# allenai/embodied-clip

Measured on AMD Instinct MI355X. Metric: env-frames/sec (CLIP encode + policy fwd/bwd + PPO update), higher is better.
Workload: dtype bf16

## Files before the change

embodied_clip_amd/_lib.py:

```python
from __future__ import annotations

import ctypes as C
import os

_HERE = os.path.dirname(os.path.abspath(__file__))
LIB_PATH = os.environ.get("EC_AMD_LIB") or os.path.join(_HERE, "lib", "libec_amd.so")

c_void_p, c_int, c_size_t, c_float = C.c_void_p, C.c_int, C.c_size_t, C.c_float

SIGNATURES = {
    "ec_version": (c_int, []),
    "ec_strerror": (C.c_char_p, [c_int]),
    "ec_bind_streams": (c_int, [c_void_p, c_int, c_int]),
    "ec_stream_pair_overlap": (c_int, [c_void_p, c_void_p, c_int, c_void_p]),
    "ec_conv_bf16": (c_int, [c_void_p] * 5 + [c_int] * 8 + [c_void_p]),
    "ec_conv_bf16_ld": (c_int, [c_void_p] * 5 + [c_int] * 9 + [c_void_p]),
    "ec_conv3x3_img_pack": (c_int, [c_void_p, c_void_p, c_int, c_void_p]),
    "ec_conv3x3_img_bf16": (c_int, [c_void_p] * 4 + [c_int] * 5 + [c_void_p]),
    "ec_conv3x3_img_bf16_ld": (c_int, [c_void_p] * 4 + [c_int] * 6 + [c_void_p]),
    "ec_bneck3_packed_elems": (c_size_t, [c_int]),
    "ec_bneck3_pack_weights": (c_int, [c_void_p] * 4 + [c_int, c_void_p]),
    "ec_bneck_conv123_bf16": (c_int, [c_void_p] * 6 + [c_int] * 4 + [c_void_p]),
    "ec_bneck_packed_elems": (c_size_t, [c_int]),
    "ec_bneck_pack_weights": (c_int, [c_void_p] * 3 + [c_int, c_void_p]),
    "ec_bneck_conv23_bf16": (c_int, [c_void_p] * 6 + [c_int] * 4 + [c_void_p]),
    "ec_clip_resize_table_ints": (c_size_t, [c_int, c_int, c_int]),
    "ec_clip_resize_table": (c_int, [c_int, c_int, c_int, c_void_p, c_size_t]),
    "ec_clip_resize_crop_u8": (c_int, [c_void_p, c_void_p, c_int, c_void_p, c_int, c_int, c_int, c_int, c_void_p]),
    "ec_semantic_labels_u8": (c_int, [c_void_p] * 4 + [c_int] * 4 + [c_void_p]),
    "ec_gemm_bf16": (c_int, [c_void_p] * 5 + [c_int] * 4 + [c_void_p]),
    "ec_split3_bf16": (c_int, [c_void_p] * 2 + [C.c_long, c_int, c_void_p]),
    "ec_gemm_bf16a_x3": (c_int, [c_void_p] * 4 + [C.c_long, c_int, c_int, c_int, c_void_p]),
    "ec_dw_tn_x3_splits": (c_int, [C.c_long, c_int]),
    "ec_dw_tn_x3": (c_int, [c_void_p] * 4 + [C.c_long, c_int, c_void_p]),
    "ec_stem_conv1": (c_int, [c_void_p] * 4 + [c_int] * 4 + [c_void_p]),
    "ec_avgpool2_bf16": (c_int, [c_void_p] * 2 + [c_int] * 4 + [c_void_p]),
    "ec_avgpool2_bf16_ld": (c_int, [c_void_p] * 2 + [c_int] * 5 + [c_void_p]),
    "ec_nhwc_bf16_to_nchw_f32": (c_int, [c_void_p] * 2 + [c_int] * 3 + [c_void_p]),
    "ec_nchw_f32_to_nhwc_bf16": (c_int, [c_void_p, c_void_p, c_int, c_int, c_int, c_void_p, c_void_p]),
    "ec_spatial_mean_bf16": (c_int, [c_void_p] * 2 + [c_int] * 3 + [c_void_p]),
    "ec_rn50_create": (c_int, [C.POINTER(c_void_p), c_int, C.POINTER(c_int), c_int, c_void_p, c_void_p, c_size_t,
                               c_void_p, c_size_t]),
    "ec_rn50tv_create": (c_int, [C.POINTER(c_void_p), C.POINTER(c_int), c_int, c_void_p, c_void_p, c_size_t, c_void_p,
                                 c_size_t]),
    "ec_conv_bf16_s2": (c_int, [c_void_p] * 5 + [c_int] * 7 + [c_void_p]),
    "ec_basic_tail_s2_bf16": (c_int, [c_void_p] * 5 + [c_int] * 6 + [c_void_p]),
    "ec_tvresnet_basic_create": (c_int, [C.POINTER(c_void_p), C.POINTER(c_int), c_int, c_void_p, c_void_p, c_size_t,
                                         c_void_p, c_size_t]),
    "ec_stem7_pool": (c_int, [c_void_p, c_int, C.POINTER(c_float), C.POINTER(c_float), c_void_p, c_void_p, c_void_p,
                              c_int, c_int, c_int, c_void_p]),
    "ec_rn50_destroy": (None, [c_void_p]),
    "ec_rn50_workspace_bytes": (c_size_t, [c_void_p, c_int]),
    "ec_rn50_out_channels": (c_int, [c_void_p]),
    "ec_rn50_out_spatial": (c_int, [c_void_p]),
    "ec_rn50_forward": (c_int, [c_void_p, c_void_p, c_int, c_void_p, c_size_t, c_void_p, c_int, c_void_p]),
    "ec_stem_conv1_depth": (c_int, [c_void_p, c_float, c_float, c_void_p, c_void_p, c_void_p] + [c_int] * 4 + [c_void_p]),
    "ec_rn50_forward_depth": (c_int, [c_void_p, c_void_p, c_float, c_float, c_void_p, c_int, c_void_p, c_size_t, c_void_p, c_int,
                                      c_void_p]),
    "ec_spatial_mean_pair_bf16": (c_int, [c_void_p] * 3 + [c_int] * 3 + [c_void_p]),
    "ec_rn50_rgbd_workspace_bytes": (c_size_t, [c_void_p, c_int]),
    "ec_rn50_embed_rgbd": (c_int, [c_void_p, c_void_p, c_int, C.POINTER(c_float), C.POINTER(c_float), c_void_p, c_float, c_float,
                                   c_void_p, c_int, c_void_p, c_size_t, c_void_p, c_int, c_void_p]),
    "ec_rn50_num_ops": (c_int, [c_void_p]),
    "ec_rn50_plan_hash": (C.c_uint64, [c_void_p]),
    "ec_rn50_set_conv8_min_tiles": (c_int, [c_void_p, c_int]),
    "ec_text_create": (c_int, [C.POINTER(c_void_p), c_int, c_int, c_int, c_int, c_int, c_int, c_void_p, c_size_t, c_void_p,
                               c_size_t]),
    "ec_text_destroy": (None, [c_void_p]),
    "ec_text_workspace_bytes": (c_size_t, [c_void_p, c_int]),
    "ec_text_forward": (c_int, [c_void_p, c_void_p, c_int, c_void_p, c_size_t, c_void_p, c_void_p]),
    "ec_probe_head": (c_int, [c_int, c_void_p, c_void_p, c_void_p, c_int, c_int, c_int, c_void_p, c_void_p, c_void_p,
                              c_void_p, c_void_p]),
    "ec_probe_pool3": (c_int, [c_void_p, c_void_p, c_int, c_int, c_int, c_int, c_void_p]),
    "ec_conv1x1_pair_pool_bf16": (c_int, [c_void_p] * 9 + [c_int] * 6 + [c_void_p]),
    "ec_conv1x1_pair_bf16": (c_int, [c_void_p] * 11 + [C.c_long, c_int, c_int, c_int, c_void_p]),
    "ec_stem_conv1_u8": (c_int, [c_void_p, C.POINTER(c_float), C.POINTER(c_float), c_void_p, c_void_p, c_void_p]
                         + [c_int] * 4 + [c_void_p]),
    "ec_rn50_forward_u8": (c_int, [c_void_p, c_void_p, C.POINTER(c_float), C.POINTER(c_float), c_int, c_void_p,
                                   c_size_t, c_void_p, c_int, c_void_p]),
    "ec_gemm_f32": (c_int, [c_void_p] * 3 + [c_int] * 3 + [C.c_long] * 4 + [c_int, c_int] + [c_void_p] * 3 + [c_int]
                    + [c_void_p] * 2 + [c_int, c_void_p]),
    "ec_policy_create": (c_int, [C.POINTER(c_void_p), c_void_p]),
    "ec_policy_destroy": (None, [c_void_p]),
    "ec_policy_num_param_tensors": (c_int, [c_void_p]),
    "ec_policy_flat_size": (c_size_t, [c_void_p]),
    "ec_policy_param_offset": (c_int, [c_void_p, c_int, C.POINTER(c_size_t), C.POINTER(c_size_t)]),
    "ec_policy_workspace_bytes": (c_size_t, [c_void_p, c_int, c_int, c_int]),
    "ec_policy_forward": (c_int, [c_void_p, c_void_p, c_void_p, c_int, c_void_p, c_void_p, c_void_p, c_int, c_int,
                                  c_void_p, c_size_t, c_int, c_void_p, c_void_p, c_void_p]),
    "ec_policy_forward2": (c_int, [c_void_p, c_void_p, c_void_p, c_void_p, c_int, c_void_p, c_void_p, c_void_p, c_int, c_int,
                                   c_void_p, c_size_t, c_int, c_void_p, c_void_p, c_void_p]),
    "ec_policy_act": (c_int, [c_void_p] * 4 + [c_int] + [c_void_p] * 3 + [c_int, c_void_p, c_size_t, c_int] + [c_void_p] * 5
                      + [C.c_uint64, C.c_uint64, c_int, c_void_p]),
    "ec_policy_forward_vec": (c_int, [c_void_p, c_void_p, c_void_p, c_void_p, c_int, c_void_p, c_void_p, c_void_p, c_int, c_int,
                                      c_void_p, c_size_t, c_int, c_void_p, c_void_p, c_void_p]),
    "ec_policy_act_vec": (c_int, [c_void_p] * 4 + [c_int] + [c_void_p] * 3 + [c_int, c_void_p, c_size_t, c_int] + [c_void_p] * 5
                          + [C.c_uint64, C.c_uint64, c_int, c_void_p]),
    "ec_policy_act_greedy": (c_int, [c_void_p] * 4 + [c_int] + [c_void_p] * 3 + [c_int, c_void_p, c_size_t, c_int] + [c_void_p] * 5
                             + [c_void_p]),
    "ec_policy_act_vec_greedy": (c_int, [c_void_p] * 4 + [c_int] + [c_void_p] * 3 + [c_int, c_void_p, c_size_t, c_int] + [c_void_p] * 5
                                 + [c_void_p]),
    "ec_policy_backward2": (c_int, [c_void_p, c_void_p, c_void_p, c_void_p, c_int, c_void_p, c_int, c_int, c_void_p, c_size_t,
                                    c_void_p, c_void_p, c_void_p, c_void_p]),
    "ec_policy_backward3": (c_int, [c_void_p, c_void_p, c_void_p, c_void_p, c_int, c_void_p, c_int, c_int, c_void_p, c_size_t,
                                    c_void_p, c_void_p, c_void_p, c_void_p, c_void_p]),
    "ec_policy_set_goal_table": (c_int, [c_void_p, c_void_p]),
    "ec_policy_backward": (c_int, [c_void_p, c_void_p, c_void_p, c_int, c_void_p, c_int, c_int, c_void_p, c_size_t,
                                   c_void_p, c_void_p, c_void_p, c_void_p]),
    "ec_gae": (c_int, [c_void_p] * 7 + [c_int, c_int, c_float, c_float, c_float, c_void_p]),
    "ec_ppo_loss": (c_int, [c_void_p] * 8 + [C.c_long, c_int, c_float, c_float, c_float, c_float, c_void_p]),
    "ec_ppo_loss_ex": (c_int, [c_void_p] * 8 + [C.c_long, c_int, c_float, c_float, c_float, c_float, c_float, c_void_p]),
    "ec_sample_actions": (c_int, [c_void_p] * 4 + [c_int, c_int, C.c_uint64, C.c_uint64, c_int, c_void_p]),
    "ec_mode_actions": (c_int, [c_void_p] * 4 + [c_int, c_int, c_void_p]),
    "ec_episode_stats": (c_int, [c_void_p] * 8 + [c_int, c_void_p, c_int, c_int, c_void_p]),
    "ec_nav_episode_stats": (c_int, [c_void_p] * 7 + [c_int] + [c_void_p] * 6 + [c_int, c_void_p, c_int, c_int, c_void_p]),
    "ec_vit_create": (c_int, [C.POINTER(c_void_p), c_int, c_int, c_int, c_int, c_int, c_void_p, c_size_t, c_void_p,
                              c_size_t]),
    "ec_vit_destroy": (None, [c_void_p]),
    "ec_vit_tokens": (c_int, [c_void_p]),
    "ec_vit_set_conv8_min_tiles": (c_int, [c_void_p, c_int]),
    "ec_vit_plan_hash": (C.c_uint64, [c_void_p]),
    "ec_vit_workspace_bytes": (c_size_t, [c_void_p, c_int]),
    "ec_vit_forward": (c_int, [c_void_p, c_void_p, c_int, c_void_p, c_size_t, c_void_p, c_void_p]),
    "ec_mha_bf16": (c_int, [c_void_p] * 2 + [c_int] * 5 + [c_void_p]),
    "ec_layernorm_bf16": (c_int, [c_void_p] * 4 + [C.c_long, c_int, c_void_p]),
    "ec_vit_assemble_bf16": (c_int, [c_void_p] * 7 + [c_int] * 3 + [c_void_p]),
    "ec_row_stats_bf16": (c_int, [c_void_p] * 2 + [C.c_long, c_int, c_void_p]),
    "ec_ln_fold_bf16": (c_int, [c_void_p] * 7 + [c_int] * 2 + [c_void_p]),
    "ec_gemm_bf16_ln": (c_int, [c_void_p] * 5 + [c_int] * 4 + [c_void_p] * 2 + [c_int, c_void_p, C.POINTER(c_int), c_void_p]),
    "ec_bf16_to_f32": (c_int, [c_void_p, c_void_p, C.c_long, C.c_long, C.c_long, c_void_p]),
    "ec_attnpool_workspace_bytes": (c_size_t, [c_int, c_int, c_int]),
    "ec_attnpool_forward": (c_int, [c_void_p, c_int, c_int, c_int, c_int, c_int] + [c_void_p] * 8 + [c_size_t, c_void_p,
                                    c_void_p]),
    "ec_clip_adam_scratch_doubles": (c_int, []),
    "ec_clip_adam_step": (c_int, [c_void_p] * 5 + [C.c_long, c_float, c_float, c_float, c_float, c_float, c_int,
                                  c_void_p]),
    "ec_imitation_scratch_doubles": (c_int, []),
    "ec_imitation_loss": (c_int, [c_void_p] * 7 + [C.c_long, c_int, c_float, c_float, c_int, c_void_p]),
    "ec_expert_count": (c_int, [c_void_p, c_int, c_int, c_int, c_int, c_void_p, c_void_p]),
    "ec_teacher_force": (c_int, [c_void_p] * 3 + [c_float] + [c_void_p] * 2 + [c_int, c_int, C.c_uint64, C.c_uint64, c_int,
                                                                            c_void_p]),
    "ec_heads_wide": (c_int, [c_void_p] * 6 + [C.c_long, c_int, c_int] + [c_void_p] * 3 + [c_int, C.c_uint64, C.c_uint64, c_int]
                      + [c_void_p] * 2 + [c_float, c_void_p]),
    "ec_policy_act_ex": (c_int, [c_void_p] * 4 + [c_int] + [c_void_p] * 4 + [c_int, c_void_p, c_size_t, c_int] + [c_void_p] * 5
                         + [c_int, C.c_uint64, C.c_uint64, c_int] + [c_void_p] * 2 + [c_float, c_void_p]),
    "ec_ppo_loss_wide_scratch_doubles": (c_int, []),
    "ec_ppo_loss_wide": (c_int, [c_void_p] * 9 + [C.c_long, c_int, c_float, c_float, c_float, c_float, c_float, c_void_p]),
    "ec_prev_action_table": (c_int, [c_void_p, c_void_p, C.c_long, c_int, c_void_p, c_int, c_int, c_int, c_int, c_void_p]),
    "ec_prev_action_add": (c_int, [c_void_p] * 4 + [c_int, c_int, C.c_long, c_int, c_void_p]),
    "ec_prev_action_grad_scratch_floats": (c_size_t, [C.c_long, c_int, c_int, c_int]),
    "ec_policy_forward_pa": (c_int, [c_void_p] * 4 + [c_int] + [c_void_p] * 5 + [c_int, c_int, c_void_p, c_size_t, c_int] + [c_void_p] * 3),
    "ec_policy_act_pa": (c_int, [c_void_p] * 4 + [c_int] + [c_void_p] * 5 + [c_int, c_void_p, c_size_t, c_int] + [c_void_p] * 5
                         + [c_int, C.c_uint64, C.c_uint64, c_int] + [c_void_p] * 2 + [c_float, c_void_p]),
    "ec_prev_action_grad": (c_int, [c_void_p] * 3 + [c_int, c_int, c_void_p, c_void_p, C.c_long, c_int] + [c_void_p] * 3
                            + [C.c_long, c_int, c_int, c_void_p]),
    "ec_policy_create_rnn": (c_int, [C.POINTER(c_void_p), c_void_p, c_int]),
    "ec_policy_rnn_type": (c_int, [c_void_p]),
    "ec_policy_create_rnn_layers": (c_int, [C.POINTER(c_void_p), c_void_p, c_int, c_int]),
    "ec_policy_rnn_layers": (c_int, [c_void_p]),
    "ec_rnn_stack_step_fwd": (c_int, [c_int, c_void_p, C.c_long] + [c_void_p] * 5 + [C.c_long, c_void_p, c_void_p, C.c_long, c_void_p, C.c_long,
                                      c_void_p, C.c_long, c_int, c_int, c_void_p]),
    "ec_policy_state_width": (c_int, [c_void_p]),
    "ec_lstm_step_fwd": (c_int, [c_void_p] * 4 + [C.c_long, c_void_p, c_void_p, C.c_long, c_void_p, C.c_long, c_void_p, c_int, c_int,
                                 c_void_p]),
    "ec_lstm_step_bwd": (c_int, [c_void_p] * 12 + [c_int, c_int, c_void_p]),
    "ec_policy_create_pooled": (c_int, [C.POINTER(c_void_p), c_void_p]),
    "ec_policy_is_pooled": (c_int, [c_void_p]),
    "ec_policy_forward_pooled": (c_int, [c_void_p] * 8 + [c_int, c_int, c_void_p, c_size_t, c_int] + [c_void_p] * 3),
    "ec_policy_act_pooled": (c_int, [c_void_p] * 8 + [c_int, c_void_p, c_size_t, c_int] + [c_void_p] * 5
                             + [c_int, C.c_uint64, C.c_uint64, c_int] + [c_void_p] * 2 + [c_float, c_void_p]),
    "ec_pooled_fc_act": (c_int, [c_void_p] * 5 + [c_int] * 3 + [c_void_p]),
    "ec_pooled_step0_fwd": (c_int, [c_int, c_void_p, C.c_long] + [c_void_p] * 7 + [c_int, c_void_p, c_void_p, c_int, c_int, c_void_p, c_void_p,
                                    c_int, c_void_p, C.c_long, c_void_p, c_void_p, C.c_long, c_void_p, C.c_long, c_void_p, C.c_long, c_int,
                                    c_int, c_void_p]),
}

RNN_TYPES = {"GRU": 0, "LSTM": 1}


class PolicyCfg(C.Structure):
    _fields_ = [(n, c_int) for n in ("in_channels", "spatial", "hidden", "goal_dims", "num_goals", "num_actions",
                                     "compress_hid", "compress_out", "comb_hid", "comb_out", "fusion", "dual", "goal_in",
                                     "prev_action_dims", "prev_action_null")]


class PooledCfg(C.Structure):
    _fields_ = [("embed_in", c_int), ("hidden", c_int), ("embed_dims", c_int), ("num_goals", c_int), ("num_sensors", c_int),
                ("sensor_in", c_int * 3), ("num_actions", c_int), ("prev_action_dims", c_int), ("prev_action_null", c_int),
                ("rnn_type", c_int), ("num_layers", c_int)]


_lib = None


class EcError(RuntimeError):
    pass


def load() -> C.CDLL:
    global _lib
    if _lib is not None:
        return _lib
    if not os.path.exists(LIB_PATH):
        raise ImportError(
            f"embodied_clip_amd: HIP library not found at {LIB_PATH}. Build it with `make` or "
            "`python -c 'import __graft_entry__ as g; g.build()'` (needs hipcc, gfx950). "
            "There is deliberately no CPU fallback.")
    lib = C.CDLL(LIB_PATH)
    for name, (res, args) in SIGNATURES.items():
        fn = getattr(lib, name)
        fn.restype = res
        fn.argtypes = args
    _lib = lib
    return lib


def check(rc: int, what: str = "") -> None:
    if rc != 0:
        msg = load().ec_strerror(rc).decode()
        raise EcError(f"{what or 'ec_amd call'} failed: {msg} (code {rc})")


def ptr(t) -> int:
    return 0 if t is None else t.data_ptr()


def stream_ptr(device=None) -> int:
    import torch
# ... 56 lines not shown
```

embodied_clip_amd/csrc/conv_pair.hip:

```cpp
#include <stdlib.h>

#include <type_traits>
#include <utility>

#include "common.h"

namespace {

typedef unsigned int u32x4 __attribute__((ext_vector_type(4)));
constexpr int PX = 32;
constexpr int NY = 256;
constexpr int KA = 64;
constexpr int SP = 272;
constexpr int STG = PX * SP;

struct PairArgs {
    const uint16_t *a0, *a1, *w0, *w1, *w2, *res;
    const float *b0, *b1, *b2;
    uint16_t *y, *z;
    int ntiles;
    uint16_t* yp;
    int H, W;
};

__device__ __forceinline__ float pq_xor1(float v) {
    return __builtin_bit_cast(float, __builtin_amdgcn_update_dpp(0, __builtin_bit_cast(int, v), 0xB1, 0xF, 0xF, true));
}
__device__ __forceinline__ float pq_xor2(float v) {
    return __builtin_bit_cast(float, __builtin_amdgcn_update_dpp(0, __builtin_bit_cast(int, v), 0x4E, 0xF, 0xF, true));
}

__device__ __forceinline__ int pw_off(int row, int chunk) {
    return row * 128 + ((chunk ^ ((row >> 1) & 7)) << 4);
}

template <int I, int LEAD, class AddrFn>
__device__ __forceinline__ void lsm_issue(u32x4 (&ring)[LEAD], AddrFn& addr) {
    const auto a = addr(std::integral_constant<int, I>{});
    asm volatile("ds_read_b128 %0, %1 offset:%2" : "=v"(ring[I % LEAD]) : "v"(a.first), "n"(decltype(a.second)::value));
}
template <int I, int NSTEP, int LEAD, class AddrFn, class MmaFn>
__device__ __forceinline__ void lsm_step(u32x4 (&ring)[LEAD], AddrFn& addr, MmaFn& mma) {
    if constexpr (I < NSTEP) {
        constexpr int after = (LEAD - 1 < NSTEP - 1 - I) ? LEAD - 1 : NSTEP - 1 - I;
        asm volatile("s_waitcnt lgkmcnt(%1)" : "+v"(ring[I % LEAD]) : "n"(after));
        mma(std::integral_constant<int, I>{}, ring[I % LEAD]);
        if constexpr (I + LEAD < NSTEP) lsm_issue<I + LEAD, LEAD>(ring, addr);
        lsm_step<I + 1, NSTEP, LEAD>(ring, addr, mma);
    }
}
template <int I, int N, int LEAD, class AddrFn>
__device__ __forceinline__ void lsm_prologue(u32x4 (&ring)[LEAD], AddrFn& addr) {
    if constexpr (I < N) {
        lsm_issue<I, LEAD>(ring, addr);
        lsm_prologue<I + 1, N, LEAD>(ring, addr);
    }
}
template <int NSTEP, int LEAD, class AddrFn, class MmaFn>
__device__ __forceinline__ void lds_stream_mfma(AddrFn addr, MmaFn mma) {
    u32x4 ring[LEAD];
    lsm_prologue<0, (LEAD < NSTEP ? LEAD : NSTEP), LEAD>(ring, addr);
    lsm_step<0, NSTEP, LEAD>(ring, addr, mma);
}

template <bool TWO, bool RES, int N2, bool PL>
__global__ __launch_bounds__(256, 1) void conv1x1_pair_kernel(PairArgs p) {
    static_assert(!PL || N2 == 128, "pooled variant: the layer-1 -> layer-2 boundary");
    constexpr int W0_BYTES = (TWO ? 2 : 1) * NY * 128;
    constexpr int W2_BYTES = 4 * N2 * 128;
    constexpr int FN2 = N2 / 32;
    extern __shared__ __attribute__((aligned(16))) unsigned char sm[];
    unsigned char* sW0 = sm;
    unsigned char* sW2 = sm + W0_BYTES;
    float* sBy = reinterpret_cast<float*>(sm + W0_BYTES + W2_BYTES);
    float* sBz = sBy + NY;
    const int tid = threadIdx.x, lane = tid & 63, wave = tid >> 6;
    unsigned char* stg = sm + W0_BYTES + W2_BYTES + (NY + N2) * 4 + wave * STG;
    const int px = lane & 31, h = lane >> 5;
    const unsigned w_lds = (unsigned)(unsigned long)(__attribute__((address_space(3))) unsigned char*)sW0;
    unsigned wk_off[4];
#pragma unroll
    for (int ks = 0; ks < 4; ++ks) wk_off[ks] = (unsigned)pw_off(px, 2 * ks + h);
    auto roff = [&](int r) -> int {
        if (!PL) return r;
        return (2 * (r >> 4) + ((r >> 1) & 1)) * p.W + 2 * ((r >> 2) & 3) + (r & 1);
    };
    const int roff_px = roff(px);
    int rrow[8];
#pragma unroll
    for (int j = 0; j < 8; ++j) rrow[j] = roff(4 * j + (lane >> 4));
    auto tile_base = [&](int tile) -> long {
        if (!PL) return (long)tile * PX;
        const int t = __builtin_amdgcn_readfirstlane(tile);
        const int tpr = p.W / 8, tpi = (p.H / 4) * tpr;
        const int b = t / tpi, rem = t - b * tpi, ty = rem / tpr, tx = rem - ty * tpr;
        return ((long)b * p.H + 4 * ty) * p.W + 8 * tx;
    };

    ec_stage_all<(TWO ? 2 : 1) * NY * 8, 256, uint4>(
        tid,
        [&](int idx) {
            const int kt = idx / (NY * 8), r = (idx / 8) % NY, c = idx & 7;
            return *reinterpret_cast<const uint4*>((kt == 0 ? p.w0 : p.w1) + r * KA + c * 8);
        },
        [&](int idx, const uint4& v) {
            const int kt = idx / (NY * 8), r = (idx / 8) % NY, c = idx & 7;
            *reinterpret_cast<uint4*>(sW0 + kt * (NY * 128) + pw_off(r, c)) = v;
        });
    ec_stage_all<N2 * 32, 256, uint4>(
        tid,
        [&](int idx) {
            const int n = idx >> 5, q = idx & 31;
            const int s = q >> 1, hh = q & 1;
            const int c0 = 32 * (s >> 1) + 16 * (s & 1) + 4 * hh;
            const uint2 lo = *reinterpret_cast<const uint2*>(p.w2 + n * NY + c0);
            const uint2 hi = *reinterpret_cast<const uint2*>(p.w2 + n * NY + c0 + 8);
            return make_uint4(lo.x, lo.y, hi.x, hi.y);
        },
        [&](int idx, const uint4& v) {
            const int n = idx >> 5, q = idx & 31;
            const int s = q >> 1, hh = q & 1;
            *reinterpret_cast<uint4*>(sW2 + (s >> 2) * (N2 * 128) + pw_off(n, 2 * (s & 3) + hh)) = v;
        });
    for (int i = tid; i < NY; i += 256) sBy[i] = p.b0[i] + (TWO ? p.b1[i] : 0.f);
    for (int i = tid; i < N2; i += 256) sBz[i] = p.b2[i];
    __syncthreads();

    const int gw = blockIdx.x * 4 + wave, GW = gridDim.x * 4;
    int t = gw;
    if (t >= p.ntiles) return;

    u32x4 a0n[4], a1n[TWO ? 4 : 1], rn[RES ? 16 : 1];
    auto prefetch = [&](int tile) {
        const long m0 = tile_base(tile);
#pragma unroll
        for (int ks = 0; ks < 4; ++ks) {
            a0n[ks] = *reinterpret_cast<const u32x4*>(p.a0 + (m0 + roff_px) * KA + (2 * ks + h) * 8);
            if (TWO) a1n[ks] = *reinterpret_cast<const u32x4*>(p.a1 + (m0 + roff_px) * KA + (2 * ks + h) * 8);
        }
        if constexpr (RES) {
            [&]<int... I>(std::integer_sequence<int, I...>) {
                ((rn[I] = *reinterpret_cast<const u32x4*>(p.res + (m0 + rrow[I & 7]) * NY + (I >> 3) * 128 +
                                                          (((I & 7) * 64 + lane) & 15) * 8)), ...);
            }(std::make_integer_sequence<int, 16>{});
        }
    };
    prefetch(t);

    for (;;) {
        const long m0 = tile_base(t);
        u32x4 a0c[4], a1c[TWO ? 4 : 1], rc[RES ? 16 : 1];
#pragma unroll
        for (int ks = 0; ks < 4; ++ks) { a0c[ks] = a0n[ks]; if (TWO) a1c[ks] = a1n[ks]; }
        if constexpr (RES) {
            [&]<int... I>(std::integer_sequence<int, I...>) { ((rc[I] = rn[I]), ...); }(std::make_integer_sequence<int, 16>{});
        }
        const int tn = t + GW;
        const bool more = tn < p.ntiles;
        if (more) prefetch(tn);

        f32x16_t acc[8];
#pragma unroll
        for (int j = 0; j < 8; ++j)
#pragma unroll
            for (int r = 0; r < 16; ++r) acc[j][r] = 0.f;
        {
            constexpr int PER_KS = (TWO ? 16 : 8);
            lds_stream_mfma<4 * PER_KS, 8>(
                [&](auto ic) {
                    constexpr int i = decltype(ic)::value, ks = i / PER_KS, r = i % PER_KS, j = r & 7, second = r >> 3;
                    return std::pair<unsigned, std::integral_constant<int, second * (NY * 128) + j * 4096>>{w_lds + wk_off[ks], {}};
                },
                [&](auto ic, const u32x4& wf) {
                    constexpr int i = decltype(ic)::value, ks = i / PER_KS, r = i % PER_KS, j = r & 7, second = r >> 3;
                    acc[j] = __builtin_amdgcn_mfma_f32_32x32x16_bf16(__builtin_bit_cast(bf16x8_t, wf),
                                                                     __builtin_bit_cast(bf16x8_t, second ? a1c[TWO ? ks : 0] : a0c[ks]),
                                                                     acc[j], 0, 0, 0);
                });
        }

        uint4 P[8][2];
        long pool_base = 0;
        if constexpr (PL) {
            const int tt = __builtin_amdgcn_readfirstlane(t);
            const int tpr = p.W / 8, tpi = (p.H / 4) * tpr;
            const int b = tt / tpi, rem = tt - b * tpi, ty = rem / tpr, tx = rem - ty * tpr;
            pool_base = ((long)b * (p.H / 2) + 2 * ty) * (p.W / 2) + 4 * tx;
        }
        auto half_epilogue = [&](auto hfc) {
            constexpr int hf = decltype(hfc)::value;
            if constexpr (RES) {
                [&]<int... I>(std::integer_sequence<int, I...>) {
                    ((*reinterpret_cast<u32x4*>(stg + ((I * 64 + lane) >> 4) * SP + ((I * 64 + lane) & 15) * 16) = rc[hf * 8 + I]), ...);
                }(std::make_integer_sequence<int, 8>{});
            }
#pragma unroll
            for (int jj = 0; jj < 4; ++jj) {
                const int j = hf * 4 + jj;
                unsigned pk[8];
#pragma unroll
                for (int g = 0; g < 4; ++g) {
                    const int lc = 32 * jj + 8 * g + 4 * h;
                    const float4 bv = *reinterpret_cast<const float4*>(sBy + hf * 128 + lc);
                    float v0 = acc[j][4 * g + 0] + bv.x, v1 = acc[j][4 * g + 1] + bv.y;
                    float v2 = acc[j][4 * g + 2] + bv.z, v3 = acc[j][4 * g + 3] + bv.w;
                    uint2* slot = reinterpret_cast<uint2*>(stg + px * SP + lc * 2);
                    if (RES) {
                        const uint2 rr = *slot;
                        v0 += ec_lo(rr.x); v1 += ec_hi(rr.x); v2 += ec_lo(rr.y); v3 += ec_hi(rr.y);
                    }
                    v0 = fmaxf(v0, 0.f); v1 = fmaxf(v1, 0.f); v2 = fmaxf(v2, 0.f); v3 = fmaxf(v3, 0.f);
                    uint2 o;
                    o.x = ec_pack2(v0, v1);
                    o.y = ec_pack2(v2, v3);
                    *slot = o;
                    pk[2 * g] = o.x; pk[2 * g + 1] = o.y;
                }
                P[j][0] = make_uint4(pk[0], pk[1], pk[2], pk[3]);
                P[j][1] = make_uint4(pk[4], pk[5], pk[6], pk[7]);
            }
            if constexpr (PL) {
#pragma unroll
                for (int it2 = 0; it2 < 2; ++it2) {
                    const int item = it2 * 64 + lane, w = item >> 4, c = item & 15;
                    const uint4 r0 = *reinterpret_cast<const uint4*>(stg + (4 * w + 0) * SP + c * 16);
                    const uint4 r1 = *reinterpret_cast<const uint4*>(stg + (4 * w + 1) * SP + c * 16);
                    const uint4 r2 = *reinterpret_cast<const uint4*>(stg + (4 * w + 2) * SP + c * 16);
                    const uint4 r3 = *reinterpret_cast<const uint4*>(stg + (4 * w + 3) * SP + c * 16);
                    auto avg2 = [](unsigned a, unsigned b, unsigned cc, unsigned d) {
                        const float lo = 0.25f * ((ec_lo(a) + ec_lo(b)) + (ec_lo(cc) + ec_lo(d)));
                        const float hi = 0.25f * ((ec_hi(a) + ec_hi(b)) + (ec_hi(cc) + ec_hi(d)));
                        return ec_pack2(lo, hi);
                    };
                    u32x4 po;
                    po[0] = avg2(r0.x, r1.x, r2.x, r3.x); po[1] = avg2(r0.y, r1.y, r2.y, r3.y);
                    po[2] = avg2(r0.z, r1.z, r2.z, r3.z); po[3] = avg2(r0.w, r1.w, r2.w, r3.w);
                    *reinterpret_cast<u32x4*>(p.yp + (pool_base + (w >> 2) * (p.W / 2) + (w & 3)) * NY + hf * 128 + c * 8) = po;
                }
            }
            if (!PL || p.y) {
#pragma unroll
            for (int i = 0; i < 8; ++i) {
                const int idx = i * 64 + lane;
                const uint4 v = *reinterpret_cast<const uint4*>(stg + (idx >> 4) * SP + (idx & 15) * 16);
                __builtin_nontemporal_store(__builtin_bit_cast(u32x4, v), reinterpret_cast<u32x4*>(p.y + (m0 + rrow[i]) * NY + hf * 128 + (idx & 15) * 8));
            }
            }
        };
        half_epilogue(std::integral_constant<int, 0>{});
        half_epilogue(std::integral_constant<int, 1>{});

        f32x16_t acc2[FN2];
#pragma unroll
        for (int n = 0; n < FN2; ++n)
#pragma unroll
            for (int r = 0; r < 16; ++r) acc2[n][r] = 0.f;
        lds_stream_mfma<16 * FN2, 8>(
            [&](auto ic) {
                constexpr int i = decltype(ic)::value, st = i / FN2, n = i % FN2;
                return std::pair<unsigned, std::integral_constant<int, (st >> 2) * (N2 * 128) + n * 4096>>{w_lds + (unsigned)W0_BYTES + wk_off[st & 3], {}};
            },
            [&](auto ic, const u32x4& wf) {
                constexpr int i = decltype(ic)::value, st = i / FN2, n = i % FN2;
                acc2[n] = __builtin_amdgcn_mfma_f32_32x32x16_bf16(__builtin_bit_cast(bf16x8_t, wf),
                                                                  __builtin_bit_cast(bf16x8_t, P[st >> 1][st & 1]), acc2[n], 0, 0, 0);
            });
        constexpr int ZP = N2 * 2 + 16;
        constexpr int ZC = N2 / 8;
#pragma unroll
        for (int n = 0; n < FN2; ++n)
#pragma unroll
            for (int g = 0; g < 4; ++g) {
                const int lc = 32 * n + 8 * g + 4 * h;
                const float4 bv = *reinterpret_cast<const float4*>(sBz + lc);
                uint2 o;
                o.x = ec_pack2(fmaxf(acc2[n][4 * g + 0] + bv.x, 0.f), fmaxf(acc2[n][4 * g + 1] + bv.y, 0.f));
                o.y = ec_pack2(fmaxf(acc2[n][4 * g + 2] + bv.z, 0.f), fmaxf(acc2[n][4 * g + 3] + bv.w, 0.f));
                *reinterpret_cast<uint2*>(stg + px * ZP + lc * 2) = o;
            }
#pragma unroll
        for (int i = 0; i < PX * ZC / 64; ++i) {
            const int idx = i * 64 + lane;
            const uint4 v = *reinterpret_cast<const uint4*>(stg + (idx / ZC) * ZP + (idx % ZC) * 16);
            __builtin_nontemporal_store(__builtin_bit_cast(u32x4, v), reinterpret_cast<u32x4*>(p.z + (m0 + (PL ? rrow[i] : idx / ZC)) * N2 + (idx % ZC) * 8));
        }
        if (!more) break;
        t = tn;
    }
}

template <bool TWO, bool RES, int N2, bool PL = false>
int launch_pair(const PairArgs& p, hipStream_t s) {
    constexpr size_t lds = (size_t)(TWO ? 2 : 1) * NY * 128 + 4 * N2 * 128 + (NY + N2) * 4 + 4 * STG;
    static_assert(lds <= 160 * 1024, "LDS budget");
    auto kern = conv1x1_pair_kernel<TWO, RES, N2, PL>;
    static std::atomic<uint64_t> attr_done{0};
    if (auto attr_g_ = ec_attr_needed(attr_done)) {
        (void)hipFuncSetAttribute(reinterpret_cast<const void*>(kern), hipFuncAttributeMaxDynamicSharedMemorySize, (int)lds);
    }
    const int wgs = (p.ntiles + 3) / 4 < 256 ? (p.ntiles + 3) / 4 : 256;
    hipLaunchKernelGGL(kern, dim3((unsigned)wgs), dim3(256), lds, s, p);
    EC_CHECK_LAUNCH();
    return EC_OK;
}


constexpr int K2 = 128, NY2 = 512, NZ2 = 128;
constexpr int YP2 = NY2 * 2 + 16;
constexpr int SP2 = 256 + 16;

struct Pair2Args {
    const uint16_t *a0, *w0, *w2, *res;
    const float *b0, *b2;
    uint16_t *y, *z;
    int ntiles;
};

__global__ __launch_bounds__(256, 1) void conv1x1_pair512_kernel(Pair2Args p) {
    extern __shared__ __attribute__((aligned(16))) unsigned char sm[];
    unsigned char* ytile = sm;
    float* sBy = reinterpret_cast<float*>(sm + 2 * PX * YP2);
    float* sBz = sBy + NY2;
    const int tid = threadIdx.x, lane = tid & 63, wave = tid >> 6;
    unsigned char* stg = sm + 2 * PX * YP2 + (NY2 + NZ2) * 4 + wave * (PX * SP2);
    unsigned char* atile = sm + 2 * PX * YP2 + (NY2 + NZ2) * 4 + 4 * (PX * SP2);
    const int px = lane & 31, h = lane >> 5;

    for (int i = tid; i < NY2; i += 256) sBy[i] = p.b0[i];
    for (int i = tid; i < NZ2; i += 256) sBz[i] = p.b2[i];

    u32x4 w0f[4][8];
    u32x4 w2f[32];
    [&]<int... I>(std::integer_sequence<int, I...>) {
        ((w0f[I >> 3][I & 7] = *reinterpret_cast<const u32x4*>(p.w0 + (long)(128 * wave + 32 * (I >> 3) + px) * K2 + 16 * (I & 7) + 8 * h)), ...);
    }(std::make_integer_sequence<int, 32>{});
    [&]<int... I>(std::integer_sequence<int, I...>) {
        ((w2f[I] = *reinterpret_cast<const u32x4*>(p.w2 + (long)(32 * wave + px) * NY2 + 16 * I + 8 * h)), ...);
    }(std::make_integer_sequence<int, 32>{});
    __syncthreads();

    int t = blockIdx.x;
    if (t >= p.ntiles) return;
    const int G = gridDim.x;

    u32x4 an[2], rn[8];
    auto prefetch = [&](int tile) {
        const long m0 = (long)tile * PX;
        [&]<int... I>(std::integer_sequence<int, I...>) {
            ((an[I] = *reinterpret_cast<const u32x4*>(p.a0 + (m0 + 8 * wave + 4 * I + (lane >> 4)) * K2 + (lane & 15) * 8)), ...);
        }(std::make_integer_sequence<int, 2>{});
        [&]<int... I>(std::integer_sequence<int, I...>) {
            ((rn[I] = *reinterpret_cast<const u32x4*>(p.res + (m0 + ((I * 64 + lane) >> 4)) * NY2 + 128 * wave + ((I * 64 + lane) & 15) * 8)), ...);
        }(std::make_integer_sequence<int, 8>{});
    };
    auto publish_a = [&](int buf) {
        [&]<int... I>(std::integer_sequence<int, I...>) {
            ((*reinterpret_cast<u32x4*>(atile + buf * (PX * SP2) + (8 * wave + 4 * I + (lane >> 4)) * SP2 + (lane & 15) * 16) = an[I]), ...);
        }(std::make_integer_sequence<int, 2>{});
    };
    prefetch(t);
    publish_a(0);
    __syncthreads();

    for (int it = 0;; ++it) {
        const long m0 = (long)t * PX;
        unsigned char* yt = ytile + (it & 1) * (PX * YP2);
        u32x4 rc[8];
        [&]<int... I>(std::integer_sequence<int, I...>) { ((rc[I] = rn[I]), ...); }(std::make_integer_sequence<int, 8>{});
        const unsigned char* at = atile + (it & 1) * (PX * SP2);
        const int tn = t + G;
        const bool more = tn < p.ntiles;
        if (more) prefetch(tn);

        f32x16_t acc[4];
#pragma unroll
        for (int j = 0; j < 4; ++j)
#pragma unroll
            for (int r = 0; r < 16; ++r) acc[j][r] = 0.f;
        {
            const unsigned a_lds = (unsigned)(unsigned long)(__attribute__((address_space(3))) const unsigned char*)at +
                                   (unsigned)(px * SP2 + 16 * h);
            lds_stream_mfma<8, 6>(
                [&](auto ic) { return std::pair<unsigned, std::integral_constant<int, 32 * decltype(ic)::value>>{a_lds, {}}; },
                [&](auto ic, const u32x4& avr) {
                    constexpr int ks = decltype(ic)::value;
                    const bf16x8_t av = __builtin_bit_cast(bf16x8_t, avr);
#pragma unroll
                    for (int j = 0; j < 4; ++j)
                        acc[j] = __builtin_amdgcn_mfma_f32_32x32x16_bf16(__builtin_bit_cast(bf16x8_t, w0f[j][ks]), av, acc[j], 0, 0, 0);
                });
        }

        [&]<int... I>(std::integer_sequence<int, I...>) {
            ((*reinterpret_cast<u32x4*>(stg + ((I * 64 + lane) >> 4) * SP2 + ((I * 64 + lane) & 15) * 16) = rc[I]), ...);
        }(std::make_integer_sequence<int, 8>{});
#pragma unroll
        for (int j = 0; j < 4; ++j)
#pragma unroll
            for (int g = 0; g < 4; ++g) {
                const int lc = 32 * j + 8 * g + 4 * h;
                const float4 bv = *reinterpret_cast<const float4*>(sBy + 128 * wave + lc);
                uint2* slot = reinterpret_cast<uint2*>(stg + px * SP2 + lc * 2);
                const uint2 rr = *slot;
                const float v0 = fmaxf(acc[j][4 * g + 0] + bv.x + ec_lo(rr.x), 0.f), v1 = fmaxf(acc[j][4 * g + 1] + bv.y + ec_hi(rr.x), 0.f);
                const float v2 = fmaxf(acc[j][4 * g + 2] + bv.z + ec_lo(rr.y), 0.f), v3 = fmaxf(acc[j][4 * g + 3] + bv.w + ec_hi(rr.y), 0.f);
                uint2 o;
                o.x = ec_pack2(v0, v1);
                o.y = ec_pack2(v2, v3);
                *slot = o;
                *reinterpret_cast<uint2*>(yt + px * YP2 + (128 * wave + lc) * 2) = o;
            }
#pragma unroll
        for (int i = 0; i < 8; ++i) {
            const int idx = i * 64 + lane;
            const u32x4 v = *reinterpret_cast<const u32x4*>(stg + (idx >> 4) * SP2 + (idx & 15) * 16);
            __builtin_nontemporal_store(v, reinterpret_cast<u32x4*>(p.y + (m0 + (idx >> 4)) * NY2 + 128 * wave + (idx & 15) * 8));
        }
        if (more) publish_a((it + 1) & 1);
        __syncthreads();

        f32x16_t acc2;
#pragma unroll
        for (int r = 0; r < 16; ++r) acc2[r] = 0.f;
        {
            const unsigned y_lds = (unsigned)(unsigned long)(__attribute__((address_space(3))) const unsigned char*)yt +
                                   (unsigned)(px * YP2 + 16 * h);
            lds_stream_mfma<32, 8>(
                [&](auto ic) { return std::pair<unsigned, std::integral_constant<int, 32 * decltype(ic)::value>>{y_lds, {}}; },
                [&](auto ic, const u32x4& yv) {
                    constexpr int I = decltype(ic)::value;
                    acc2 = __builtin_amdgcn_mfma_f32_32x32x16_bf16(__builtin_bit_cast(bf16x8_t, w2f[I]), __builtin_bit_cast(bf16x8_t, yv), acc2, 0, 0, 0);
                });
// ... 78 lines not shown
    u32x4 an[AL], rn[RES ? OL : 1];
    const int Wq = PL ? p.W / 2 : 1, QPF = PL ? (p.H / 2) * Wq : 1;
    const int coff = PL ? ((lane >> 5) & 1) * p.W + ((lane >> 4) & 1) : 0;
    auto qpix = [&](int q_) -> long {
        const int q = __builtin_amdgcn_readfirstlane(q_);
        const int f = q / QPF, rem = q - f * QPF, qr = rem / Wq, qc = rem - qr * Wq;
        return ((long)f * p.H + 2 * qr) * p.W + 2 * qc;
    };
    long opix[PL ? OL : 1];
    auto prefetch = [&](int tile) {
        const long m0 = (long)tile * PX;
        if constexpr (PL) {
            static_assert(!PL || (CPR == 16 && OC == 16 && AL == 2 && OL == 8), "row = 4 I + (lane >> 4)");
            [&]<int... I>(std::integer_sequence<int, I...>) {
                ((an[I] = *reinterpret_cast<const u32x4*>(p.a + (qpix(8 * tile + 2 * wave + I) + coff) * K + (lane & 15) * 8)), ...);
            }(std::make_integer_sequence<int, AL>{});
            [&]<int... I>(std::integer_sequence<int, I...>) {
                ((opix[I] = qpix(8 * tile + I) + coff,
                  rn[I] = *reinterpret_cast<const u32x4*>(resg + opix[I] * ld + NPW * wave + (lane & 15) * 8)), ...);
            }(std::make_integer_sequence<int, OL>{});
            return;
        }
        [&]<int... I>(std::integer_sequence<int, I...>) {
            ((an[I] = *reinterpret_cast<const u32x4*>(p.a + (m0 + 8 * wave + (I * 64 + lane) / CPR) * K + ((I * 64 + lane) % CPR) * 8)), ...);
        }(std::make_integer_sequence<int, AL>{});
        if constexpr (RES) {
            [&]<int... I>(std::integer_sequence<int, I...>) {
                ((rn[I] = *reinterpret_cast<const u32x4*>(resg + (m0 + (I * 64 + lane) / OC) * ld + NPW * wave + ((I * 64 + lane) % OC) * 8)), ...);
            }(std::make_integer_sequence<int, OL>{});
        }
    };
    auto publish_a = [&](int buf) {
        [&]<int... I>(std::integer_sequence<int, I...>) {
            ((*reinterpret_cast<u32x4*>(atile + buf * (PX * AP) + (8 * wave + (I * 64 + lane) / CPR) * AP + ((I * 64 + lane) % CPR) * 16) = an[I]), ...);
        }(std::make_integer_sequence<int, AL>{});
    };
    prefetch(t);
    publish_a(0);
    __syncthreads();

    for (int it = 0;; ++it) {
        const long m0 = (long)t * PX;
        const unsigned char* at = atile + (it & 1) * (PX * AP);
        u32x4 rc[RES ? OL : 1];
        long opc[PL ? OL : 1];
        if constexpr (RES) {
            [&]<int... I>(std::integer_sequence<int, I...>) { ((rc[I] = rn[I]), ...); }(std::make_integer_sequence<int, OL>{});
        }
        if constexpr (PL) {
            [&]<int... I>(std::integer_sequence<int, I...>) { ((opc[I] = opix[I]), ...); }(std::make_integer_sequence<int, OL>{});
        }
        const int tn = t + G;
        const bool more = tn < p.ntiles;
        if (more) prefetch(tn);

        f32x16_t acc[FJ];
#pragma unroll
        for (int j = 0; j < FJ; ++j)
#pragma unroll
            for (int r = 0; r < 16; ++r) acc[j][r] = 0.f;
        {
            const unsigned a_lds = (unsigned)(unsigned long)(__attribute__((address_space(3))) const unsigned char*)at +
                                   (unsigned)(px * AP + 16 * h);
            lds_stream_mfma<KS, (KS < 6 ? KS : 6)>(
                [&](auto ic) { return std::pair<unsigned, std::integral_constant<int, 32 * decltype(ic)::value>>{a_lds, {}}; },
                [&](auto ic, const u32x4& avr) {
                    constexpr int I = decltype(ic)::value;
                    const bf16x8_t av = __builtin_bit_cast(bf16x8_t, avr);
#pragma unroll
                    for (int j = 0; j < FJ; ++j)
                        acc[j] = __builtin_amdgcn_mfma_f32_32x32x16_bf16(__builtin_bit_cast(bf16x8_t, wf[j][I]), av, acc[j], 0, 0, 0);
                });
        }

        if constexpr (RES) {
            [&]<int... I>(std::integer_sequence<int, I...>) {
                ((*reinterpret_cast<u32x4*>(stg + ((I * 64 + lane) / OC) * OPW + ((I * 64 + lane) % OC) * 16) = rc[I]), ...);
            }(std::make_integer_sequence<int, OL>{});
        }
#pragma unroll
        for (int j = 0; j < FJ; ++j)
#pragma unroll
            for (int g = 0; g < 4; ++g) {
                const int lc = 32 * j + 8 * g + 4 * h;
                const float4 bv = *reinterpret_cast<const float4*>(sB + NPW * wave + lc);
                uint2* slot = reinterpret_cast<uint2*>(stg + px * OPW + lc * 2);
                float v0 = acc[j][4 * g + 0] + bv.x, v1 = acc[j][4 * g + 1] + bv.y;
                float v2 = acc[j][4 * g + 2] + bv.z, v3 = acc[j][4 * g + 3] + bv.w;
                if constexpr (RES) {
                    const uint2 rr = *slot;
                    v0 += ec_lo(rr.x); v1 += ec_hi(rr.x); v2 += ec_lo(rr.y); v3 += ec_hi(rr.y);
                }
                if constexpr (RELU) { v0 = fmaxf(v0, 0.f); v1 = fmaxf(v1, 0.f); v2 = fmaxf(v2, 0.f); v3 = fmaxf(v3, 0.f); }
                uint2 o;
                o.x = ec_pack2(v0, v1);
                o.y = ec_pack2(v2, v3);
                *slot = o;
            }
#pragma unroll
        for (int i = 0; i < OL; ++i) {
            const int idx = i * 64 + lane;
            const u32x4 v = *reinterpret_cast<const u32x4*>(stg + (idx / OC) * OPW + (idx % OC) * 16);
            if constexpr (PL) *reinterpret_cast<u32x4*>(yg + opc[i] * ld + NPW * wave + (idx % OC) * 8) = v;
            else
            *reinterpret_cast<u32x4*>(yg + (m0 + idx / OC) * ld + NPW * wave + (idx % OC) * 8) = v;
        }
        if constexpr (PL) {
#pragma unroll
            for (int it2 = 0; it2 < 2; ++it2) {
                const int item = it2 * 64 + lane, w = item >> 4, c = item & 15;
                const uint4 r0 = *reinterpret_cast<const uint4*>(stg + (4 * w + 0) * OPW + c * 16);
                const uint4 r1 = *reinterpret_cast<const uint4*>(stg + (4 * w + 1) * OPW + c * 16);
                const uint4 r2 = *reinterpret_cast<const uint4*>(stg + (4 * w + 2) * OPW + c * 16);
                const uint4 r3 = *reinterpret_cast<const uint4*>(stg + (4 * w + 3) * OPW + c * 16);
                auto avg2 = [](unsigned a, unsigned b, unsigned cc, unsigned d) {
                    const float lo = 0.25f * (ec_lo(a) + ec_lo(b) + ec_lo(cc) + ec_lo(d));
                    const float hi = 0.25f * (ec_hi(a) + ec_hi(b) + ec_hi(cc) + ec_hi(d));
                    return ec_pack2(lo, hi);
                };
                u32x4 po;
                po[0] = avg2(r0.x, r1.x, r2.x, r3.x); po[1] = avg2(r0.y, r1.y, r2.y, r3.y);
                po[2] = avg2(r0.z, r1.z, r2.z, r3.z); po[3] = avg2(r0.w, r1.w, r2.w, r3.w);
                *reinterpret_cast<u32x4*>(p.yp + ((long)t * 8 + w) * p.ldp + c0 + NPW * wave + c * 8) = po;
            }
        }
        if (!more) break;
        publish_a((it + 1) & 1);
        __syncthreads();
        t = tn;
    }
}

template <int K, int N, bool RES, bool RELU, bool PL = false>
int launch_regw(const RegwArgs& p, hipStream_t s, int groups = 1) {
    constexpr size_t lds = 2 * (size_t)PX * (K * 2 + 16) + N * 4 + 4 * (size_t)PX * (N / 4 * 2 + 16);
    static_assert(lds <= 160 * 1024, "LDS budget");
    auto kern = conv1x1_regw_kernel<K, N, RES, RELU, PL>;
    static std::atomic<uint64_t> attr_done{0};
    if (auto attr_g_ = ec_attr_needed(attr_done)) {
        (void)hipFuncSetAttribute(reinterpret_cast<const void*>(kern), hipFuncAttributeMaxDynamicSharedMemorySize, (int)lds);
    }
    int wgs = 256 / groups;
    if (wgs > p.ntiles) wgs = p.ntiles;
    hipLaunchKernelGGL(kern, dim3((unsigned)wgs, (unsigned)groups), dim3(256), lds, s, p);
    EC_CHECK_LAUNCH();
    return EC_OK;
}

}

extern "C" int ec_conv1x1_pair_bf16(const void* a0, const void* w0, const float* b0, const void* a1, const void* w1,
                                    const float* b1, const void* res, void* y, const void* w2, const float* b2, void* z,
                                    long M, int K0, int N, int N2, ec_stream_t stream) {
    if (!a0 || !w0 || !b0 || !y || !w2 || !b2 || !z) return EC_ERR_ARG;
    if ((a1 != nullptr) != (w1 != nullptr) || (a1 != nullptr) != (b1 != nullptr)) return EC_ERR_ARG;
    if (M <= 0 || (M % PX) != 0 || M / PX > 0x7fffffffL) return EC_ERR_SHAPE;
    if (K0 == K2 && N == NY2 && N2 == NZ2) {
        if (a1 || !res) return EC_ERR_SHAPE;
        Pair2Args q{(const uint16_t*)a0, (const uint16_t*)w0, (const uint16_t*)w2, (const uint16_t*)res, b0, b2, (uint16_t*)y,
                    (uint16_t*)z, (int)(M / PX)};
        return launch_pair512(q, (hipStream_t)stream);
    }
    if (K0 != KA || N != NY || (N2 != 64 && N2 != 128)) return EC_ERR_SHAPE;
    PairArgs p{(const uint16_t*)a0, (const uint16_t*)a1, (const uint16_t*)w0, (const uint16_t*)w1, (const uint16_t*)w2,
               (const uint16_t*)res, b0, b1, b2, (uint16_t*)y, (uint16_t*)z, (int)(M / PX), nullptr, 0, 0};
    hipStream_t s = (hipStream_t)stream;
    const bool two = a1 != nullptr, hres = res != nullptr;
    if (N2 == 64) {
        if (two && hres) return launch_pair<true, true, 64>(p, s);
        if (two) return launch_pair<true, false, 64>(p, s);
        if (hres) return launch_pair<false, true, 64>(p, s);
        return launch_pair<false, false, 64>(p, s);
    }
    if (two) return EC_ERR_SHAPE;
    if (hres) return launch_pair<false, true, 128>(p, s);
    return launch_pair<false, false, 128>(p, s);
}

extern "C" int ec_conv1x1_pair_pool_bf16(const void* a0, const void* w0, const float* b0, const void* res, void* y,
                                         void* y_pooled, const void* w2, const float* b2, void* z, int B, int H, int W,
                                         int K0, int N, int N2, ec_stream_t stream) {
    if (!a0 || !w0 || !b0 || !res || !y_pooled || !w2 || !b2 || !z) return EC_ERR_ARG;
    if (K0 != KA || N != NY || N2 != 128 || B <= 0 || H <= 0 || W <= 0 || (H % 4) != 0 || (W % 8) != 0) return EC_ERR_SHAPE;
    const long tiles = (long)B * (H / 4) * (W / 8);
    if (tiles > 0x7fffffffL) return EC_ERR_SHAPE;
    PairArgs p{(const uint16_t*)a0, nullptr, (const uint16_t*)w0, nullptr, (const uint16_t*)w2, (const uint16_t*)res, b0,
               nullptr, b2, (uint16_t*)y, (uint16_t*)z, (int)tiles, (uint16_t*)y_pooled, H, W};
    return launch_pair<false, true, 128, true>(p, (hipStream_t)stream);
}

int ec_conv1x1_regw(const void* a, const void* w, const float* bias, const void* res, void* y, long M, int K, int N, int act,
                    hipStream_t s) {
    const bool on = ec_config().conv_regw != 0;
    if (!on || (M % PX) != 0 || M / PX > 0x7fffffffL) return EC_ERR_SHAPE;
    const long tiles = M / PX;
    RegwArgs p{(const uint16_t*)a, (const uint16_t*)w, (const uint16_t*)res, bias, (uint16_t*)y, (int)tiles, N, nullptr, 0, 0, 0};
    if (tiles >= 1024) {
        if (K == 256 && N == 512 && !res && act == EC_ACT_NONE) return launch_regw<256, 512, false, false>(p, s);
        if (K == 512 && N == 256 && !res && act == EC_ACT_RELU) return launch_regw<512, 256, false, true>(p, s);
        if (K == 128 && N == 512 && res && act == EC_ACT_RELU) return launch_regw<128, 512, true, true>(p, s);
    }
    return EC_ERR_SHAPE;
}

int ec_conv1x1_regw_pool(const void* a, const void* w, const float* bias, const void* res, void* y, void* y_pooled, int B, int H,
                         int W, int K, int N, int act, int ld_pooled, hipStream_t s) {
    if (!a || !w || !bias || !res || !y || !y_pooled) return EC_ERR_ARG;
    if (!ec_config().conv_regw || !ec_config().rn50_poolout) return EC_ERR_SHAPE;
    if (K != 128 || N != 512 || act != EC_ACT_RELU || B <= 0 || (H & 1) || (W & 1) || ld_pooled < N || (ld_pooled & 7) ||
        ((size_t)y_pooled & 15))
        return EC_ERR_SHAPE;
    const long windows = (long)B * (H / 2) * (W / 2);
    if ((windows % 8) != 0 || windows / 8 < 1024 || windows / 8 > 0x7fffffffL) return EC_ERR_SHAPE;
    RegwArgs p{(const uint16_t*)a, (const uint16_t*)w, (const uint16_t*)res, bias, (uint16_t*)y, (int)(windows / 8), N,
               (uint16_t*)y_pooled, ld_pooled, H, W};
    return launch_regw<128, 512, true, true, true>(p, s);
}
```

embodied_clip_amd/csrc/rn50.hip:

```cpp
#include <stdlib.h>

#include <new>
#include <vector>

#include "common.h"


namespace {

enum OpKind { OP_STEM1, OP_CONV, OP_POOL, OP_PAIR, OP_BNECK, OP_STEM7, OP_BTAIL, OP_CAT, OP_CONV_POOLOUT };

constexpr int BUF_NONE = -1, BUF_IN = -2, BUF_OUT = -3;

struct Slot { size_t w = 0, b = 0; };

struct Conv {
    int src, dst, res;
    int H, W, Cin, Cout, ks, pool, act;
    int stride;
    Slot at;
    int ldo = 0, ocol = 0;
    int img_max = 0;
    size_t wimg_off = 0;
};

struct Cat { Slot a, b; int Ka, Kb; size_t w_off = 0, b_off = 0; };

struct Op {
    OpKind kind;
    Conv c;
    struct { int src, dst, H, W, C, ldo, ocol, pool_of; } pl;
    struct { int dst, ld, col; } pd;
    Conv c1, c2, c3, ds, next_c1;
    bool fold_ds;
    int pooled_dst;
    bool fold_c1;
    size_t wpack_off;
    Cat cat;
};

}

struct ec_rn50 {
    int width, res, out_c, out_sp;
    int tv = 0;
    std::vector<Op> ops;
    size_t max_elems_per_frame;
    const float* stem_w;
    const uint16_t* w;
    const float* bias;
    size_t n_w, n_b;
    int conv8_min_tiles = 0;
    uint16_t* wbneck = nullptr;
    float* bias_cat = nullptr;
    ~ec_rn50() {
        if (wbneck) (void)hipFree(wbneck);
        if (bias_cat) (void)hipFree(bias_cat);
    }
};

namespace {
constexpr int NBUF = 5;
inline size_t align_up(size_t v, size_t a) { return (v + a - 1) / a * a; }

enum TowerKind { CLIP = 0, TV_BOTTLENECK = 1, TV_BASIC = 2 };

struct Blk {
    int li, planes, inplanes, stride;
    int R, Ro;
    int x, out;
    int y;
    bool ds, last_of_layer;
    Slot c1, c2, c3, dsc;
};
struct Arch { TowerKind kind; int width, R1; Slot stem[3], total; std::vector<Blk> B; };

Arch walk_arch(TowerKind kind, int width, int sc, const int* layers4, int R) {
    Arch a{kind, width, R};
    Slot& at = a.total;
    auto take = [&](size_t Cout, size_t K) { const Slot s = at; at.w += Cout * K; at.b += Cout; return s; };
    a.stem[0] = take(kind == CLIP ? sc : width, 0);
    if (kind == CLIP) { a.stem[1] = take(sc, (size_t)9 * sc); a.stem[2] = take(width, (size_t)9 * sc); }
    const int expansion = kind == TV_BASIC ? 1 : 4;
    int inplanes = width, x = 0;
    for (int li = 0; li < 4; ++li)
        for (int b = 0; b < layers4[li]; ++b) {
            Blk k{li, width << li, inplanes, (b == 0 && li > 0) ? 2 : 1};
            const size_t p = k.planes, in = inplanes;
            k.ds = k.stride > 1 || inplanes != k.planes * expansion;
            k.last_of_layer = b + 1 == layers4[li];
            k.R = R; k.Ro = R / k.stride;
            k.x = x; k.y = k.out = (x == 0) ? 4 : 0;
            k.c1 = take(p, kind == TV_BASIC ? 9 * in : in);
            k.c2 = take(p, 9 * p);
            if (kind != TV_BASIC) k.c3 = take(4 * p, p);
            if (k.ds) k.dsc = take(expansion * p, in);
            a.B.push_back(k);
            x = k.y; inplanes = k.planes * expansion; R = k.Ro;
        }
    if (!a.B.empty()) a.B.back().out = BUF_OUT;
    return a;
}

int img3_max_frames(const Conv& c, bool bneck_conv2 = false) {
    if (!ec_config().rn50_img3 || c.ks != 3) return 0;
    if (bneck_conv2) return 32;
    if (c.Cin != 512 || c.Cout != 512 || c.res >= 0) return 0;
    return !c.pool && c.H == 7 && c.W == 7 ? 64 : c.pool && c.H == 14 && c.W == 14 ? 16 : 0;
}

Conv mk_conv(int src, int dst, int res, int H, int W, int Cin, int Cout, int ks, int pool, int act, Slot at, int stride = 1) {
    Conv c{src, dst, res, H, W, Cin, Cout, ks, pool, act, stride, at};
    c.img_max = img3_max_frames(c);
    return c;
}

struct Plan {
    std::vector<Op>& ops;
    size_t mx = 0;
    void track(int H, int W, int C) { mx = std::max(mx, (size_t)H * W * C); }
    void push(const Op& o, int H, int W, int C) { ops.push_back(o); track(H, W, C); }
    void conv(const Conv& c) {
        Op o{OP_CONV, c};
        const int half = (c.pool || c.stride == 2) ? 2 : 1;
        push(o, c.H / half, c.W / half, c.Cout);
    }
    void pool(int src, int dst, int R, int C, int ldo, int ocol, bool pool_of) {
        Op o{OP_POOL};
        o.pl = {src, dst, R, R, C, ldo, ocol, pool_of};
        push(o, R / 2, R / 2, ldo ? ldo : C);
    }
};

struct Given { int c1_buf = BUF_NONE, pooled_in = BUF_NONE; };

enum Form {
    F_PLAIN,
    F_POOLOUT,
    F_PAIR1,
    F_PAIR1_POOL,
    F_PAIR2,
    F_CAT,
    F_BNECK
};

Form block_form(const Arch& a, size_t i) {
    const Blk& k = a.B[i];
    const Blk* nx = i + 1 < a.B.size() ? &a.B[i + 1] : nullptr;
    const auto& cfg = ec_config();
    const bool fuse = cfg.rn50_fuse != 0 && a.width == 64 && (a.R1 % 8) == 0;
    if (fuse && k.li == 0 && nx && nx->li <= 1 && (!k.ds || (k.inplanes == k.planes && !k.last_of_layer)))
        return (a.kind == CLIP && k.last_of_layer && !k.ds) ? F_PAIR1_POOL : F_PAIR1;
    if (k.ds && a.kind == CLIP && k.stride > 1 && k.li >= 2 && cfg.rn50_dscat && (k.planes % 8) == 0) return F_CAT;
    if (fuse && k.li == 1 && k.planes == 128 && !k.last_of_layer) return F_PAIR2;
    if (cfg.rn50_bneck > 0 && !k.ds && k.stride == 1 && k.planes == 256 && k.Ro == 14) return F_BNECK;
    if (cfg.rn50_poolout && k.planes == 128 && nx && block_form(a, i + 1) == F_CAT) return F_POOLOUT;
    return F_PLAIN;
}

Given plan_bottleneck(Plan& p, const Arch& a, size_t i, Given g) {
    const Blk& k = a.B[i];
    const Blk* nx = i + 1 < a.B.size() ? &a.B[i + 1] : nullptr;
    const Form f = block_form(a, i);
    const bool tv = a.kind != CLIP, c1_given = g.c1_buf != BUF_NONE;
    const int planes = k.planes, inplanes = k.inplanes, R = k.R, Ro = k.Ro, x = k.x, c1_buf = c1_given ? g.c1_buf : 1;
    const bool fold_c1 = f == F_BNECK && ec_config().rn50_bneck3 && !c1_given;
    const Conv c1 = mk_conv(x, 1, BUF_NONE, R, R, inplanes, planes, 1, 0, EC_ACT_RELU, k.c1);
    Conv c2 = tv && k.stride > 1 ? mk_conv(c1_buf, 2, BUF_NONE, R, R, planes, planes, 3, 0, EC_ACT_RELU, k.c2, 2)
                                 : mk_conv(c1_buf, 2, BUF_NONE, R, R, planes, planes, 3, k.stride > 1 ? 1 : 0, EC_ACT_RELU, k.c2);
    if (!c1_given && !fold_c1) p.conv(c1);
    Op o{};
    if (f == F_BNECK) {
        o.kind = OP_BNECK; o.fold_c1 = fold_c1;
        o.c1 = c1; o.c2 = c2; o.c2.img_max = img3_max_frames(c2, true);
        o.c3 = mk_conv(2, k.out, x, Ro, Ro, planes, planes * 4, 1, 0, EC_ACT_RELU, k.c3);
        p.push(o, Ro, Ro, planes * 4);
        return Given{};
    }
    if (f == F_PAIR1 || f == F_PAIR1_POOL) {
        p.conv(c2);
        o.kind = OP_PAIR;
        o.c3 = mk_conv(2, k.out, k.ds ? BUF_NONE : x, R, R, planes, planes * 4, 1, 0, EC_ACT_RELU, k.c3);
        o.fold_ds = k.ds;
        if (k.ds) o.ds = mk_conv(x, BUF_NONE, BUF_NONE, R, R, inplanes, planes * 4, 1, 0, EC_ACT_NONE, k.dsc);
        o.next_c1 = mk_conv(k.out, 1, BUF_NONE, R, R, planes * 4, nx->planes, 1, 0, EC_ACT_RELU, nx->c1);
        o.pooled_dst = f == F_PAIR1_POOL ? 3 : BUF_NONE;
        if (f == F_PAIR1_POOL) p.track(R / 2, R / 2, planes * 4);
        p.push(o, R, R, planes * 4);
        return Given{1, o.pooled_dst};
    }
    if (f == F_CAT) {
        const int Kc = planes + inplanes;
        const int cat = 3;
        c2.dst = cat; c2.ldo = Kc;
        p.conv(c2);
        p.pool(x, cat, R, inplanes, Kc, planes, i > 0 && block_form(a, i - 1) == F_POOLOUT);
        o.kind = OP_CAT;
        o.c = mk_conv(cat, k.out, BUF_NONE, Ro, Ro, Kc, planes * 4, 1, 0, EC_ACT_RELU, Slot{});
        o.cat = Cat{k.c3, k.dsc, planes, inplanes};
        p.push(o, Ro, Ro, planes * 4);
        return Given{};
    }
    p.conv(c2);
    int idt = x;
    if (k.ds) {
        int dsrc = x, ddst = 3;
        if (tv) {
        } else if (k.stride > 1 && g.pooled_in != BUF_NONE) {
            dsrc = g.pooled_in;
            ddst = 1;
        } else if (k.stride > 1) {
            p.pool(x, k.y, R, inplanes, 0, 0, false);
            dsrc = k.y;
        }
        p.conv(tv && k.stride > 1 ? mk_conv(dsrc, ddst, BUF_NONE, R, R, inplanes, planes * 4, 1, 0, EC_ACT_NONE, k.dsc, 2)
                                  : mk_conv(dsrc, ddst, BUF_NONE, Ro, Ro, inplanes, planes * 4, 1, 0, EC_ACT_NONE, k.dsc));
        idt = ddst;
    }
    const Conv c3 = mk_conv(2, k.out, idt, Ro, Ro, planes, planes * 4, 1, 0, EC_ACT_RELU, k.c3);
    if (f == F_PLAIN) { p.conv(c3); return Given{}; }
    if (f == F_PAIR2) {
        o.kind = OP_PAIR;
        o.c3 = c3;
        o.next_c1 = mk_conv(k.out, idt == 1 ? 3 : 1, BUF_NONE, Ro, Ro, planes * 4, planes, 1, 0, EC_ACT_RELU, nx->c1);
        o.pooled_dst = BUF_NONE;
    } else {
        o.kind = OP_CONV_POOLOUT;
        o.c = c3;
        o.pd = {3, nx->planes + nx->inplanes, nx->planes};
    }
    p.push(o, Ro, Ro, planes * 4);
    return f == F_PAIR2 ? Given{o.next_c1.dst, BUF_NONE} : Given{};
}

void plan_basic(Plan& p, const Blk& k) {
    const int planes = k.planes, Ro = k.Ro;
    p.conv(mk_conv(k.x, 1, BUF_NONE, k.R, k.R, k.inplanes, planes, 3, 0, EC_ACT_RELU, k.c1, k.stride));
    if (!k.ds) {
        p.conv(mk_conv(1, k.out, k.x, Ro, Ro, planes, planes, 3, 0, EC_ACT_RELU, k.c2));
        return;
    }
    Op o{};
    o.kind = OP_BTAIL;
    o.ds = mk_conv(k.x, 3, BUF_NONE, k.R, k.R, k.inplanes, planes, 1, 0, EC_ACT_NONE, k.dsc, 2);
    o.c2 = mk_conv(1, k.out, 3, Ro, Ro, planes, planes, 3, 0, EC_ACT_RELU, k.c2);
    o.cat = Cat{k.c2, k.dsc, 9 * planes, k.inplanes};
    p.push(o, Ro, Ro, planes);
}

int pack_plan_weights(ec_rn50* h) {
    size_t tot = 0, btot = 0;
    auto cat_n = [](const Op& o) { return (size_t)(o.kind == OP_CAT ? o.c.Cout : o.c2.Cout); };
    for (Op& o : h->ops)
        if (o.kind == OP_CAT || o.kind == OP_BTAIL) {
            o.cat.w_off = tot; tot += cat_n(o) * (size_t)(o.cat.Ka + o.cat.Kb);
            o.cat.b_off = btot; btot += cat_n(o);
        }
    for (Op& o : h->ops) {
        if (o.kind == OP_BNECK) { o.wpack_off = o.c2.wimg_off = tot; tot += ec_bneck3_packed_elems(o.c2.Cin); }
        if (o.kind == OP_CONV && o.c.img_max) { o.c.wimg_off = tot; tot += (size_t)o.c.Cout * 9 * o.c.Cin; }
    }
    if (btot && hipMalloc(&h->bias_cat, btot * sizeof(float)) != hipSuccess) { h->bias_cat = nullptr; return EC_ERR_LAUNCH; }
    if (!tot) return EC_OK;
    if (hipMalloc(&h->wbneck, tot * sizeof(uint16_t)) != hipSuccess) { h->wbneck = nullptr; return EC_ERR_LAUNCH; }
    auto pack_cat = [&](const Cat& c, size_t N) -> int {
        const size_t K = (size_t)c.Ka + c.Kb;
        uint16_t* wc = h->wbneck + c.w_off;
        if (hipMemcpy2D(wc, K * 2, h->w + c.a.w, (size_t)c.Ka * 2, (size_t)c.Ka * 2, N, hipMemcpyDeviceToDevice) != hipSuccess ||
            hipMemcpy2D(wc + c.Ka, K * 2, h->w + c.b.w, (size_t)c.Kb * 2, (size_t)c.Kb * 2, N, hipMemcpyDeviceToDevice) != hipSuccess) return EC_ERR_LAUNCH;
        std::vector<float> ba(N), bb(N);
        if (hipMemcpy(ba.data(), h->bias + c.a.b, N * 4, hipMemcpyDeviceToHost) != hipSuccess ||
            hipMemcpy(bb.data(), h->bias + c.b.b, N * 4, hipMemcpyDeviceToHost) != hipSuccess) return EC_ERR_LAUNCH;
        for (size_t i = 0; i < N; ++i) ba[i] += bb[i];
        return hipMemcpy(h->bias_cat + c.b_off, ba.data(), N * 4, hipMemcpyHostToDevice) != hipSuccess ? EC_ERR_LAUNCH : EC_OK;
    };
    for (const Op& o : h->ops) {
        int rc = EC_OK;
        if (o.kind == OP_CAT || o.kind == OP_BTAIL) rc = pack_cat(o.cat, cat_n(o));
        else if (o.kind == OP_BNECK)
            rc = o.fold_c1 ? ec_bneck3_pack_weights(h->w + o.c1.at.w, h->w + o.c2.at.w, h->w + o.c3.at.w, h->wbneck + o.wpack_off, o.c2.Cin, nullptr)
                           : ec_bneck_pack_weights(h->w + o.c2.at.w, h->w + o.c3.at.w, h->wbneck + o.wpack_off, o.c2.Cin, nullptr);
        else if (o.kind == OP_CONV && o.c.img_max) rc = ec_conv3x3_img_pack(h->w + o.c.at.w, h->wbneck + o.c.wimg_off, o.c.Cin, nullptr);
        if (rc != EC_OK) return EC_ERR_LAUNCH;
    }
    (void)hipStreamSynchronize(nullptr);
    return EC_OK;
}

int rn50_build(ec_rn50_t** out, TowerKind kind, int width, const int* layers4, int input_resolution, const void* stem_w,
               const void* w_bf16, size_t n_w, const float* bias, size_t n_bias) {
    if (!out || !layers4 || !stem_w || !w_bf16 || !bias) return EC_ERR_ARG;
    if (width % 32 != 0 || width < 32 || input_resolution % 32 != 0) return EC_ERR_SHAPE;
    if (kind == TV_BASIC && (input_resolution < 32 || layers4[0] < 1 || layers4[1] < 1 || layers4[2] < 1 || layers4[3] < 1)) return EC_ERR_SHAPE;
    const int sc = (width / 2 + 31) / 32 * 32, res = input_resolution;
    const Arch a = walk_arch(kind, width, sc, layers4, res / 4);
    if (n_w != a.total.w || n_bias != a.total.b) return EC_ERR_SHAPE;
    ec_rn50* h = new (std::nothrow) ec_rn50();
    if (!h) return EC_ERR_ALLOC;
    h->width = width; h->res = res; h->tv = kind;
    h->stem_w = (const float*)stem_w; h->w = (const uint16_t*)w_bf16; h->bias = bias;
    h->n_w = a.total.w; h->n_b = a.total.b;
    Plan p{h->ops};
    const int x0 = a.B.empty() ? BUF_OUT : 0;
    if (kind == CLIP) {
        const int R = res / 2;
        p.push(Op{OP_STEM1, mk_conv(BUF_IN, 1, BUF_NONE, res, res, 3, sc, 3, 0, EC_ACT_RELU, a.stem[0])}, R, R, sc);
        p.conv(mk_conv(1, 2, BUF_NONE, R, R, sc, sc, 3, 0, EC_ACT_RELU, a.stem[1]));
        p.conv(mk_conv(2, x0, BUF_NONE, R, R, sc, width, 3, 1, EC_ACT_RELU, a.stem[2]));
    } else {
        p.push(Op{OP_STEM7, mk_conv(BUF_IN, x0, BUF_NONE, res, res, 3, width, 7, 0, EC_ACT_RELU, a.stem[0])}, a.R1, a.R1, width);
    }
    Given g;
    for (size_t i = 0; i < a.B.size(); ++i)
        if (kind == TV_BASIC) plan_basic(p, a.B[i]);
        else g = plan_bottleneck(p, a, i, g);
    h->out_c = a.B.empty() ? width : a.B.back().planes * (kind == TV_BASIC ? 1 : 4);
    h->out_sp = a.B.empty() ? a.R1 : a.B.back().Ro;
    h->max_elems_per_frame = p.mx;
    const int rc = pack_plan_weights(h);
    if (rc != EC_OK) { delete h; return rc; }
    *out = h;
    return EC_OK;
}
}

extern "C" int ec_rn50_create(ec_rn50_t** out, int width, const int* layers4, int input_resolution, const float* stem_w_f32,
                              const void* w_bf16, size_t n_w, const float* bias, size_t n_bias) {
    return rn50_build(out, CLIP, width, layers4, input_resolution, stem_w_f32, w_bf16, n_w, bias, n_bias);
}

extern "C" int ec_rn50tv_create(ec_rn50_t** out, const int* layers4, int input_resolution, const void* stem_w_bf16,
                                const void* w_bf16, size_t n_w, const float* bias, size_t n_bias) {
    return rn50_build(out, TV_BOTTLENECK, 64, layers4, input_resolution, stem_w_bf16, w_bf16, n_w, bias, n_bias);
}

extern "C" int ec_tvresnet_basic_create(ec_rn50_t** out, const int* layers4, int input_resolution, const void* stem_w_bf16,
                                        const void* w_bf16, size_t n_w, const float* bias, size_t n_bias) {
    return rn50_build(out, TV_BASIC, 64, layers4, input_resolution, stem_w_bf16, w_bf16, n_w, bias, n_bias);
}

extern "C" void ec_rn50_destroy(ec_rn50_t* h) { delete h; }
extern "C" int ec_rn50_out_channels(const ec_rn50_t* h) { return h ? h->out_c : 0; }
extern "C" int ec_rn50_out_spatial(const ec_rn50_t* h) { return h ? h->out_sp : 0; }
extern "C" int ec_rn50_num_ops(const ec_rn50_t* h) { return h ? (int)h->ops.size() : 0; }

extern "C" uint64_t ec_rn50_plan_hash(const ec_rn50_t* h) {
    if (!h) return 0;
    uint64_t x = 1469598103934665603ull;
    auto mix = [&](long v) {
        for (int i = 0; i < 8; ++i) { x ^= (uint64_t)((v >> (8 * i)) & 0xff); x *= 1099511628211ull; }
    };
    mix(ec_version()); mix((long)ec_config_hash());
    mix(h->width); mix(h->res); mix(h->conv8_min_tiles); mix(h->tv);
    for (const Op& o : h->ops) {
        const Conv& c = o.kind == OP_PAIR || o.kind == OP_BNECK ? o.c3 : o.kind == OP_BTAIL ? o.c2 : o.c;
        long f[24] = {o.kind, c.src, c.dst, c.res, c.H, c.W, c.Cin, c.Cout, c.ks, c.pool, c.act, c.stride, -1, -1, 0, -1, 0, c.ldo, c.ocol, 0, -1, 0, 0, 0};
        if (o.kind == OP_POOL) {
            const long p[12] = {OP_POOL, o.pl.src, o.pl.dst, -1, o.pl.H, o.pl.W, o.pl.C, o.pl.C, 0, 0, 0, 1};
            std::copy(p, p + 12, f);
            f[17] = o.pl.ldo; f[18] = o.pl.ocol; f[23] = o.pl.pool_of;
        }
        if (o.kind == OP_PAIR) { f[12] = o.fold_ds ? o.ds.src : -1; f[13] = o.next_c1.dst; f[14] = o.next_c1.Cout; f[15] = o.pooled_dst; }
        if (o.kind == OP_BNECK) { f[1] = o.c2.src; f[8] = 3; f[16] = o.fold_c1; }
        if (o.kind == OP_BTAIL) { f[3] = -1; f[6] = o.cat.Ka + o.cat.Kb; f[12] = o.ds.src; f[14] = o.cat.Ka; f[19] = 1; }
        if (o.kind == OP_CAT) { f[0] = OP_CONV; f[14] = o.cat.Ka; f[19] = 1; }
        if (o.kind == OP_CONV_POOLOUT) { f[0] = OP_CONV; f[20] = o.pd.dst; f[21] = o.pd.ld; f[22] = o.pd.col; }
        for (long v : f) mix(v);
    }
    return x;
}

extern "C" int ec_rn50_set_conv8_min_tiles(ec_rn50_t* h, int n) {
    if (!h) return EC_ERR_ARG;
    h->conv8_min_tiles = n > 0 ? n : 0;
    return EC_OK;
}

extern "C" size_t ec_rn50_workspace_bytes(const ec_rn50_t* h, int batch) {
    if (!h || batch <= 0) return 0;
    return NBUF * align_up(h->max_elems_per_frame * 2 * (size_t)batch, 256);
}

namespace {
struct FrameIn {
    enum Kind { F32, U8, DEPTH, RGBD } kind;
    const void* p;
    const float *mean3, *std3;
    float scale, shift;
    const float* stem_w9;
    const float* depth = nullptr;
    bool rgb_u8 = false;
    bool u8() const { return kind == U8 || (kind == RGBD && rgb_u8); }
};
struct Run {
    const ec_rn50* h;
    const FrameIn& in;
    const void* frames;
    const float* depth;
    int nb;
    unsigned char* base;
    size_t bufsz;
    void* out;
    hipStream_t stream;
    bool pooled_emitted;
    void* buf(int id) const { return id == BUF_OUT ? out : base + (size_t)id * bufsz; }
    const void* opt(int id) const { return id == BUF_NONE ? nullptr : buf(id); }
};

int run_conv(const Run& r, const Conv& c) {
    const ec_rn50* h = r.h;
    if (c.stride == 2)
        return ec_conv_bf16_s2(r.buf(c.src), h->w + c.at.w, h->bias + c.at.b, r.opt(c.res), r.buf(c.dst), r.nb, c.H, c.W, c.Cin, c.Cout, c.ks,
                               c.act, r.stream);
    uint16_t* dst = (uint16_t*)r.buf(c.dst) + c.ocol;
    if (r.nb <= c.img_max)
        return ec_conv3x3_img_bf16_ld(r.buf(c.src), h->wbneck + c.wimg_off, h->bias + c.at.b, dst, r.nb, c.H, c.W, c.Cin, c.pool,
                                      c.ldo ? c.ldo : c.Cin, r.stream);
    return ec_conv_bf16_ld(r.buf(c.src), h->w + c.at.w, h->bias + c.at.b, r.opt(c.res), dst, r.nb, c.H, c.W, c.Cin, c.Cout, c.ks, c.pool, c.act,
                           c.ldo ? c.ldo : c.Cout, r.stream);
}

int run_stem(const Run& r, const Op& o) {
    const FrameIn& in = r.in;
    const Conv& c = o.c;
    const float* bias = r.h->bias + c.at.b;
    if (o.kind == OP_STEM7)
        return ec_stem7_pool(r.frames, in.u8() ? 1 : 0, in.mean3, in.std3, r.h->stem_w, bias, r.buf(c.dst), r.nb, c.H, c.W, r.stream);
    const int n_rgb = !r.frames ? 0 : r.depth ? r.nb / 2 : r.nb;
    int rc = EC_OK;
    if (n_rgb && in.u8())
        rc = ec_stem_conv1_u8((const uint8_t*)r.frames, in.mean3, in.std3, r.h->stem_w, bias, r.buf(c.dst), n_rgb, c.H, c.W, c.Cout, r.stream);
    else if (n_rgb)
        rc = ec_stem_conv1((const float*)r.frames, r.h->stem_w, bias, r.buf(c.dst), n_rgb, c.H, c.W, c.Cout, r.stream);
    if (rc != EC_OK || !r.depth) return rc;
    const size_t frame_out = (size_t)((c.H - 1) / 2 + 1) * ((c.W - 1) / 2 + 1) * c.Cout;
    return ec_stem_conv1_depth(r.depth, in.scale, in.shift, in.stem_w9, bias, (uint16_t*)r.buf(c.dst) + (size_t)n_rgb * frame_out, r.nb - n_rgb,
                               c.H, c.W, c.Cout, r.stream);
}

int run_pool(Run& r, const Op& o) {
    const auto& p = o.pl;
    if (p.pool_of && r.pooled_emitted) { r.pooled_emitted = false; return EC_OK; }
    if (p.ldo) return ec_avgpool2_bf16_ld(r.buf(p.src), (uint16_t*)r.buf(p.dst) + p.ocol, r.nb, p.H, p.W, p.C, p.ldo, r.stream);
    return ec_avgpool2_bf16(r.buf(p.src), r.buf(p.dst), r.nb, p.H, p.W, p.C, r.stream);
}

int run_conv_poolout(Run& r, const Op& o) {
    const Conv& c = o.c;
    const int rc = ec_conv1x1_regw_pool(r.buf(c.src), r.h->w + c.at.w, r.h->bias + c.at.b, r.buf(c.res), r.buf(c.dst),
                                        (uint16_t*)r.buf(o.pd.dst) + o.pd.col, r.nb, c.H, c.W, c.Cin, c.Cout, c.act, o.pd.ld, r.stream);
    if (rc == EC_OK) r.pooled_emitted = true;
    return rc == EC_ERR_SHAPE ? run_conv(r, c) : rc;
}

int run_cat(const Run& r, const Op& o) {
    const Conv& c = o.c;
    return ec_conv_bf16_ld(r.buf(c.src), r.h->wbneck + o.cat.w_off, r.h->bias_cat + o.cat.b_off, nullptr, r.buf(c.dst), r.nb, c.H, c.W, c.Cin,
                           c.Cout, 1, 0, c.act, c.Cout, r.stream);
}

int run_pair(const Run& r, const Op& o) {
    const ec_rn50* h = r.h;
    const Conv &c3 = o.c3, &c1 = o.next_c1;
    if (o.pooled_dst != BUF_NONE)
        return ec_conv1x1_pair_pool_bf16(r.buf(c3.src), h->w + c3.at.w, h->bias + c3.at.b, r.buf(c3.res), nullptr, r.buf(o.pooled_dst),
                                         h->w + c1.at.w, h->bias + c1.at.b, r.buf(c1.dst), r.nb, c3.H, c3.W, c3.Cin, c3.Cout, c1.Cout, r.stream);
    int rc = ec_conv1x1_pair_bf16(r.buf(c3.src), h->w + c3.at.w, h->bias + c3.at.b, o.fold_ds ? r.buf(o.ds.src) : nullptr,
                                  o.fold_ds ? h->w + o.ds.at.w : nullptr, o.fold_ds ? h->bias + o.ds.at.b : nullptr, r.opt(c3.res),
                                  r.buf(c3.dst), h->w + c1.at.w, h->bias + c1.at.b, r.buf(c1.dst), (long)r.nb * c3.H * c3.W, c3.Cin, c3.Cout,
                                  c1.Cout, r.stream);
    if (rc == EC_ERR_SHAPE && !o.fold_ds) {
        rc = run_conv(r, c3);
        if (rc == EC_OK) rc = run_conv(r, c1);
    }
    return rc;
}

bool bneck_fused(int nb) { return nb >= ec_config().rn50_bneck; }

int run_bneck(const Run& r, const Op& o) {
    const ec_rn50* h = r.h;
    const Conv &c1 = o.c1, &c2 = o.c2, &c3 = o.c3;
    if (bneck_fused(r.nb) && o.fold_c1)
        return ec_bneck_conv123_bf16(r.buf(c3.res), h->wbneck + o.wpack_off, h->bias + c1.at.b, h->bias + c2.at.b, h->bias + c3.at.b,
                                     r.buf(c3.dst), r.nb, c3.H, c3.W, c2.Cin, r.stream);
    if (bneck_fused(r.nb))
        return ec_bneck_conv23_bf16(r.buf(c2.src), h->wbneck + o.wpack_off, h->bias + c2.at.b, h->bias + c3.at.b, r.buf(c3.res),
                                    r.buf(c3.dst), r.nb, c3.H, c3.W, c2.Cin, r.stream);
    int rc = o.fold_c1 ? run_conv(r, c1) : EC_OK;
    if (rc == EC_OK) rc = run_conv(r, c2);
    return rc == EC_OK ? run_conv(r, c3) : rc;
}

bool btail_fused(const Op& o, int nb) { return o.c2.Cout <= 128 || (o.c2.Cout <= 256 && nb <= 32); }

int run_btail(const Run& r, const Op& o) {
    const Conv &c2 = o.c2, &ds = o.ds;
    if (btail_fused(o, r.nb))
        return ec_basic_tail_s2_bf16(r.buf(c2.src), r.buf(ds.src), r.h->wbneck + o.cat.w_off, r.h->bias_cat + o.cat.b_off, r.buf(c2.dst), r.nb,
                                     c2.H, c2.W, c2.Cin, ds.Cin, c2.Cout, r.stream);
    const int rc = run_conv(r, ds);
    return rc == EC_OK ? run_conv(r, c2) : rc;
}

bool rgbd_joint(int ) { return ec_config().rgbd_joint != 0; }

int rn50_run(const ec_rn50_t* h, const FrameIn& in, int batch, void* workspace, size_t ws_bytes, void* feat, int chunk,
             ec_stream_t stream_main) {
    const bool rgbd = in.kind == FrameIn::RGBD;
    if (!h || !in.p || !workspace || !feat || (rgbd && !in.depth)) return EC_ERR_ARG;
    if (batch <= 0) return EC_ERR_SHAPE;
    if ((in.kind == FrameIn::DEPTH || rgbd) && (h->ops.empty() || h->ops.front().kind != OP_STEM1))
        return EC_ERR_UNSUPPORTED;
    if (chunk <= 0 || chunk > batch) chunk = batch;
    const int per = rgbd ? 2 : 1;
    {
        const long maxc = ((1L << 31) - 1) / (long)(h->max_elems_per_frame * 2) / per;
        if (chunk > maxc) chunk = (int)(maxc > 0 ? maxc : 1);
    }
    if (ws_bytes < (rgbd ? ec_rn50_rgbd_workspace_bytes(h, chunk) : ec_rn50_workspace_bytes(h, chunk))) return EC_ERR_WORKSPACE;
    const ec_min_tiles_scope mint_scope(h->conv8_min_tiles);
    const size_t bufsz = align_up(h->max_elems_per_frame * 2 * (size_t)chunk * per, 256);
    const size_t frame_bytes = (size_t)h->res * h->res * (in.kind == FrameIn::DEPTH ? 1 : 3) * (in.u8() ? 1 : 4);
    const size_t out_stride = (size_t)h->out_sp * h->out_sp * h->out_c;
    const hipStream_t stream = (hipStream_t)stream_main;
    auto pass = [&](Run r) -> int {
        for (const Op& o : h->ops) {
            int rc;
            switch (o.kind) {
                case OP_STEM1:
                case OP_STEM7: rc = run_stem(r, o); break;
                case OP_POOL: rc = run_pool(r, o); break;
                case OP_PAIR: rc = run_pair(r, o); break;
                case OP_BNECK: rc = run_bneck(r, o); break;
                case OP_BTAIL: rc = run_btail(r, o); break;
                case OP_CAT: rc = run_cat(r, o); break;
                case OP_CONV_POOLOUT: rc = run_conv_poolout(r, o); break;
                default: rc = run_conv(r, o.c);
            }
            if (rc != EC_OK) return rc;
        }
        return EC_OK;
    };
    unsigned char* const base = (unsigned char*)workspace;
    for (int b0 = 0; b0 < batch; b0 += chunk) {
        const int nb = std::min(chunk, batch - b0);
        const void* frames = (const unsigned char*)in.p + (size_t)b0 * frame_bytes;
        int rc;
        if (!rgbd) {
            const bool d = in.kind == FrameIn::DEPTH;
            rc = pass(Run{h, in, d ? nullptr : frames, d ? (const float*)frames : nullptr, nb, base, bufsz,
                          (uint16_t*)feat + (size_t)b0 * out_stride, stream, false});
        } else {
            const float* dep = in.depth + (size_t)b0 * h->res * h->res;
            uint16_t* map = (uint16_t*)(base + NBUF * bufsz);
            if (rgbd_joint(nb)) {
                rc = pass(Run{h, in, frames, dep, 2 * nb, base, bufsz, map, stream, false});
            } else {
                rc = pass(Run{h, in, frames, nullptr, nb, base, bufsz, map, stream, false});
                if (rc == EC_OK) rc = pass(Run{h, in, nullptr, dep, nb, base, bufsz, map + (size_t)nb * out_stride, stream, false});
            }
            if (rc == EC_OK)
                rc = ec_spatial_mean_pair_bf16(map, map + (size_t)nb * out_stride, (float*)feat + (size_t)b0 * h->out_c, nb,
                                               h->out_sp * h->out_sp, h->out_c, stream_main);
        }
        if (rc != EC_OK) return rc;
    }
    return EC_OK;
}
}

extern "C" size_t ec_rn50_rgbd_workspace_bytes(const ec_rn50_t* h, int pairs) {
    if (!h || pairs <= 0) return 0;
    const size_t map = (size_t)2 * pairs * h->out_sp * h->out_sp * h->out_c * sizeof(uint16_t);
    return ec_rn50_workspace_bytes(h, 2 * pairs) + align_up(map, 256);
}

extern "C" int ec_rn50_embed_rgbd(const ec_rn50_t* h, const void* rgb, int rgb_u8, const float* h_mean3, const float* h_std3,
                                  const float* depth, float scale, float shift, const float* stem_w9, int pairs, void* workspace,
                                  size_t ws_bytes, float* embed, int chunk, ec_stream_t stream) {
    if (!depth || !stem_w9 || (rgb_u8 && (!h_mean3 || !h_std3))) return EC_ERR_ARG;
    FrameIn in{FrameIn::RGBD, rgb, h_mean3, h_std3, scale, shift, stem_w9};
    in.depth = depth;
    in.rgb_u8 = rgb_u8 != 0;
    return rn50_run(h, in, pairs, workspace, ws_bytes, embed, chunk, stream);
}

extern "C" int ec_rn50_forward(const ec_rn50_t* h, const float* rgb, int batch, void* workspace, size_t ws_bytes,
                               void* feat, int chunk, ec_stream_t stream) {
    return rn50_run(h, FrameIn{FrameIn::F32, rgb, nullptr, nullptr, 1.f, 0.f, nullptr}, batch, workspace, ws_bytes, feat, chunk, stream);
}

extern "C" int ec_rn50_forward_u8(const ec_rn50_t* h, const uint8_t* rgb_u8, const float* h_mean3, const float* h_std3, int batch,
                                  void* workspace, size_t ws_bytes, void* feat, int chunk, ec_stream_t stream) {
    if (!h_mean3 || !h_std3) return EC_ERR_ARG;
    return rn50_run(h, FrameIn{FrameIn::U8, rgb_u8, h_mean3, h_std3, 1.f, 0.f, nullptr}, batch, workspace, ws_bytes, feat, chunk, stream);
}

extern "C" int ec_rn50_forward_depth(const ec_rn50_t* h, const float* depth, float scale, float shift, const float* stem_w9,
                                     int batch, void* workspace, size_t ws_bytes, void* feat, int chunk, ec_stream_t stream) {
    if (!stem_w9) return EC_ERR_ARG;
    return rn50_run(h, FrameIn{FrameIn::DEPTH, depth, nullptr, nullptr, scale, shift, stem_w9}, batch, workspace, ws_bytes, feat, chunk, stream);
}
```

embodied_clip_amd/encoder.py:

```python
from __future__ import annotations

import ctypes as C
from typing import Dict, List, Optional, Tuple

import torch

from . import _lib

BN_EPS = 1e-5


def _fold(w: torch.Tensor, sd: Dict[str, torch.Tensor], bn: str) -> Tuple[torch.Tensor, torch.Tensor]:
    g, b = sd[bn + ".weight"].float(), sd[bn + ".bias"].float()
    mu, var = sd[bn + ".running_mean"].float(), sd[bn + ".running_var"].float()
    s = g / torch.sqrt(var + BN_EPS)
    return w.float() * s.view(-1, 1, 1, 1), b - mu * s


def _layers(sd) -> List[int]:
    out = []
    for li in range(1, 5):
        n = 0
        while f"layer{li}.{n}.conv1.weight" in sd:
            n += 1
        out.append(n)
    return out


def pack_rn50(sd: Dict[str, torch.Tensor]):
    sd = {k[len("visual."):] if k.startswith("visual.") else k: v.detach().cpu() for k, v in sd.items()}
    width = sd["conv3.weight"].shape[0]
    layers = _layers(sd)
    ws: List[torch.Tensor] = []
    bs: List[torch.Tensor] = []

    def add(conv, bn, keep_f32=False):
        w, b = _fold(sd[conv + ".weight"], sd, bn)
        bs.append(b)
        w = w.permute(0, 2, 3, 1).contiguous()
        if keep_f32:
            return w
        ws.append(w.reshape(-1).to(torch.bfloat16))
        return None

    sc_real = sd["conv1.weight"].shape[0]
    sc = (sc_real + 31) // 32 * 32

    def pad_out(w, b):
        if w.shape[0] == sc:
            return w, b
        return (torch.cat([w, w.new_zeros((sc - w.shape[0],) + tuple(w.shape[1:]))]), torch.cat([b, b.new_zeros(sc - b.shape[0])]))

    def pad_in(w):
        if w.shape[3] == sc:
            return w
        return torch.cat([w, w.new_zeros(tuple(w.shape[:3]) + (sc - w.shape[3],))], dim=3)

    w1, b1 = _fold(sd["conv1.weight"], sd, "bn1")
    w1, b1 = pad_out(w1.permute(0, 2, 3, 1).contiguous(), b1)
    bs.append(b1)
    stem_w = w1.reshape(sc, 27).t().contiguous()
    w2, b2 = _fold(sd["conv2.weight"], sd, "bn2")
    w2, b2 = pad_out(pad_in(w2.permute(0, 2, 3, 1).contiguous()), b2)
    bs.append(b2)
    ws.append(w2.reshape(-1).to(torch.bfloat16))
    w3, b3 = _fold(sd["conv3.weight"], sd, "bn3")
    bs.append(b3)
    ws.append(pad_in(w3.permute(0, 2, 3, 1).contiguous()).reshape(-1).to(torch.bfloat16))
    for li, n in enumerate(layers, start=1):
        for b in range(n):
            p = f"layer{li}.{b}"
            add(p + ".conv1", p + ".bn1")
            add(p + ".conv2", p + ".bn2")
            add(p + ".conv3", p + ".bn3")
            if (p + ".downsample.0.weight") in sd:
                add(p + ".downsample.0", p + ".downsample.1")
    return (width, layers), stem_w, torch.cat(ws), torch.cat(bs)


def fold_stem_depth(stem_w: torch.Tensor) -> torch.Tensor:
    w = stem_w.detach().to("cpu", torch.float32)
    assert w.dim() == 2 and w.shape[0] == 27, tuple(w.shape)
    return w.view(9, 3, w.shape[1]).sum(dim=1).contiguous()


class ClipResizeCrop:

    def __init__(self, device="cuda", n_px: int = 224):
        self.lib = _lib.load()
        self.device = torch.device(device)
        self.n_px = n_px
        self._tables: Dict[Tuple[int, int], Tuple[torch.Tensor, int]] = {}

    def table(self, H: int, W: int) -> Tuple[torch.Tensor, int]:
        n = self.lib.ec_clip_resize_table_ints(H, W, self.n_px)
        if n == 0:
            raise _lib.EcError(f"unsupported frame geometry {H}x{W} -> {self.n_px}")
        t = torch.empty(n, dtype=torch.int32)
        _lib.check(self.lib.ec_clip_resize_table(H, W, self.n_px, t.data_ptr(), n), "ec_clip_resize_table")
        return t, int(t[6])

    @_lib.on_device
    def __call__(self, frames_u8: torch.Tensor, out: Optional[torch.Tensor] = None) -> torch.Tensor:
        assert frames_u8.is_cuda and frames_u8.dtype == torch.uint8 and frames_u8.is_contiguous() and frames_u8.shape[3] == 3
        B, H, W, _ = frames_u8.shape
        if (H, W) not in self._tables:
            t, rows = self.table(H, W)
            self._tables[(H, W)] = (t.to(self.device), rows)
        tab, rows = self._tables[(H, W)]
        if out is None:
            out = torch.empty((B, self.n_px, self.n_px, 3), dtype=torch.uint8, device=self.device)
        _lib.check(self.lib.ec_clip_resize_crop_u8(frames_u8.data_ptr(), tab.data_ptr(), rows, out.data_ptr(), B, H, W,
                                                   self.n_px, _lib.stream_ptr()), "ec_clip_resize_crop_u8")
        return out


class RN50Trunk:

    def __init__(self, state_dict: Dict[str, torch.Tensor], device="cuda", input_resolution: int = 224,
                 chunk: int = 0, weights_from: Optional["RN50Trunk"] = None):
        self.lib = _lib.load()
        self.device = torch.device(device)
        if weights_from is not None:
            assert weights_from.device == self.device and weights_from.input_resolution == input_resolution
            width, layers = weights_from._arch
            self.stem_w, self.w, self.bias = weights_from.stem_w, weights_from.w, weights_from.bias
            self.stem_w9 = weights_from.stem_w9
        else:
            (width, layers), stem_w, w, bias = self._pack(state_dict)
            self.stem_w = stem_w.to(self.device)
            self.stem_w9 = fold_stem_depth(stem_w).to(self.device) if stem_w.dtype == torch.float32 and stem_w.shape[0] == 27 else None
            self.w = w.to(self.device)
            self.bias = bias.to(self.device)
        self._arch = (width, layers)
        self.input_resolution = input_resolution
        self.chunk = chunk
        self.h = self._create(width, layers, input_resolution)
        self.out_channels = self.lib.ec_rn50_out_channels(self.h)
        self.out_spatial = self.lib.ec_rn50_out_spatial(self.h)
        self._ws: Optional[torch.Tensor] = None
        self._ws_rgbd: Optional[torch.Tensor] = None
        self._resize: Optional[ClipResizeCrop] = None

    _pack = staticmethod(pack_rn50)

    def _create(self, width, layers, input_resolution):
        h = C.c_void_p()
        arr = (C.c_int * 4)(*layers)
        _lib.check(self.lib.ec_rn50_create(C.byref(h), width, arr, input_resolution, self.stem_w.data_ptr(),
                                           self.w.data_ptr(), self.w.numel(), self.bias.data_ptr(),
                                           self.bias.numel()), "ec_rn50_create")
        return h

    def __del__(self):
        try:
            if getattr(self, "h", None):
                self.lib.ec_rn50_destroy(self.h)
                self.h = None
        except Exception:
            pass

    def plan_hash(self) -> str:
        return f"{self.lib.ec_rn50_plan_hash(self.h):016x}"

    def set_conv8_min_tiles(self, n: int) -> None:
        _lib.check(self.lib.ec_rn50_set_conv8_min_tiles(self.h, int(n)), "ec_rn50_set_conv8_min_tiles")

    def _workspace(self, n: int) -> torch.Tensor:
        need = self.lib.ec_rn50_workspace_bytes(self.h, n)
        if self._ws is None or self._ws.numel() < need:
            self._ws = torch.empty(need, dtype=torch.uint8, device=self.device)
        return self._ws

    @_lib.on_device
    def forward(self, rgb: torch.Tensor, out: Optional[torch.Tensor] = None) -> torch.Tensor:
        assert rgb.is_cuda and rgb.dtype == torch.float32 and rgb.is_contiguous()
        B, R, R2, c3 = rgb.shape
        assert R == self.input_resolution and R2 == R and c3 == 3, rgb.shape
        S, Cc = self.out_spatial, self.out_channels
        if out is None:
            out = torch.empty((B, S, S, Cc), dtype=torch.bfloat16, device=self.device)
        assert out.is_contiguous() and out.dtype == torch.bfloat16 and out.numel() == B * S * S * Cc
        chunk = self.chunk if self.chunk > 0 else B
        ws = self._workspace(min(chunk, B))
        _lib.check(self.lib.ec_rn50_forward(self.h, rgb.data_ptr(), B, ws.data_ptr(), ws.numel(), out.data_ptr(),
                                            chunk, _lib.stream_ptr()), "ec_rn50_forward")
        return out

    @_lib.on_device
    def forward_u8(self, rgb_u8: torch.Tensor, out: Optional[torch.Tensor] = None,
                   mean=(0.48145466, 0.4578275, 0.40821073), std=(0.26862954, 0.26130258, 0.27577711)) -> torch.Tensor:
        assert rgb_u8.is_cuda and rgb_u8.dtype == torch.uint8 and rgb_u8.is_contiguous() and rgb_u8.shape[3] == 3
        if rgb_u8.shape[1] != self.input_resolution or rgb_u8.shape[2] != self.input_resolution:
            if self._resize is None:
                self._resize = ClipResizeCrop(self.device, self.input_resolution)
            rgb_u8 = self._resize(rgb_u8)
        B, R = rgb_u8.shape[0], rgb_u8.shape[1]
        S, Cc = self.out_spatial, self.out_channels
        if out is None:
            out = torch.empty((B, S, S, Cc), dtype=torch.bfloat16, device=self.device)
        chunk = self.chunk if self.chunk > 0 else B
        ws = self._workspace(min(chunk, B))
        m3, s3 = (C.c_float * 3)(*mean), (C.c_float * 3)(*std)
        _lib.check(self.lib.ec_rn50_forward_u8(self.h, rgb_u8.data_ptr(), m3, s3, B, ws.data_ptr(), ws.numel(),
                                               out.data_ptr(), chunk, _lib.stream_ptr()), "ec_rn50_forward_u8")
        return out

    @_lib.on_device
    def forward_depth(self, depth: torch.Tensor, out: Optional[torch.Tensor] = None, scale: float = 1.0,
                      shift: float = 0.0) -> torch.Tensor:
        assert depth.is_cuda and depth.dtype == torch.float32 and depth.is_contiguous()
        assert depth.dim() in (3, 4) and (depth.dim() == 3 or depth.shape[3] == 1), depth.shape
        B, R, R2 = depth.shape[:3]
        assert R == self.input_resolution and R2 == R, depth.shape
        if self.stem_w9 is None:
            raise _lib.EcError("forward_depth: this tower has no one-channel stem (CLIP ModifiedResNet towers only)")
        S, Cc = self.out_spatial, self.out_channels
        if out is None:
            out = torch.empty((B, S, S, Cc), dtype=torch.bfloat16, device=self.device)
        assert out.is_contiguous() and out.dtype == torch.bfloat16 and out.numel() == B * S * S * Cc
        chunk = self.chunk if self.chunk > 0 else B
        ws = self._workspace(min(chunk, B))
        _lib.check(self.lib.ec_rn50_forward_depth(self.h, depth.data_ptr(), float(scale), float(shift), self.stem_w9.data_ptr(),
                                                  B, ws.data_ptr(), ws.numel(), out.data_ptr(), chunk, _lib.stream_ptr()),
                   "ec_rn50_forward_depth")
        return out

    @_lib.on_device
    def embed_rgbd(self, rgb: torch.Tensor, depth: torch.Tensor, out: Optional[torch.Tensor] = None, scale: float = 1.0,
                   shift: float = 0.0, mean=(0.48145466, 0.4578275, 0.40821073),
                   std=(0.26862954, 0.26130258, 0.27577711)) -> torch.Tensor:
        assert rgb.is_cuda and rgb.dtype in (torch.float32, torch.uint8) and rgb.is_contiguous()
        assert depth.is_cuda and depth.dtype == torch.float32 and depth.is_contiguous()
        assert depth.dim() in (3, 4) and (depth.dim() == 3 or depth.shape[3] == 1), depth.shape
        B, R, R2 = depth.shape[:3]
        assert R == self.input_resolution and R2 == R, depth.shape
        assert tuple(rgb.shape) == (B, R, R, 3), (rgb.shape, depth.shape)
        if self.stem_w9 is None:
            raise _lib.EcError("embed_rgbd: this tower has no one-channel stem (CLIP ModifiedResNet towers only)")
        Cc = self.out_channels
        if out is None:
            out = torch.empty((B, Cc), dtype=torch.float32, device=self.device)
        assert out.is_contiguous() and out.dtype == torch.float32 and out.numel() == B * Cc
        chunk = self.chunk if self.chunk > 0 else B
        need = self.lib.ec_rn50_rgbd_workspace_bytes(self.h, min(chunk, B))
        if self._ws_rgbd is None or self._ws_rgbd.numel() < need:
            self._ws_rgbd = torch.empty(need, dtype=torch.uint8, device=self.device)
        ws = self._ws_rgbd
        u8 = rgb.dtype == torch.uint8
        m3, s3 = ((C.c_float * 3)(*mean), (C.c_float * 3)(*std)) if u8 else (None, None)
        _lib.check(self.lib.ec_rn50_embed_rgbd(self.h, rgb.data_ptr(), int(u8), m3, s3, depth.data_ptr(), float(scale), float(shift),
                                               self.stem_w9.data_ptr(), B, ws.data_ptr(), ws.numel(), out.data_ptr(), chunk,
                                               _lib.stream_ptr()), "ec_rn50_embed_rgbd")
        return out

    @_lib.on_device
    def to_nchw_f32(self, feat: torch.Tensor, out: Optional[torch.Tensor] = None) -> torch.Tensor:
        B = feat.shape[0]
        S, Cc = self.out_spatial, self.out_channels
        o = out if out is not None else torch.empty((B, Cc, S, S), dtype=torch.float32, device=self.device)
        assert o.is_contiguous() and o.dtype == torch.float32 and o.numel() == B * Cc * S * S
        _lib.check(self.lib.ec_nhwc_bf16_to_nchw_f32(feat.data_ptr(), o.data_ptr(), B, S * S, Cc, _lib.stream_ptr()),
                   "ec_nhwc_bf16_to_nchw_f32")
        if out is not None and not torch.is_inference(o):
            o.view(-1)[:0].zero_()
        return o

    @_lib.on_device
    def spatial_mean(self, feat: torch.Tensor) -> torch.Tensor:
        B = feat.shape[0]
        S, Cc = self.out_spatial, self.out_channels
        o = torch.empty((B, Cc), dtype=torch.float32, device=self.device)
        _lib.check(self.lib.ec_spatial_mean_bf16(feat.data_ptr(), o.data_ptr(), B, S * S, Cc, _lib.stream_ptr()),
                   "ec_spatial_mean_bf16")
        return o


IMAGENET_RGB_MEANS = (0.485, 0.456, 0.406)
IMAGENET_RGB_STDS = (0.229, 0.224, 0.225)
TV_STEM_KROW, TV_STEM_K = 24, 176


def pack_tv_resnet(sd: Dict[str, torch.Tensor]):
    sd = {k: v.detach().cpu() for k, v in sd.items()}
    width = sd["conv1.weight"].shape[0]
    assert tuple(sd["conv1.weight"].shape[1:]) == (3, 7, 7), "not a torchvision ResNet state dict"
    layers = _layers(sd)
    w1, b1 = _fold(sd["conv1.weight"], sd, "bn1")
    rows = w1.permute(0, 2, 3, 1).reshape(width, 7, 21)
    stem = torch.zeros(width, TV_STEM_K)
    stem[:, :7 * TV_STEM_KROW].view(width, 7, TV_STEM_KROW)[:, :, :21] = rows
    ws: List[torch.Tensor] = []
    bs: List[torch.Tensor] = [b1]
    for li, n in enumerate(layers, start=1):
        for b in range(n):
            p = f"layer{li}.{b}"
            for conv, bn in ((".conv1", ".bn1"), (".conv2", ".bn2"), (".conv3", ".bn3"), (".downsample.0", ".downsample.1")):
                if (p + conv + ".weight") not in sd:
                    continue
                w, bb = _fold(sd[p + conv + ".weight"], sd, p + bn)
                bs.append(bb)
                ws.append(w.permute(0, 2, 3, 1).reshape(-1).to(torch.bfloat16))
    return (width, layers), stem.to(torch.bfloat16).contiguous(), torch.cat(ws), torch.cat(bs)


class ImageNetRN50Trunk(RN50Trunk):

    _pack = staticmethod(pack_tv_resnet)

    def _create(self, width, layers, input_resolution):
        if width != 64:
            raise _lib.EcError("ec_rn50tv_create: the 7x7 stem kernel is built for 64 channels (torchvision resnet50/101/152)")
        h = C.c_void_p()
        arr = (C.c_int * 4)(*layers)
        _lib.check(self.lib.ec_rn50tv_create(C.byref(h), arr, input_resolution, self.stem_w.data_ptr(), self.w.data_ptr(),
                                             self.w.numel(), self.bias.data_ptr(), self.bias.numel()), "ec_rn50tv_create")
        return h

    def forward_u8(self, rgb_u8, out=None, mean=IMAGENET_RGB_MEANS, std=IMAGENET_RGB_STDS):
# ... 176 lines not shown


@_guard_first
def conv_bf16(x, w, bias, res=None, ksize=1, pool=False, act=1, out=None):
    lib = _lib.load()
    B, H, W, Cin = x.shape
    Cout = w.shape[0]
    Ho, Wo = (H // 2, W // 2) if pool else (H, W)
    if out is None:
        out = torch.empty((B, Ho, Wo, Cout), dtype=torch.bfloat16, device=x.device)
    ld = _row_stride(out, (B, Ho, Wo, Cout))
    _lib.check(lib.ec_conv_bf16_ld(x.data_ptr(), w.data_ptr(), _lib.ptr(bias), _lib.ptr(res), out.data_ptr(), B, H, W,
                                   Cin, Cout, ksize, int(pool), act, ld, _lib.stream_ptr()), "ec_conv_bf16_ld")
    return out


def _row_stride(out, shape) -> int:
    assert tuple(out.shape) == tuple(shape) and out.dtype == torch.bfloat16, (out.shape, shape, out.dtype)
    B, H, W, C = shape
    ld = out.stride(2)
    assert out.stride(3) == 1 and ld >= C and out.stride(1) == W * ld and (B == 1 or out.stride(0) == H * W * ld), out.stride()
    return ld


@_guard_first
def avgpool2_bf16(x, out=None):
    lib = _lib.load()
    B, H, W, C = x.shape
    if out is None:
        out = torch.empty((B, H // 2, W // 2, C), dtype=torch.bfloat16, device=x.device)
    ld = _row_stride(out, (B, H // 2, W // 2, C))
    _lib.check(lib.ec_avgpool2_bf16_ld(x.data_ptr(), out.data_ptr(), B, H, W, C, ld, _lib.stream_ptr()), "ec_avgpool2_bf16_ld")
    return out


@_guard_first
def conv_bf16_s2(x, w, bias, res=None, ksize=1, act=1, out=None):
    lib = _lib.load()
    B, H, W, Cin = x.shape
    Cout = w.shape[0]
    if out is None:
        out = torch.empty((B, H // 2, W // 2, Cout), dtype=torch.bfloat16, device=x.device)
    _lib.check(lib.ec_conv_bf16_s2(x.data_ptr(), w.data_ptr(), _lib.ptr(bias), _lib.ptr(res), out.data_ptr(), B, H, W, Cin, Cout,
                                   ksize, act, _lib.stream_ptr()), "ec_conv_bf16_s2")
    return out


@_guard_first
def stem7_pool(rgb, stem_w, bias, mean=None, std=None):
    lib = _lib.load()
    B, H, W, _ = rgb.shape
    u8 = rgb.dtype == torch.uint8
    out = torch.empty((B, H // 4, W // 4, 64), dtype=torch.bfloat16, device=rgb.device)
    m3 = (C.c_float * 3)(*(mean or (0.0, 0.0, 0.0)))
    s3 = (C.c_float * 3)(*(std or (1.0, 1.0, 1.0)))
    _lib.check(lib.ec_stem7_pool(rgb.data_ptr(), int(u8), m3, s3, stem_w.data_ptr(), bias.data_ptr(), out.data_ptr(), B, H, W,
                                 _lib.stream_ptr()), "ec_stem7_pool")
    return out


@_guard_first
def bneck_conv23_bf16(c1, w2, b2, w3, b3, x, out=None):
    lib = _lib.load()
    B, H, W, C = c1.shape
    if out is None:
        out = torch.empty_like(x)
    packed = bneck_pack_weights(w2, w3)
    _lib.check(lib.ec_bneck_conv23_bf16(c1.data_ptr(), packed.data_ptr(), b2.data_ptr(), b3.data_ptr(), x.data_ptr(),
                                        out.data_ptr(), B, H, W, C, _lib.stream_ptr()), "ec_bneck_conv23_bf16")
    return out


@_guard_first
def conv3x3_img_bf16(x, w, bias, out=None, pool=False):
    lib = _lib.load()
    B, H, W, C = x.shape
    packed = _packed_lookup("img", (w,))
    if packed is None:
        packed = torch.empty_like(w)
        _lib.check(lib.ec_conv3x3_img_pack(w.data_ptr(), packed.data_ptr(), C, _lib.stream_ptr()), "ec_conv3x3_img_pack")
        _packed_store("img", (w,), packed)
    if out is None:
        out = torch.empty((B, H // 2, W // 2, C), dtype=x.dtype, device=x.device) if pool else torch.empty_like(x)
    ld = _row_stride(out, (B, H // 2, W // 2, C) if pool else (B, H, W, C))
    _lib.check(lib.ec_conv3x3_img_bf16_ld(x.data_ptr(), packed.data_ptr(), bias.data_ptr(), out.data_ptr(), B, H, W, C, int(pool),
                                          ld, _lib.stream_ptr()), "ec_conv3x3_img_bf16_ld")
    return out


@_guard_first
def bneck_conv123_bf16(x, w1, b1, w2, b2, w3, b3, out=None):
    lib = _lib.load()
    B, H, W, C4 = x.shape
    C = C4 // 4
    packed = _packed_lookup("bneck3", (w1, w2, w3))
    if packed is None:
        packed = torch.empty(lib.ec_bneck3_packed_elems(C), dtype=torch.bfloat16, device=x.device)
        _lib.check(lib.ec_bneck3_pack_weights(w1.data_ptr(), w2.data_ptr(), w3.data_ptr(), packed.data_ptr(), C, _lib.stream_ptr()),
                   "ec_bneck3_pack_weights")
        _packed_store("bneck3", (w1, w2, w3), packed)
    if out is None:
        out = torch.empty_like(x)
    _lib.check(lib.ec_bneck_conv123_bf16(x.data_ptr(), packed.data_ptr(), b1.data_ptr(), b2.data_ptr(), b3.data_ptr(), out.data_ptr(),
                                         B, H, W, C, _lib.stream_ptr()), "ec_bneck_conv123_bf16")
    return out


_BNECK_PACKED = {}


def _packed_lookup(tag, tensors):
    import weakref
    hit = _BNECK_PACKED.get((tag,) + tuple(id(t) for t in tensors))
    if hit is None:
        return None
    refs, versions, packed = hit
    if all(r() is t for r, t in zip(refs, tensors)) and versions == tuple(t._version for t in tensors):
        return packed
    return None


def _packed_store(tag, tensors, packed):
    import weakref
    if len(_BNECK_PACKED) > 32:
        _BNECK_PACKED.clear()
    _BNECK_PACKED[(tag,) + tuple(id(t) for t in tensors)] = (tuple(weakref.ref(t) for t in tensors),
                                                           tuple(t._version for t in tensors), packed)


def bneck_pack_weights(w2, w3):
    hit = _packed_lookup("bneck", (w2, w3))
    if hit is not None:
        return hit
    lib = _lib.load()
    C = w3.shape[1]
    packed = torch.empty(lib.ec_bneck_packed_elems(C), dtype=torch.bfloat16, device=w2.device)
    _lib.check(lib.ec_bneck_pack_weights(w2.data_ptr(), w3.data_ptr(), packed.data_ptr(), C, _lib.stream_ptr()), "ec_bneck_pack_weights")
    _packed_store("bneck", (w2, w3), packed)
    return packed


@_guard_first
def gemm_bf16(a, w, bias=None, res=None, act=0):
    lib = _lib.load()
    M, K = a.shape
    N = w.shape[0]
    out = torch.empty((M, N), dtype=torch.bfloat16, device=a.device)
    _lib.check(lib.ec_gemm_bf16(a.data_ptr(), w.data_ptr(), _lib.ptr(bias), _lib.ptr(res), out.data_ptr(), M, N, K,
                                act, _lib.stream_ptr()), "ec_gemm_bf16")
    return out


@_guard_first
def conv1x1_pair_bf16(a0, w0, b0, w2, b2, a1=None, w1=None, b1=None, res=None):
    lib = _lib.load()
    M, K0 = a0.shape
    N, N2 = w0.shape[0], w2.shape[0]
    y = torch.empty((M, N), dtype=torch.bfloat16, device=a0.device)
    z = torch.empty((M, N2), dtype=torch.bfloat16, device=a0.device)
    _lib.check(lib.ec_conv1x1_pair_bf16(a0.data_ptr(), w0.data_ptr(), b0.data_ptr(), _lib.ptr(a1), _lib.ptr(w1),
                                        _lib.ptr(b1), _lib.ptr(res), y.data_ptr(), w2.data_ptr(), b2.data_ptr(),
                                        z.data_ptr(), M, K0, N, N2, _lib.stream_ptr()), "ec_conv1x1_pair_bf16")
    return y, z


def pack_text(sd: Dict[str, torch.Tensor]):
    sd = {k: v.detach().cpu().float() for k, v in sd.items()}
    vocab, D = sd["token_embedding.weight"].shape
    ctx = sd["positional_embedding"].shape[0]
    E = sd["text_projection"].shape[1]
    n = 0
    while f"transformer.resblocks.{n}.ln_1.weight" in sd:
        n += 1
    ws, fs = [], [sd["token_embedding.weight"].reshape(-1), sd["positional_embedding"].reshape(-1)]
    for i in range(n):
        p = f"transformer.resblocks.{i}."
        ws += [sd[p + "attn.in_proj_weight"], sd[p + "attn.out_proj.weight"], sd[p + "mlp.c_fc.weight"],
               sd[p + "mlp.c_proj.weight"]]
        fs += [sd[p + "ln_1.weight"], sd[p + "ln_1.bias"], sd[p + "attn.in_proj_bias"], sd[p + "attn.out_proj.bias"],
               sd[p + "ln_2.weight"], sd[p + "ln_2.bias"], sd[p + "mlp.c_fc.bias"], sd[p + "mlp.c_proj.bias"]]
    ws.append(sd["text_projection"].t().contiguous())
    fs += [sd["ln_final.weight"], sd["ln_final.bias"]]
    w = torch.cat([t.reshape(-1) for t in ws]).to(torch.bfloat16)
    f = torch.cat([t.reshape(-1) for t in fs]).float()
    return dict(width=D, layers=n, context_length=ctx, vocab_size=vocab, embed_dim=E), w, f


class ClipTextEncoder:

    def __init__(self, state_dict, device="cuda", heads: Optional[int] = None):
        self.lib = _lib.load()
        self.device = torch.device(device)
        cfg, w, f = pack_text(state_dict)
        self.cfg = cfg
        self.w, self.f = w.to(self.device), f.to(self.device)
        heads = cfg["width"] // 64 if heads is None else heads
        h = C.c_void_p()
        _lib.check(self.lib.ec_text_create(C.byref(h), cfg["width"], cfg["layers"], heads, cfg["context_length"],
                                           cfg["vocab_size"], cfg["embed_dim"], self.w.data_ptr(), self.w.numel(),
                                           self.f.data_ptr(), self.f.numel()), "ec_text_create")
        self.h = h
        self._ws = None

    def __del__(self):
        try:
            if getattr(self, "h", None):
                self.lib.ec_text_destroy(self.h)
                self.h = None
        except Exception:
            pass

    @_lib.on_device
    @torch.no_grad()
    def encode_text(self, tokens: torch.Tensor) -> torch.Tensor:
        assert tokens.dim() == 2 and tokens.shape[1] == self.cfg["context_length"], tokens.shape
        t = tokens.to(self.device, torch.int32).contiguous()
        B = t.shape[0]
        need = self.lib.ec_text_workspace_bytes(self.h, B)
        if self._ws is None or self._ws.numel() < need:
            self._ws = torch.empty(need, dtype=torch.uint8, device=self.device)
        out = torch.empty((B, self.cfg["embed_dim"]), dtype=torch.float32, device=self.device)
        _lib.check(self.lib.ec_text_forward(self.h, t.data_ptr(), B, self._ws.data_ptr(), self._ws.numel(),
                                            out.data_ptr(), _lib.stream_ptr()), "ec_text_forward")
        return out

    def goal_table(self, goal_tokens: torch.Tensor, normalize: bool = True) -> torch.Tensor:
        e = self.encode_text(goal_tokens)
        return e / e.norm(dim=-1, keepdim=True) if normalize else e


@_guard_first
def conv1x1_pair_pool_bf16(a0, w0, b0, res, w2, b2):
    lib = _lib.load()
    B, H, W, K0 = a0.shape
    N, N2 = w0.shape[0], w2.shape[0]
    y = torch.empty((B, H, W, N), dtype=torch.bfloat16, device=a0.device)
    yp = torch.empty((B, H // 2, W // 2, N), dtype=torch.bfloat16, device=a0.device)
    z = torch.empty((B, H, W, N2), dtype=torch.bfloat16, device=a0.device)
    _lib.check(lib.ec_conv1x1_pair_pool_bf16(a0.data_ptr(), w0.data_ptr(), b0.data_ptr(), res.data_ptr(), y.data_ptr(),
                                             yp.data_ptr(), w2.data_ptr(), b2.data_ptr(), z.data_ptr(), B, H, W, K0, N,
                                             N2, _lib.stream_ptr()), "ec_conv1x1_pair_pool_bf16")
    return y, yp, z
```

embodied_clip_amd/engine.py:

```python
from __future__ import annotations

from collections import OrderedDict
from typing import Dict, List, Optional

import os
import random

import torch

from . import _lib
from . import synthetic as syn
from .dist import (allreduce_flat, check_job_seed, collective_active, gather_actor_counts, global_minibatch_sizes,
                   minibatch_bounds)
from .episodes import EpisodeTracker, NavEpisodeTracker, nav_env_tensors
from .encoder import AttentionPool, ClipTextEncoder, ImageNetBasicTrunk, ImageNetRN50Trunk, RN50Trunk, ViTEmbedder
from .policy import PolicyHandle
from .imitation import imitation_loss_raw, imitation_scratch
from .ppo import PPO_NARROW_MAX_A, FlatAdam, linear_decay_lr, ppo_loss_raw, ppo_wide_scratch

IMAGENET_ENCODERS = {
    "imagenet_rn18": ((2, 2, 2, 2), "basic", ImageNetBasicTrunk),
    "imagenet_rn34": ((3, 4, 6, 3), "basic", ImageNetBasicTrunk),
    "imagenet_rn50": ((3, 4, 6, 3), "bottleneck", ImageNetRN50Trunk),
}
# ... 159 lines not shown
                             f"(rnn_type={getattr(policy, 'rnn_type', 'GRU')!r})")


class _SlicedActor:
    depth = False

    @property
    def dual(self) -> bool:
        return self.depth and not self.pooled_net
    prev_action_dims = 0
    prev_action_null = 0
    rnn_type = "GRU"
    rnn_layers = 1
    hidden_size = 512
    pooled_net = False
    pooling = None
    net_sensors = ()
    goal_ids = True

    _embed = None

    def _goal(self, t: int, rs):
        return self.env.goals[t][rs] if (self.goal_ids or not self.pooled_net) else None

    def _side(self, t: int, rs):
        return {"sensors": self.env.sensors[t][rs]} if self.net_sensors else {}

    def _build_model(self, n_actors, encoder, encoder_sd, policy_sd, encoder_chunk, encoder_streams):
        self.encoder = encoder
        self._embed = "attnpool" if self.zeroshot else self.pooling
        two_min = int(os.environ.get("EC_TWO_SLICE_MIN", "48"))
        ns = encoder_streams if (encoder_streams > 1 and n_actors >= two_min and n_actors % encoder_streams == 0) else 1
        self.ns = ns
        d = self.dev
        pools = [None] * ns
        if encoder in ("rn50", "rn50x16"):
            sd = encoder_sd if encoder_sd is not None else (
                syn.rn50_visual_state_dict(0) if encoder == "rn50" else
                syn.rn50_visual_state_dict(0, width=96, layers=(6, 8, 18, 8), output_dim=768, heads=48))
            share = os.environ.get("EC_SHARE_WEIGHTS", "1") != "0"
            encs = [RN50Trunk(sd, device=d, chunk=encoder_chunk)]
            encs += [RN50Trunk(sd, device=d, chunk=encoder_chunk, weights_from=encs[0] if share else None) for _ in range(ns - 1)]
            self.S, self.C = encs[0].out_spatial, encs[0].out_channels
            if self._embed == "attnpool":
                pools = [AttentionPool(sd, device=d)]
                pools += [AttentionPool(sd, device=d, weights_from=pools[0] if share else None) for _ in range(ns - 1)]
                self.trunk_S, self.trunk_C = self.S, self.C
                self.S, self.C = 1, pools[0].out_dim
        elif encoder in IMAGENET_ENCODERS:
            layers, block, cls = IMAGENET_ENCODERS[encoder]
            sd = encoder_sd if encoder_sd is not None else syn.tv_resnet_state_dict(0, layers=layers, block=block)
            share = os.environ.get("EC_SHARE_WEIGHTS", "1") != "0"
            encs = [cls(sd, device=d, chunk=encoder_chunk)]
            encs += [cls(sd, device=d, chunk=encoder_chunk, weights_from=encs[0] if share else None) for _ in range(ns - 1)]
            self.S, self.C = encs[0].out_spatial, encs[0].out_channels
        elif encoder == "vit":
            sd = encoder_sd if encoder_sd is not None else syn.vit_visual_state_dict(0)
            share = os.environ.get("EC_SHARE_WEIGHTS", "1") != "0"
            encs = [ViTEmbedder(sd, device=d)]
            encs += [ViTEmbedder(sd, device=d, weights_from=encs[0] if share else None) for _ in range(ns - 1)]
            self.S, self.C = 7, encs[0].D
        else:
            raise ValueError(encoder)
        if self._embed == "avgpool":
            self.trunk_S, self.trunk_C = self.S, self.C
            self.S = 1
        if self.pooled_net:
            self.policy = PolicyHandle.pooled(self.C, hidden=self.hidden_size, num_goals=12 if self.goal_ids else 0, sensors=self.net_sensors,
                                              num_actions=self._num_actions, prev_action_dims=self.prev_action_dims,
                                              prev_action_null=self.prev_action_null, rnn_type=self.rnn_type, rnn_layers=self.rnn_layers)
            if policy_sd is not None:
                check_model_tensors(self.policy, policy_sd, getattr(self, "_checkpoint", None) or "policy_sd")
            self.H, self.A, self.SW = self.policy.H, self.policy.A, self.policy.state_width
            self.params = self.policy.flatten(policy_sd if policy_sd is not None
                                              else syn.policy_state_dict(0, pooled=self.policy.pooled_cfg), d)
            return encs, pools
        pkw = dict(in_channels=self.C, spatial=self.S, num_actions=self._num_actions)
        if self.goal_in:
            pkw["goal_in"] = self.goal_in
        if self.dual:
            pkw["dual"] = 1
        if self.zeroshot:
            assert encoder == "rn50", "the zero-shot variant uses the CLIP-RN50 image embedding"
            pkw["fusion"] = 1
        if self.prev_action_dims:
            pkw.update(prev_action_dims=self.prev_action_dims, prev_action_null=self.prev_action_null)
        if self.hidden_size != 512:
            pkw["hidden"] = self.hidden_size
        self.policy = PolicyHandle(rnn_type=self.rnn_type, rnn_layers=self.rnn_layers, **pkw)
        if policy_sd is not None:
            check_model_tensors(self.policy, policy_sd, getattr(self, "_checkpoint", None) or "policy_sd")
        if self.zeroshot:
            tsd = self._text_sd if self._text_sd is not None else syn.text_state_dict(0)
            tok = self._goal_tokens if self._goal_tokens is not None else syn.synthetic_tokens(
                7, 12, context_length=tsd["positional_embedding"].shape[0], vocab_size=tsd["token_embedding.weight"].shape[0])
            self.goal_table = ClipTextEncoder(tsd, device=d).goal_table(tok).contiguous()
            self.policy.set_goal_table(self.goal_table)
        self.H, self.A = self.policy.H, self.policy.A
        self.SW = self.policy.state_width
        self.params = self.policy.flatten(policy_sd if policy_sd is not None
                                          else syn.policy_state_dict(0, **pkw, rnn_type=self.rnn_type, rnn_layers=self.rnn_layers), d)
        return encs, pools

    def _build_slices(self, n_actors, encs, pools, feat_steps, n_comm, frames_host):
        ns, d, encoder = self.ns, self.dev, self.encoder
        n = n_actors // ns
        S2 = self.S * self.S
        self.slices: List[_Slice] = []
        n_own = ns if ns > 1 else 0
        n_copy = ns if frames_host else 0
        plain = lambda k: [torch.cuda.Stream(device=d) for _ in range(k)]
        pool = None
        for take_comm, take_copy in ((n_comm, n_copy), (n_comm, 0), (0, 0)):
            want = n_own + take_comm + take_copy
            try:
                pool = (_lib.concurrent_streams(want, d) if want > 1 else plain(want))
            except RuntimeError:
                if take_comm == 0 and take_copy == 0:
                    raise
                continue
            if (take_comm, take_copy) != (n_comm, n_copy):
                import warnings
                warnings.warn(f"{n_own + n_comm + n_copy} streams exceed the runtime's hardware queues: only {want} are verified concurrent")
            pool = pool + plain(n_comm - take_comm + n_copy - take_copy)
            order = ["own"] * n_own + ["comm"] * take_comm + ["copy"] * take_copy + ["comm"] * (n_comm - take_comm) + ["copy"] * (n_copy - take_copy)
            break
        by = lambda kind: [s_ for s_, k_ in zip(pool, order) if k_ == kind]
        slice_streams = by("own") if n_own else [None]
        copy_streams = by("copy")
        self.comm_stream = by("comm")[0] if n_comm else None
        for i in range(ns):
            sl = _Slice()
            sl.o, sl.n, sl.enc, sl.pool = i * n, n, encs[i], pools[i]
            sl.stream = slice_streams[i]
            sl.feat = torch.empty((feat_steps, n, S2, self.C), dtype=torch.float32 if self._embed else torch.bfloat16, device=d)
            sl.feat2 = torch.empty_like(sl.feat) if self.dual else None
            sl.trunk_out = (torch.empty((n, self.trunk_S, self.trunk_S, self.trunk_C), dtype=torch.bfloat16, device=d)
                            if self._embed and not self.depth else None)
            sl.tok = (torch.empty((n, encs[i].L, encs[i].D), dtype=torch.bfloat16, device=d) if encoder == "vit" else None)
            sl.ws_act = torch.empty(self.policy.workspace_bytes(1, n, False), dtype=torch.uint8, device=d)
            sl.act_tables_valid = False
            if frames_host:
                fshape = (n,) + tuple(self.env.frames.shape[2:])
                sl.stage = [torch.empty(fshape, dtype=self.env.frames.dtype, device=d) for _ in range(2)]
                sl.copy_stream = copy_streams[i]
                sl.copied = [torch.cuda.Event() for _ in range(2)]
                sl.consumed = [None, None]
                sl.k = 0
            self.slices.append(sl)
        self.encode_frames = n
        self._conv8_min_tiles = (50 if n >= 128 else (75 if n >= 64 else 0)) if ns == 2 else 0
        for e in encs:
            e.set_conv8_min_tiles(self._conv8_min_tiles)
        fused = os.environ.get("EC_ACT_FUSED_SAMPLE", "1") != "0"
        self._act_fused = fused and self.A + 1 <= 8
        self._act_wide = fused and 8 < self.A + 1 <= 257 and self.H <= 3576
        self.trunk_events: List = []
        self.time_trunk = False

    @property
    def feat(self) -> torch.Tensor:
        return self.slices[0].feat if self.ns == 1 else torch.cat([sl.feat for sl in self.slices], dim=1)

    @property
    def feat2(self) -> Optional[torch.Tensor]:
        if not self.dual:
            return None
        return self.slices[0].feat2 if self.ns == 1 else torch.cat([sl.feat2 for sl in self.slices], dim=1)

    def _f2(self, sl, t: int):
        return sl.feat2[t] if self.dual else None

    def _observe(self, actions_host=None):
        rgb = self.env.observe(actions_host) if actions_host is not None else self.env.observe()
        return rgb, (self.env.observe_depth() if self.depth else None)

    @property
    def enc_streams(self):
        return [sl.stream for sl in self.slices if sl.stream is not None]

    def _on(self, sl):
        return torch.cuda.stream(sl.stream) if sl.stream is not None else _NullCtx()

    def _fork(self):
        if self.ns > 1:
            cur = torch.cuda.current_stream()
            for sl in self.slices:
                sl.stream.wait_stream(cur)

    def _join(self):
        if self.ns > 1:
            cur = torch.cuda.current_stream()
            for sl in self.slices:
                cur.wait_stream(sl.stream)

    def _encode_slice(self, sl, rgb: torch.Tensor, t: int, dep: Optional[torch.Tensor] = None):
        src = rgb[sl.o:sl.o + sl.n]
        if self.env.host:
            i = sl.k & 1
            sl.k += 1
            cur = torch.cuda.current_stream()
            with torch.cuda.stream(sl.copy_stream):
                if sl.consumed[i] is not None:
                    sl.copy_stream.wait_event(sl.consumed[i])
                sl.stage[i].copy_(src, non_blocking=True)
                sl.copied[i].record(sl.copy_stream)
            cur.wait_event(sl.copied[i])
            src = sl.stage[i]
        timed = self.time_trunk
        if timed:
            e0, e1 = torch.cuda.Event(enable_timing=True), torch.cuda.Event(enable_timing=True)
            e0.record(torch.cuda.current_stream())
        if self._embed and self.depth:
            sl.enc.embed_rgbd(src, dep[sl.o:sl.o + sl.n], sl.feat[t].view(sl.n, self.C))
        elif self._embed:
            (sl.enc.forward_u8 if src.dtype == torch.uint8 else sl.enc.forward)(src, sl.trunk_out)
            if self._embed == "attnpool":
                sl.pool.forward(sl.trunk_out, sl.feat[t].view(sl.n, self.C))
            else:
                _lib.check(self.lib.ec_spatial_mean_bf16(sl.trunk_out.data_ptr(), sl.feat[t].data_ptr(), sl.n, self.trunk_S * self.trunk_S,
                                                         self.trunk_C, _lib.stream_ptr()), "ec_spatial_mean_bf16")
        elif self.encoder in ("rn50", "rn50x16") or self.encoder in IMAGENET_ENCODERS:
            (sl.enc.forward_u8 if src.dtype == torch.uint8 else sl.enc.forward)(src, sl.feat[t])
            if self.dual:
                sl.enc.forward_depth(dep[sl.o:sl.o + sl.n], sl.feat2[t])
        else:
            sl.enc.forward(src, sl.tok)
            sl.feat[t].copy_(sl.tok[:, 1:, :])
        if timed:
            e1.record(torch.cuda.current_stream())
            self.trunk_events.append((e0, e1))
        if self.env.host:
            ev = torch.cuda.Event()
            ev.record(torch.cuda.current_stream())
            sl.consumed[i] = ev

    def invalidate_act_tables(self):
        for sl in self.slices:
            sl.act_tables_valid = False

    def set_params(self, flat: torch.Tensor):
        self.params.copy_(flat.to(self.params.device, self.params.dtype).view_as(self.params))
        self.invalidate_act_tables()


class Worker(_SlicedActor):

    def __init__(self, n_actors: int, T: int = 128, device="cuda:0", seed: int = 0, rank: int = 0, world: int = 1,
                 update_repeats: int = 4, lr: float = 3e-4, max_grad_norm: float = 0.5, gamma: float = 0.99,
                 tau: float = 0.95, encoder_sd=None, policy_sd=None, lr_total_steps: int = 300_000_000,
                 encoder_chunk: int = 0, encoder: str = "rn50", encoder_streams: int = 2, frames_u8: bool = False,
                 frames_host: bool = False, zeroshot: bool = False, text_sd=None, goal_tokens=None,
                 num_mini_batch: int = 1, sync_actions: bool = False, force_allreduce: bool = False,
                 overlap_allreduce: bool = True, goal_in: int = 0, num_actions: int = 6, track_episodes: bool = False,
                 nav_metrics: bool = False, depth: bool = False, loss: str = "ppo", il_weight: float = 1.0,
                 teacher_forcing=None, prev_actions: int = 0, prev_action_null_token: bool = True, rnn_type: str = "GRU",
                 rnn_layers: int = 1, hidden: int = 512, net: str = "goal_encoder", pooling: str = "attnpool", sensors=(),
                 goal_ids: bool = True):
        self.pooled_net, self.pooling, self.net_sensors = check_net(net, pooling, sensors, goal_ids, encoder, bool(depth), bool(zeroshot), goal_in)
        self.goal_ids = bool(goal_ids)
        if depth:
            check_rgbd(encoder, zeroshot, goal_in, frames_host)
        two_tower = bool(depth) and not self.pooled_net
        self.prev_action_dims = check_prev_actions(prev_actions, two_tower, bool(zeroshot))
        self.prev_action_null = int(bool(prev_action_null_token)) if self.prev_action_dims else 0
        self.rnn_type = check_rnn_type(rnn_type, two_tower, bool(zeroshot))
        self.rnn_layers = check_rnn_layers(rnn_layers, two_tower, bool(zeroshot))
        self.hidden_size = int(hidden)
        self.depth = bool(depth)
        self.lib = _lib.load()
        self.zeroshot, self._text_sd, self._goal_tokens = zeroshot, text_sd, goal_tokens
        assert not (goal_in and zeroshot), "coordinate goals go through the goal encoder, not the zero-shot fusion"
        self.goal_in, self._num_actions = goal_in, num_actions
        self.track_episodes = track_episodes
        if nav_metrics and not track_episodes:
            raise ValueError("Worker(nav_metrics=True) needs track_episodes=True")
        self.nav_metrics = nav_metrics
        if loss not in ("ppo", "imitation", "ppo+imitation"):
            raise ValueError(f"Worker(loss={loss!r}): one of 'ppo', 'imitation', 'ppo+imitation'")
        if teacher_forcing is not None and not callable(teacher_forcing):
            raise ValueError("Worker(teacher_forcing=...): None or a callable of total_steps")
        self.loss_mode, self.il_weight, self.teacher_forcing = loss, float(il_weight), teacher_forcing
        self._ppo, self._il = loss != "imitation", loss != "ppo"
        self._tf_p = 0.0
        self.sync_actions = sync_actions
        self.force_allreduce = force_allreduce
        self.overlap_allreduce = overlap_allreduce
        assert 1 <= num_mini_batch <= n_actors, "num_mini_batch must not exceed the number of samplers"
        self.num_mini_batch = num_mini_batch
        self._mb_rng = random.Random(seed)
        self.dev = self.device = torch.device(device)
        if self.dev.index is None:
            self.dev = self.device = torch.device("cuda", torch.cuda.current_device())
        check_job_seed(seed, world, device=self.dev)
        self.shard_counts = gather_actor_counts(n_actors, world, device=self.dev)
        assert all(num_mini_batch <= c for c in self.shard_counts), "num_mini_batch must not exceed the smallest shard"
        self._mb_global = global_minibatch_sizes(self.shard_counts, num_mini_batch)
        self._init(n_actors, T, seed, rank, world, update_repeats, lr, max_grad_norm, gamma, tau, encoder_sd, policy_sd,
                   lr_total_steps, encoder_chunk, encoder, encoder_streams, frames_u8, frames_host)

    @_lib.on_device
    def _init(self, n_actors, T, seed, rank, world, update_repeats, lr, max_grad_norm, gamma, tau, encoder_sd, policy_sd,
              lr_total_steps, encoder_chunk, encoder, encoder_streams, frames_u8, frames_host=False):
        self.N, self.T, self.rank, self.world = n_actors, T, rank, world
        self.update_repeats, self.gamma, self.tau = update_repeats, gamma, tau
        self.base_lr, self.lr_total_steps = lr, lr_total_steps
# ... 429 lines not shown
```

include/ec_amd.h:

```cpp
#ifndef EC_AMD_H
#define EC_AMD_H

#include <stddef.h>
#include <stdint.h>

#ifdef __cplusplus
extern "C" {
#endif

typedef void* ec_stream_t;
typedef void* ec_event_t;

enum {
    EC_OK = 0,
    EC_ERR_ARG = -1,
    EC_ERR_SHAPE = -2,
    EC_ERR_LAUNCH = -3,
    EC_ERR_WORKSPACE = -4,
    EC_ERR_ALLOC = -5,
    EC_ERR_UNSUPPORTED = -6
};

enum { EC_ACT_NONE = 0, EC_ACT_RELU = 1, EC_ACT_QUICKGELU = 2 };

int ec_version(void);
const char* ec_strerror(int code);

int ec_bind_streams(ec_stream_t* streams, int n, int spin_us);
int ec_stream_pair_overlap(ec_stream_t a, ec_stream_t b, int spin_us, float* ratio);


int ec_conv_bf16(const void* in, const void* w, const float* bias, const void* res, void* out,
                 int B, int H, int W, int Cin, int Cout, int ksize, int pool, int act,
                 ec_stream_t stream);
int ec_conv_bf16_ld(const void* in, const void* w, const float* bias, const void* res, void* out,
                    int B, int H, int W, int Cin, int Cout, int ksize, int pool, int act, int out_row_stride,
                    ec_stream_t stream);
int ec_gemm_bf16(const void* A, const void* W, const float* bias, const void* res, void* out,
                 int M, int N, int K, int act, ec_stream_t stream);

int ec_mha_bf16(const void* qkv, void* out, int B, int L, int D, int heads, int causal, ec_stream_t stream);
int ec_layernorm_bf16(const void* x, const float* gamma, const float* beta, void* out, long rows, int D, ec_stream_t stream);
int ec_vit_assemble_bf16(const void* pemb, const float* cls, const float* pos, const float* gamma, const float* beta, void* out,
                         float* stats_or_null, int B, int L, int D, ec_stream_t stream);
int ec_row_stats_bf16(const void* x, float* stats, long rows, int D, ec_stream_t stream);
int ec_ln_fold_bf16(const void* W, const float* gamma, const float* beta, const float* b, void* Wg, float* s, float* c, int N,
                    int K, ec_stream_t stream);
int ec_gemm_bf16_ln(const void* A, const void* Wt, const float* bias, const void* res, void* out, int M, int N, int K, int act,
                    const float* ln_s, const float* ln_stats, int ln_np, float* stats_out, int* np_out, ec_stream_t stream);

size_t ec_clip_resize_table_ints(int H, int W, int n_px);
int ec_clip_resize_table(int H, int W, int n_px, int* host_table, size_t n_ints);
int ec_clip_resize_crop_u8(const uint8_t* frames_u8, const int* table_dev, int table_max_rows, uint8_t* out_u8, int B,
                           int H, int W, int n_px, ec_stream_t stream);

int ec_semantic_labels_u8(const uint8_t* sem_u8, const uint8_t* colors_u8, int64_t* presence, int64_t* localization,
                          int B, int H, int W, int C, ec_stream_t stream);


int ec_split3_bf16(const float* W, void* planes, long rows, int K, ec_stream_t stream);
int ec_gemm_bf16a_x3(const void* A_bf16, const void* W_planes, const float* bias, float* out, long M, int N, int K,
                     int act, ec_stream_t stream);

int ec_dw_tn_x3_splits(long M, int NX);
int ec_dw_tn_x3(const void* dY_planes, const void* X_bf16, float* part, float* dW, long M, int NX, ec_stream_t stream);

int ec_stem_conv1(const float* rgb_nhwc, const float* w, const float* bias, void* out,
                  int B, int H, int W, int Cout, ec_stream_t stream);

int ec_stem_conv1_depth(const float* depth, float scale, float shift, const float* w9, const float* bias, void* out,
                        int B, int H, int W, int Cout, ec_stream_t stream);

int ec_conv1x1_pair_bf16(const void* a0, const void* w0, const float* b0, const void* a1, const void* w1,
                         const float* b1, const void* res, void* y, const void* w2, const float* b2, void* z,
                         long M, int K0, int N, int N2, ec_stream_t stream);

int ec_conv1x1_pair_pool_bf16(const void* a0, const void* w0, const float* b0, const void* res, void* y,
                              void* y_pooled, const void* w2, const float* b2, void* z, int B, int H, int W, int K0,
                              int N, int N2, ec_stream_t stream);

int ec_stem_conv1_u8(const uint8_t* rgb_u8_nhwc, const float* h_mean3, const float* h_std3, const float* w,
                     const float* bias, void* out, int B, int H, int W, int Cout, ec_stream_t stream);

size_t ec_bneck_packed_elems(int C);
int ec_bneck_pack_weights(const void* w2, const void* w3, void* packed, int C, ec_stream_t stream);
int ec_bneck_conv23_bf16(const void* c1, const void* packed, const float* b2, const float* b3,
                         const void* x, void* y, int B, int H, int W, int C, ec_stream_t stream);

size_t ec_bneck3_packed_elems(int C);
int ec_bneck3_pack_weights(const void* w1, const void* w2, const void* w3, void* packed, int C, ec_stream_t stream);
int ec_bneck_conv123_bf16(const void* x, const void* packed, const float* b1, const float* b2, const float* b3,
                          void* y, int B, int H, int W, int C, ec_stream_t stream);

int ec_conv3x3_img_pack(const void* w, void* packed, int C, ec_stream_t stream);
int ec_conv3x3_img_bf16(const void* in, const void* packed, const float* bias, void* out, int B, int H, int W, int C,
                        int pool, ec_stream_t stream);
int ec_conv3x3_img_bf16_ld(const void* in, const void* packed, const float* bias, void* out, int B, int H, int W, int C,
                           int pool, int out_row_stride, ec_stream_t stream);

int ec_conv_bf16_s2(const void* in, const void* w, const float* bias, const void* res, void* out, int B, int H, int W,
                    int Cin, int Cout, int ksize, int act, ec_stream_t stream);
int ec_basic_tail_s2_bf16(const void* c1, const void* x, const void* w_cat, const float* bias_cat, void* out, int B, int Ho,
                          int Wo, int planes, int inplanes, int Cout, ec_stream_t stream);
int ec_stem7_pool(const void* rgb, int u8, const float* h_mean3, const float* h_std3, const void* w, const float* bias,
                  void* out, int B, int H, int W, ec_stream_t stream);

int ec_avgpool2_bf16(const void* in, void* out, int B, int H, int W, int C, ec_stream_t stream);
int ec_avgpool2_bf16_ld(const void* in, void* out, int B, int H, int W, int C, int out_row_stride, ec_stream_t stream);

int ec_nhwc_bf16_to_nchw_f32(const void* in, float* out, int B, int HW, int C, ec_stream_t stream);
int ec_nchw_f32_to_nhwc_bf16(const float* in, void* out, int B, int HW, int C, int* inexact, ec_stream_t stream);

int ec_spatial_mean_bf16(const void* in, float* out, int B, int HW, int C, ec_stream_t stream);
int ec_spatial_mean_pair_bf16(const void* a, const void* b, float* out, int B, int HW, int C, ec_stream_t stream);

typedef struct ec_rn50 ec_rn50_t;

int ec_rn50_create(ec_rn50_t** out, int width, const int* layers4, int input_resolution,
                   const float* stem_w_f32, const void* w_bf16, size_t n_w, const float* bias, size_t n_bias);
int ec_rn50tv_create(ec_rn50_t** out, const int* layers4, int input_resolution, const void* stem_w_bf16,
                     const void* w_bf16, size_t n_w, const float* bias, size_t n_bias);
int ec_tvresnet_basic_create(ec_rn50_t** out, const int* layers4, int input_resolution, const void* stem_w_bf16,
                             const void* w_bf16, size_t n_w, const float* bias, size_t n_bias);
void ec_rn50_destroy(ec_rn50_t* h);
size_t ec_rn50_workspace_bytes(const ec_rn50_t* h, int batch);
int ec_rn50_out_channels(const ec_rn50_t* h);
int ec_rn50_out_spatial(const ec_rn50_t* h);
int ec_rn50_forward(const ec_rn50_t* h, const float* rgb_nhwc, int batch, void* workspace, size_t ws_bytes,
                    void* feat_bf16_nhwc, int chunk, ec_stream_t stream);
int ec_rn50_forward_u8(const ec_rn50_t* h, const uint8_t* rgb_u8_nhwc, const float* h_mean3, const float* h_std3,
                       int batch, void* workspace, size_t ws_bytes, void* feat_bf16_nhwc, int chunk,
                       ec_stream_t stream);
int ec_rn50_forward_depth(const ec_rn50_t* h, const float* depth, float scale, float shift, const float* stem_w9, int batch,
                          void* workspace, size_t ws_bytes, void* feat_bf16_nhwc, int chunk, ec_stream_t stream);
size_t ec_rn50_rgbd_workspace_bytes(const ec_rn50_t* h, int pairs);
int ec_rn50_embed_rgbd(const ec_rn50_t* h, const void* rgb, int rgb_u8, const float* h_mean3, const float* h_std3,
                       const float* depth, float scale, float shift, const float* stem_w9, int pairs, void* workspace,
                       size_t ws_bytes, float* embed, int chunk, ec_stream_t stream);
int ec_rn50_num_ops(const ec_rn50_t* h);
uint64_t ec_rn50_plan_hash(const ec_rn50_t* h);
int ec_rn50_set_conv8_min_tiles(ec_rn50_t* h, int n);


enum {
    EC_GEMM_A_BF16 = 1,
    EC_GEMM_B_BF16 = 2,
    EC_GEMM_RELU = 4,
    EC_GEMM_ACCUMULATE = 8,
    EC_GEMM_SPLIT_PARTS = 16,
    EC_GEMM_3PRODUCTS = 32
};
int ec_gemm_f32(const void* A, const void* B, float* C, int M, int N, int K, long sam, long sak, long sbk, long sbn,
                int ldc, int flags, const float* bias, const float* gbias, const int* gidx, int group,
                const float* dmask, const float* rowscale, int splitk, ec_stream_t stream);

typedef struct {
    int in_channels;
    int spatial;
    int hidden;
    int goal_dims;
    int num_goals;
    int num_actions;
    int compress_hid;
    int compress_out;
    int comb_hid;
    int comb_out;
    int fusion;
    int dual;
    int goal_in;
    int prev_action_dims;
    int prev_action_null;
} ec_policy_cfg;
typedef struct ec_policy ec_policy_t;

int ec_policy_create(ec_policy_t** out, const ec_policy_cfg* cfg);
enum { EC_RNN_GRU = 0, EC_RNN_LSTM = 1 };
int ec_policy_create_rnn(ec_policy_t** out, const ec_policy_cfg* cfg, int rnn_type);
int ec_policy_rnn_type(const ec_policy_t* h);
int ec_policy_state_width(const ec_policy_t* h);
#define EC_RNN_MAX_LAYERS 4
int ec_policy_create_rnn_layers(ec_policy_t** out, const ec_policy_cfg* cfg, int rnn_type, int num_layers);
int ec_policy_rnn_layers(const ec_policy_t* h);
int ec_policy_set_goal_table(ec_policy_t* h, const float* table);
void ec_policy_destroy(ec_policy_t* h);
int ec_policy_num_param_tensors(const ec_policy_t* h);
size_t ec_policy_flat_size(const ec_policy_t* h);
int ec_policy_param_offset(const ec_policy_t* h, int idx, size_t* off, size_t* numel);
size_t ec_policy_workspace_bytes(const ec_policy_t* h, int T, int N, int for_backward);
enum { EC_POLICY_INFER = 0, EC_POLICY_LEARN = 1, EC_POLICY_INFER_REUSE = 2 };
int ec_policy_forward(const ec_policy_t* h, const float* params, const void* feat, int feat_bf16,
                      const int64_t* goal, const float* h0, const float* masks, int T, int N,
                      void* workspace, size_t ws_bytes, int for_backward, float* hv, float* h_final, ec_stream_t stream);
int ec_policy_forward2(const ec_policy_t* h, const float* params, const void* feat, const void* feat2, int feat_bf16,
                       const int64_t* goal, const float* h0, const float* masks, int T, int N,
                       void* workspace, size_t ws_bytes, int for_backward, float* hv, float* h_final, ec_stream_t stream);
int ec_policy_act(const ec_policy_t* h, const float* params, const void* feat, const void* feat2, int feat_bf16,
                  const int64_t* goal, const float* h0, const float* masks, int N, void* workspace, size_t ws_bytes,
                  int reuse_tables, float* hv, float* h_final, int64_t* actions, float* logp, float* values,
                  uint64_t seed, uint64_t step, int first_actor, ec_stream_t stream);
int ec_policy_forward_vec(const ec_policy_t* h, const float* params, const void* feat, const void* feat2, int feat_bf16,
                          const float* goal_vec, const float* h0, const float* masks, int T, int N,
                          void* workspace, size_t ws_bytes, int for_backward, float* hv, float* h_final, ec_stream_t stream);
int ec_policy_act_vec(const ec_policy_t* h, const float* params, const void* feat, const void* feat2, int feat_bf16,
                      const float* goal_vec, const float* h0, const float* masks, int N, void* workspace, size_t ws_bytes,
                      int reuse_tables, float* hv, float* h_final, int64_t* actions, float* logp, float* values,
                      uint64_t seed, uint64_t step, int first_actor, ec_stream_t stream);
int ec_policy_act_greedy(const ec_policy_t* h, const float* params, const void* feat, const void* feat2, int feat_bf16,
                         const int64_t* goal, const float* h0, const float* masks, int N, void* workspace, size_t ws_bytes,
                         int reuse_tables, float* hv, float* h_final, int64_t* actions, float* logp, float* values,
                         ec_stream_t stream);
int ec_policy_act_vec_greedy(const ec_policy_t* h, const float* params, const void* feat, const void* feat2, int feat_bf16,
                             const float* goal_vec, const float* h0, const float* masks, int N, void* workspace, size_t ws_bytes,
                             int reuse_tables, float* hv, float* h_final, int64_t* actions, float* logp, float* values,
                             ec_stream_t stream);
int ec_policy_backward(const ec_policy_t* h, const float* params, const void* feat, int feat_bf16,
                       const float* masks, int T, int N, void* workspace, size_t ws_bytes, const float* dhv,
                       const float* dh_final, float* grads, ec_stream_t stream);
int ec_policy_backward2(const ec_policy_t* h, const float* params, const void* feat, const void* feat2, int feat_bf16,
                        const float* masks, int T, int N, void* workspace, size_t ws_bytes, const float* dhv,
                        const float* dh_final, float* grads, ec_stream_t stream);
int ec_policy_backward3(const ec_policy_t* h, const float* params, const void* feat, const void* feat2, int feat_bf16,
                        const float* masks, int T, int N, void* workspace, size_t ws_bytes, const float* dhv,
                        const float* dh_final, float* grads, ec_event_t recurrent_grads_ready, ec_stream_t stream);

int ec_lstm_step_fwd(const float* a_in, const float* whh, const float* bhh, const float* state_prev, long ld_prev,
                     const float* mask, float* h_out, long ld_h, float* c_out, long ld_c, float* gates, int N, int H,
                     ec_stream_t stream);
int ec_lstm_step_bwd(const float* dhs, const float* gates, const float* c, const float* c_prev, const float* mask,
                     const float* whh, const float* whhT, const float* da_next, const float* mask_next, float* carry_h,
                     float* carry_c, float* da, int N, int H, ec_stream_t stream);

int ec_rnn_stack_step_fwd(int rnn_type, const float* x, long ld_x, const float* wih, const float* whh, const float* bih,
                          const float* bhh, const float* state_prev, long ld_prev, const float* mask, float* h_out, long ld_h,
                          float* c_out, long ld_c, float* h_out2, long ld_h2, int N, int H, ec_stream_t stream);

int ec_gae(const float* rewards, const float* values, const float* masks, float* returns, float* adv,
           float* norm_adv, double* stats2, int T, int N, float gamma, float tau, float eps, ec_stream_t stream);
int ec_ppo_loss(const float* hv, const int64_t* actions, const float* old_logp, const float* old_values,
                const float* returns, const float* norm_adv, float* dhv, double* sums4, long B, int A,
                float clip, float vcoef, float ecoef, float grad_scale, ec_stream_t stream);
int ec_ppo_loss_ex(const float* hv, const int64_t* actions, const float* old_logp, const float* old_values,
                   const float* returns, const float* norm_adv, float* dhv, double* sums4, long B, int A,
                   float clip, float value_clip, float vcoef, float ecoef, float grad_scale, ec_stream_t stream);
int ec_sample_actions(const float* hv, int64_t* actions, float* logp, float* values, int N, int A,
                      uint64_t seed, uint64_t step, int first_actor, ec_stream_t stream);
int ec_mode_actions(const float* hv, int64_t* actions, float* logp, float* values, int N, int A, ec_stream_t stream);
int ec_episode_stats(const float* rewards, const float* masks, const float* success, float* carry_ret, int32_t* carry_len,
                     double* totals5, float* rec_f, int32_t* rec_i, int cap, int32_t* n_records, int T, int N,
                     ec_stream_t stream);
int ec_nav_episode_stats(const float* rewards, const float* masks, const float* success, const float* step_dist,
                         const float* start_dist, const float* goal_dist, const int64_t* category, int C, float* carry_ret,
                         int32_t* carry_len, float* carry_path, double* totals, float* rec_f, int32_t* rec_i, int cap,
                         int32_t* n_records, int T, int N, ec_stream_t stream);
int ec_clip_adam_scratch_doubles(void);
int ec_clip_adam_step(float* params, const float* grads, float* exp_avg, float* exp_avg_sq, double* sumsq1,
                      long n, float max_grad_norm, float lr, float beta1, float beta2, float eps, int step,
                      ec_stream_t stream);

int ec_imitation_scratch_doubles(void);
int ec_imitation_loss(const float* hv, const int64_t* expert_actions, const float* expert_mask, const double* denom,
                      float* dhv, double* sums3, double* scratch, long B, int A, float weight, float grad_scale,
                      int accumulate, ec_stream_t stream);
int ec_expert_count(const float* expert_mask, int T, int N, int n0, int n1, double* out, ec_stream_t stream);
int ec_teacher_force(const float* hv, const int64_t* expert_actions, const float* expert_mask, float p, int64_t* actions,
                     float* logp, int N, int A, uint64_t seed, uint64_t step, int first_actor, ec_stream_t stream);

int ec_heads_wide(const float* hs, const float* Wa, const float* ba, const float* wc, const float* bc, float* hv, long B, int H,
                  int A, int64_t* actions, float* logp, float* values, int greedy, uint64_t seed, uint64_t step,
                  int first_actor, const int64_t* expert_actions, const float* expert_mask, float force_p, ec_stream_t stream);
int ec_policy_act_ex(const ec_policy_t* h, const float* params, const void* feat, const void* feat2, int feat_bf16,
                     const int64_t* goal, const float* goal_vec, const float* h0, const float* masks, int N, void* workspace,
                     size_t ws_bytes, int reuse_tables, float* hv, float* h_final, int64_t* actions, float* logp, float* values,
                     int greedy, uint64_t seed, uint64_t step, int first_actor, const int64_t* expert_actions,
                     const float* expert_mask, float force_p, ec_stream_t stream);
int ec_ppo_loss_wide_scratch_doubles(void);
int ec_ppo_loss_wide(const float* hv, const int64_t* actions, const float* old_logp, const float* old_values,
                     const float* returns, const float* norm_adv, float* dhv, double* sums4, double* scratch, long B, int A,
                     float clip, float value_clip, float vcoef, float ecoef, float grad_scale, ec_stream_t stream);

int ec_prev_action_table(const float* emb, const float* w, long ld, int col0, float* pt, int A, int null_token, int G, int E,
                         ec_stream_t stream);
int ec_prev_action_add(float* gi, const float* pt, const int64_t* prev_actions, const float* masks, int null_token, int A, long B,
                       int G, ec_stream_t stream);
size_t ec_prev_action_grad_scratch_floats(long B, int G, int A, int null_token);
int ec_prev_action_grad(const float* dgi, const int64_t* prev_actions, const float* masks, int null_token, int A, const float* emb,
                        const float* w, long ld, int col0, float* demb, float* dw, float* scratch, long B, int G, int E,
                        ec_stream_t stream);
int ec_policy_forward_pa(const ec_policy_t* h, const float* params, const void* feat, const void* feat2, int feat_bf16,
                         const int64_t* goal, const float* goal_vec, const int64_t* prev_actions, const float* h0,
                         const float* masks, int T, int N, void* workspace, size_t ws_bytes, int for_backward, float* hv,
                         float* h_final, ec_stream_t stream);
int ec_policy_act_pa(const ec_policy_t* h, const float* params, const void* feat, const void* feat2, int feat_bf16,
                     const int64_t* goal, const float* goal_vec, const int64_t* prev_actions, const float* h0, const float* masks,
                     int N, void* workspace, size_t ws_bytes, int reuse_tables, float* hv, float* h_final, int64_t* actions,
// ... 66 lines not shown
```

Before: 64480.

## Recompute layer1 block-0 residual in next pair kernel instead of storing it

Adds a rebuild kernel for the first two layer1 bottleneck blocks of the RN50 tower. The block-0 output is no longer written to memory; the next block recomputes it from the block-0 conv3 and downsample inputs (two K=64 GEMMs) and then applies its own conv3 plus the following conv1. The existing pair kernel can now skip the y store, and its bias reads in the epilogues now go through the pipelined LDS stream helper, which is shared via a new header. This trades extra MFMA work and LDS pressure for less HBM traffic on the large layer1 activations, and the engine enables it by default for rn50.

```diff
diff --git a/embodied_clip_amd/_lib.py b/embodied_clip_amd/_lib.py
--- a/embodied_clip_amd/_lib.py
+++ b/embodied_clip_amd/_lib.py
@@ -64,6 +64,7 @@
     "ec_rn50_num_ops": (c_int, [c_void_p]),
     "ec_rn50_plan_hash": (C.c_uint64, [c_void_p]),
     "ec_rn50_set_conv8_min_tiles": (c_int, [c_void_p, c_int]),
+    "ec_rn50_set_l1_rebuild": (c_int, [c_void_p, c_int]),
     "ec_text_create": (c_int, [C.POINTER(c_void_p), c_int, c_int, c_int, c_int, c_int, c_int, c_void_p, c_size_t, c_void_p,
                                c_size_t]),
     "ec_text_destroy": (None, [c_void_p]),
@@ -74,6 +75,7 @@
     "ec_probe_pool3": (c_int, [c_void_p, c_void_p, c_int, c_int, c_int, c_int, c_void_p]),
     "ec_conv1x1_pair_pool_bf16": (c_int, [c_void_p] * 9 + [c_int] * 6 + [c_void_p]),
     "ec_conv1x1_pair_bf16": (c_int, [c_void_p] * 11 + [C.c_long, c_int, c_int, c_int, c_void_p]),
+    "ec_conv1x1_pair_rebuild_bf16": (c_int, [c_void_p] * 13 + [C.c_long, c_int, c_int, c_int, c_void_p]),
     "ec_stem_conv1_u8": (c_int, [c_void_p, C.POINTER(c_float), C.POINTER(c_float), c_void_p, c_void_p, c_void_p]
                          + [c_int] * 4 + [c_void_p]),
     "ec_rn50_forward_u8": (c_int, [c_void_p, c_void_p, C.POINTER(c_float), C.POINTER(c_float), c_int, c_void_p,
diff --git a/embodied_clip_amd/csrc/conv_pair.hip b/embodied_clip_amd/csrc/conv_pair.hip
--- a/embodied_clip_amd/csrc/conv_pair.hip
+++ b/embodied_clip_amd/csrc/conv_pair.hip
@@ -1,16 +1,9 @@
 #include <stdlib.h>
 
-#include <type_traits>
-#include <utility>
-
-#include "common.h"
+#include "conv_pair_common.h"
 
 namespace {
 
-typedef unsigned int u32x4 __attribute__((ext_vector_type(4)));
-constexpr int PX = 32;
-constexpr int NY = 256;
-constexpr int KA = 64;
 constexpr int SP = 272;
 constexpr int STG = PX * SP;
 
@@ -28,39 +21,6 @@
 }
 __device__ __forceinline__ float pq_xor2(float v) {
     return __builtin_bit_cast(float, __builtin_amdgcn_update_dpp(0, __builtin_bit_cast(int, v), 0x4E, 0xF, 0xF, true));
-}
-
-__device__ __forceinline__ int pw_off(int row, int chunk) {
-    return row * 128 + ((chunk ^ ((row >> 1) & 7)) << 4);
-}
-
-template <int I, int LEAD, class AddrFn>
-__device__ __forceinline__ void lsm_issue(u32x4 (&ring)[LEAD], AddrFn& addr) {
-    const auto a = addr(std::integral_constant<int, I>{});
-    asm volatile("ds_read_b128 %0, %1 offset:%2" : "=v"(ring[I % LEAD]) : "v"(a.first), "n"(decltype(a.second)::value));
-}
-template <int I, int NSTEP, int LEAD, class AddrFn, class MmaFn>
-__device__ __forceinline__ void lsm_step(u32x4 (&ring)[LEAD], AddrFn& addr, MmaFn& mma) {
-    if constexpr (I < NSTEP) {
-        constexpr int after = (LEAD - 1 < NSTEP - 1 - I) ? LEAD - 1 : NSTEP - 1 - I;
-        asm volatile("s_waitcnt lgkmcnt(%1)" : "+v"(ring[I % LEAD]) : "n"(after));
-        mma(std::integral_constant<int, I>{}, ring[I % LEAD]);
-        if constexpr (I + LEAD < NSTEP) lsm_issue<I + LEAD, LEAD>(ring, addr);
-        lsm_step<I + 1, NSTEP, LEAD>(ring, addr, mma);
-    }
-}
-template <int I, int N, int LEAD, class AddrFn>
-__device__ __forceinline__ void lsm_prologue(u32x4 (&ring)[LEAD], AddrFn& addr) {
-    if constexpr (I < N) {
-        lsm_issue<I, LEAD>(ring, addr);
-        lsm_prologue<I + 1, N, LEAD>(ring, addr);
-    }
-}
-template <int NSTEP, int LEAD, class AddrFn, class MmaFn>
-__device__ __forceinline__ void lds_stream_mfma(AddrFn addr, MmaFn mma) {
-    u32x4 ring[LEAD];
-    lsm_prologue<0, (LEAD < NSTEP ? LEAD : NSTEP), LEAD>(ring, addr);
-    lsm_step<0, NSTEP, LEAD>(ring, addr, mma);
 }
 
 template <bool TWO, bool RES, int N2, bool PL>
@@ -81,6 +41,7 @@
     unsigned wk_off[4];
 #pragma unroll
     for (int ks = 0; ks < 4; ++ks) wk_off[ks] = (unsigned)pw_off(px, 2 * ks + h);
+    const unsigned b_lds = w_lds + (unsigned)(W0_BYTES + W2_BYTES) + 16u * h;
     auto roff = [&](int r) -> int {
         if (!PL) return r;
         return (2 * (r >> 4) + ((r >> 1) & 1)) * p.W + 2 * ((r >> 2) & 3) + (r & 1);
@@ -194,16 +155,14 @@
                     ((*reinterpret_cast<u32x4*>(stg + ((I * 64 + lane) >> 4) * SP + ((I * 64 + lane) & 15) * 16) = rc[hf * 8 + I]), ...);
                 }(std::make_integer_sequence<int, 8>{});
             }
-#pragma unroll
-            for (int jj = 0; jj < 4; ++jj) {
-                const int j = hf * 4 + jj;
-                unsigned pk[8];
-#pragma unroll
-                for (int g = 0; g < 4; ++g) {
+            lds_stream_mfma<16, 4>(
+                [&](auto ic) { return std::pair<unsigned, std::integral_constant<int, hf * 512 + 32 * decltype(ic)::value>>{b_lds, {}}; },
+                [&](auto ic, const u32x4& bq) {
+                    constexpr int i = decltype(ic)::value, jj = i / 4, g = i % 4, j = hf * 4 + jj;
                     const int lc = 32 * jj + 8 * g + 4 * h;
-                    const float4 bv = *reinterpret_cast<const float4*>(sBy + hf * 128 + lc);
-                    float v0 = acc[j][4 * g + 0] + bv.x, v1 = acc[j][4 * g + 1] + bv.y;
-                    float v2 = acc[j][4 * g + 2] + bv.z, v3 = acc[j][4 * g + 3] + bv.w;
+                    const f32x4_t bv = __builtin_bit_cast(f32x4_t, bq);
+                    float v0 = acc[j][4 * g + 0] + bv[0], v1 = acc[j][4 * g + 1] + bv[1];
+                    float v2 = acc[j][4 * g + 2] + bv[2], v3 = acc[j][4 * g + 3] + bv[3];
                     uint2* slot = reinterpret_cast<uint2*>(stg + px * SP + lc * 2);
                     if (RES) {
                         const uint2 rr = *slot;
@@ -214,11 +173,10 @@
                     o.x = ec_pack2(v0, v1);
                     o.y = ec_pack2(v2, v3);
                     *slot = o;
-                    pk[2 * g] = o.x; pk[2 * g + 1] = o.y;
-                }
-                P[j][0] = make_uint4(pk[0], pk[1], pk[2], pk[3]);
-                P[j][1] = make_uint4(pk[4], pk[5], pk[6], pk[7]);
-            }
+                    uint4& pq = P[j][g >> 1];
+                    if constexpr (g & 1) { pq.z = o.x; pq.w = o.y; }
+                    else { pq.x = o.x; pq.y = o.y; }
+                });
             if constexpr (PL) {
 #pragma unroll
                 for (int it2 = 0; it2 < 2; ++it2) {
@@ -238,7 +196,7 @@
                     *reinterpret_cast<u32x4*>(p.yp + (pool_base + (w >> 2) * (p.W / 2) + (w & 3)) * NY + hf * 128 + c * 8) = po;
                 }
             }
-            if (!PL || p.y) {
+            if (p.y) {
 #pragma unroll
             for (int i = 0; i < 8; ++i) {
                 const int idx = i * 64 + lane;
@@ -267,17 +225,17 @@
             });
         constexpr int ZP = N2 * 2 + 16;
         constexpr int ZC = N2 / 8;
-#pragma unroll
-        for (int n = 0; n < FN2; ++n)
-#pragma unroll
-            for (int g = 0; g < 4; ++g) {
+        lds_stream_mfma<4 * FN2, 4>(
+            [&](auto ic) { return std::pair<unsigned, std::integral_constant<int, NY * 4 + 32 * decltype(ic)::value>>{b_lds, {}}; },
+            [&](auto ic, const u32x4& bq) {
+                constexpr int i = decltype(ic)::value, n = i / 4, g = i % 4;
                 const int lc = 32 * n + 8 * g + 4 * h;
-                const float4 bv = *reinterpret_cast<const float4*>(sBz + lc);
+                const f32x4_t bv = __builtin_bit_cast(f32x4_t, bq);
                 uint2 o;
-                o.x = ec_pack2(fmaxf(acc2[n][4 * g + 0] + bv.x, 0.f), fmaxf(acc2[n][4 * g + 1] + bv.y, 0.f));
-                o.y = ec_pack2(fmaxf(acc2[n][4 * g + 2] + bv.z, 0.f), fmaxf(acc2[n][4 * g + 3] + bv.w, 0.f));
+                o.x = ec_pack2(fmaxf(acc2[n][4 * g + 0] + bv[0], 0.f), fmaxf(acc2[n][4 * g + 1] + bv[1], 0.f));
+                o.y = ec_pack2(fmaxf(acc2[n][4 * g + 2] + bv[2], 0.f), fmaxf(acc2[n][4 * g + 3] + bv[3], 0.f));
                 *reinterpret_cast<uint2*>(stg + px * ZP + lc * 2) = o;
-            }
+            });
 #pragma unroll
         for (int i = 0; i < PX * ZC / 64; ++i) {
             const int idx = i * 64 + lane;
@@ -662,10 +620,11 @@
 extern "C" int ec_conv1x1_pair_bf16(const void* a0, const void* w0, const float* b0, const void* a1, const void* w1,
                                     const float* b1, const void* res, void* y, const void* w2, const float* b2, void* z,
                                     long M, int K0, int N, int N2, ec_stream_t stream) {
-    if (!a0 || !w0 || !b0 || !y || !w2 || !b2 || !z) return EC_ERR_ARG;
+    if (!a0 || !w0 || !b0 || !w2 || !b2 || !z) return EC_ERR_ARG;
     if ((a1 != nullptr) != (w1 != nullptr) || (a1 != nullptr) != (b1 != nullptr)) return EC_ERR_ARG;
     if (M <= 0 || (M % PX) != 0 || M / PX > 0x7fffffffL) return EC_ERR_SHAPE;
     if (K0 == K2 && N == NY2 && N2 == NZ2) {
+        if (!y) return EC_ERR_ARG;
         if (a1 || !res) return EC_ERR_SHAPE;
         Pair2Args q{(const uint16_t*)a0, (const uint16_t*)w0, (const uint16_t*)w2, (const uint16_t*)res, b0, b2, (uint16_t*)y,
                     (uint16_t*)z, (int)(M / PX)};
diff --git a/embodied_clip_amd/csrc/conv_pair_common.h b/embodied_clip_amd/csrc/conv_pair_common.h
--- /dev/null
+++ b/embodied_clip_amd/csrc/conv_pair_common.h
@@ -0,0 +1,48 @@
+#pragma once
+
+#include <type_traits>
+#include <utility>
+
+#include "common.h"
+
+namespace {
+
+typedef unsigned int u32x4 __attribute__((ext_vector_type(4)));
+constexpr int PX = 32;
+constexpr int NY = 256;
+constexpr int KA = 64;
+
+__device__ __forceinline__ int pw_off(int row, int chunk) {
+    return row * 128 + ((chunk ^ ((row >> 1) & 7)) << 4);
+}
+
+template <int I, int LEAD, class AddrFn>
+__device__ __forceinline__ void lsm_issue(u32x4 (&ring)[LEAD], AddrFn& addr) {
+    const auto a = addr(std::integral_constant<int, I>{});
+    asm volatile("ds_read_b128 %0, %1 offset:%2" : "=v"(ring[I % LEAD]) : "v"(a.first), "n"(decltype(a.second)::value));
+}
+template <int I, int NSTEP, int LEAD, class AddrFn, class MmaFn>
+__device__ __forceinline__ void lsm_step(u32x4 (&ring)[LEAD], AddrFn& addr, MmaFn& mma) {
+    if constexpr (I < NSTEP) {
+        constexpr int after = (LEAD - 1 < NSTEP - 1 - I) ? LEAD - 1 : NSTEP - 1 - I;
+        asm volatile("s_waitcnt lgkmcnt(%1)" : "+v"(ring[I % LEAD]) : "n"(after));
+        mma(std::integral_constant<int, I>{}, ring[I % LEAD]);
+        if constexpr (I + LEAD < NSTEP) lsm_issue<I + LEAD, LEAD>(ring, addr);
+        lsm_step<I + 1, NSTEP, LEAD>(ring, addr, mma);
+    }
+}
+template <int I, int N, int LEAD, class AddrFn>
+__device__ __forceinline__ void lsm_prologue(u32x4 (&ring)[LEAD], AddrFn& addr) {
+    if constexpr (I < N) {
+        lsm_issue<I, LEAD>(ring, addr);
+        lsm_prologue<I + 1, N, LEAD>(ring, addr);
+    }
+}
+template <int NSTEP, int LEAD, class AddrFn, class MmaFn>
+__device__ __forceinline__ void lds_stream_mfma(AddrFn addr, MmaFn mma) {
+    u32x4 ring[LEAD];
+    lsm_prologue<0, (LEAD < NSTEP ? LEAD : NSTEP), LEAD>(ring, addr);
+    lsm_step<0, NSTEP, LEAD>(ring, addr, mma);
+}
+
+}
diff --git a/embodied_clip_amd/csrc/conv_pair_rebuild.hip b/embodied_clip_amd/csrc/conv_pair_rebuild.hip
--- /dev/null
+++ b/embodied_clip_amd/csrc/conv_pair_rebuild.hip
@@ -0,0 +1,231 @@
+#include <stdlib.h>
+
+#include "conv_pair_common.h"
+
+namespace {
+
+constexpr int N2R = 64;
+constexpr int QP = 144;
+constexpr int QSTG = PX * QP;
+constexpr int WIMG = NY * 128;
+constexpr size_t LDS_REBUILD = 4 * (size_t)WIMG + (2 * NY + N2R) * 4 + 4 * (size_t)QSTG;
+static_assert(LDS_REBUILD <= 160 * 1024, "LDS budget");
+
+struct RebuildArgs {
+    const uint16_t *a, *i0, *i1, *w3, *wi0, *wi1, *w2;
+    const float *b3, *bi0, *bi1, *b2;
+    uint16_t *y, *z;
+    int ntiles;
+};
+
+__global__ __launch_bounds__(256, 1) void conv1x1_pair_rebuild_kernel(RebuildArgs p) {
+    extern __shared__ __attribute__((aligned(16))) unsigned char sm[];
+    unsigned char* sWi = sm;
+    unsigned char* sW2 = sm + 3 * WIMG;
+    float* sBi = reinterpret_cast<float*>(sm + 4 * WIMG);
+    float* sBy = sBi + NY;
+    float* sBz = sBy + NY;
+    const int tid = threadIdx.x, lane = tid & 63, wave = tid >> 6;
+    unsigned char* stg = sm + 4 * WIMG + (2 * NY + N2R) * 4 + wave * QSTG;
+    const int px = lane & 31, h = lane >> 5;
+    const unsigned w_lds = (unsigned)(unsigned long)(__attribute__((address_space(3))) unsigned char*)sm;
+    const unsigned b_lds = w_lds + 4u * WIMG + 16u * h;
+    unsigned wk_off[4];
+#pragma unroll
+    for (int ks = 0; ks < 4; ++ks) wk_off[ks] = (unsigned)pw_off(px, 2 * ks + h);
+
+    ec_stage_all<3 * NY * 8, 256, uint4>(
+        tid,
+        [&](int idx) {
+            const int kt = idx / (NY * 8), r = (idx / 8) % NY, c = idx & 7;
+            return *reinterpret_cast<const uint4*>((kt == 0 ? p.wi0 : kt == 1 ? p.wi1 : p.w3) + r * KA + c * 8);
+        },
+        [&](int idx, const uint4& v) {
+            const int kt = idx / (NY * 8), r = (idx / 8) % NY, c = idx & 7;
+            *reinterpret_cast<uint4*>(sWi + kt * WIMG + pw_off(r, c)) = v;
+        });
+    ec_stage_all<N2R * 32, 256, uint4>(
+        tid,
+        [&](int idx) {
+            const int n = idx >> 5, q = idx & 31;
+            const int s = q >> 1, hh = q & 1;
+            const int c0 = 32 * (s >> 1) + 16 * (s & 1) + 4 * hh;
+            const uint2 lo = *reinterpret_cast<const uint2*>(p.w2 + n * NY + c0);
+            const uint2 hi = *reinterpret_cast<const uint2*>(p.w2 + n * NY + c0 + 8);
+            return make_uint4(lo.x, lo.y, hi.x, hi.y);
+        },
+        [&](int idx, const uint4& v) {
+            const int n = idx >> 5, q = idx & 31;
+            const int s = q >> 1, hh = q & 1;
+            *reinterpret_cast<uint4*>(sW2 + (s >> 2) * (N2R * 128) + pw_off(n, 2 * (s & 3) + hh)) = v;
+        });
+    for (int i = tid; i < NY; i += 256) {
+        sBi[i] = p.bi0[i] + p.bi1[i];
+        sBy[i] = p.b3[i] + 0.f;
+    }
+    for (int i = tid; i < N2R; i += 256) sBz[i] = p.b2[i];
+    __syncthreads();
+
+    const int gw = blockIdx.x * 4 + wave, GW = gridDim.x * 4;
+    int t = gw;
+    if (t >= p.ntiles) return;
+
+    u32x4 an[4], i0n[4], i1n[4];
+    auto prefetch = [&](int tile) {
+        const long row = (long)tile * PX + px;
+#pragma unroll
+        for (int ks = 0; ks < 4; ++ks) {
+            i0n[ks] = *reinterpret_cast<const u32x4*>(p.i0 + row * KA + (2 * ks + h) * 8);
+            i1n[ks] = *reinterpret_cast<const u32x4*>(p.i1 + row * KA + (2 * ks + h) * 8);
+            an[ks] = *reinterpret_cast<const u32x4*>(p.a + row * KA + (2 * ks + h) * 8);
+        }
+    };
+    prefetch(t);
+
+    for (;;) {
+        const long m0 = (long)t * PX;
+        u32x4 ac[4], i0c[4], i1c[4];
+#pragma unroll
+        for (int ks = 0; ks < 4; ++ks) { ac[ks] = an[ks]; i0c[ks] = i0n[ks]; i1c[ks] = i1n[ks]; }
+        const int tn = t + GW;
+        const bool more = tn < p.ntiles;
+        if (more) prefetch(tn);
+
+        f32x16_t acc[8];
+#pragma unroll
+        for (int j = 0; j < 8; ++j)
+#pragma unroll
+            for (int r = 0; r < 16; ++r) acc[j][r] = 0.f;
+        lds_stream_mfma<64, 8>(
+            [&](auto ic) {
+                constexpr int i = decltype(ic)::value, ks = i / 16, r = i % 16, j = r & 7, second = r >> 3;
+                return std::pair<unsigned, std::integral_constant<int, second * WIMG + j * 4096>>{w_lds + wk_off[ks], {}};
+            },
+            [&](auto ic, const u32x4& wf) {
+                constexpr int i = decltype(ic)::value, ks = i / 16, r = i % 16, j = r & 7, second = r >> 3;
+                acc[j] = __builtin_amdgcn_mfma_f32_32x32x16_bf16(__builtin_bit_cast(bf16x8_t, wf),
+                                                                 __builtin_bit_cast(bf16x8_t, second ? i1c[ks] : i0c[ks]), acc[j], 0, 0, 0);
+            });
+        uint4 P[8][2];
+        lds_stream_mfma<32, 4>(
+            [&](auto ic) { return std::pair<unsigned, std::integral_constant<int, 32 * decltype(ic)::value>>{b_lds, {}}; },
+            [&](auto ic, const u32x4& bq) {
+                constexpr int i = decltype(ic)::value, j = i / 4, g = i % 4;
+                const f32x4_t bv = __builtin_bit_cast(f32x4_t, bq);
+                const float v0 = fmaxf(acc[j][4 * g + 0] + bv[0], 0.f), v1 = fmaxf(acc[j][4 * g + 1] + bv[1], 0.f);
+                const float v2 = fmaxf(acc[j][4 * g + 2] + bv[2], 0.f), v3 = fmaxf(acc[j][4 * g + 3] + bv[3], 0.f);
+                uint4& o = P[j][g >> 1];
+                if constexpr (g & 1) { o.z = ec_pack2(v0, v1); o.w = ec_pack2(v2, v3); }
+                else { o.x = ec_pack2(v0, v1); o.y = ec_pack2(v2, v3); }
+            });
+
+#pragma unroll
+        for (int j = 0; j < 8; ++j)
+#pragma unroll
+            for (int r = 0; r < 16; ++r) acc[j][r] = 0.f;
+        lds_stream_mfma<32, 8>(
+            [&](auto ic) {
+                constexpr int i = decltype(ic)::value, ks = i / 8, j = i % 8;
+                return std::pair<unsigned, std::integral_constant<int, j * 4096>>{w_lds + (unsigned)(2 * WIMG) + wk_off[ks], {}};
+            },
+            [&](auto ic, const u32x4& wf) {
+                constexpr int i = decltype(ic)::value, ks = i / 8, j = i % 8;
+                acc[j] = __builtin_amdgcn_mfma_f32_32x32x16_bf16(__builtin_bit_cast(bf16x8_t, wf), __builtin_bit_cast(bf16x8_t, ac[ks]),
+                                                                 acc[j], 0, 0, 0);
+            });
+
+        auto quarter_epilogue = [&](auto qc) {
+            constexpr int qt = decltype(qc)::value;
+            lds_stream_mfma<8, 4>(
+                [&](auto ic) {
+                    return std::pair<unsigned, std::integral_constant<int, NY * 4 + qt * 256 + 32 * decltype(ic)::value>>{b_lds, {}};
+                },
+                [&](auto ic, const u32x4& bq) {
+                    constexpr int i = decltype(ic)::value, jj = i / 4, g = i % 4, j = qt * 2 + jj;
+                    const int lc = 32 * jj + 8 * g + 4 * h;
+                    const f32x4_t bv = __builtin_bit_cast(f32x4_t, bq);
+                    uint4& idv = P[j][g >> 1];
+                    const unsigned rx = (g & 1) ? idv.z : idv.x, ry = (g & 1) ? idv.w : idv.y;
+                    float v0 = acc[j][4 * g + 0] + bv[0], v1 = acc[j][4 * g + 1] + bv[1];
+                    float v2 = acc[j][4 * g + 2] + bv[2], v3 = acc[j][4 * g + 3] + bv[3];
+                    v0 += ec_lo(rx); v1 += ec_hi(rx); v2 += ec_lo(ry); v3 += ec_hi(ry);
+                    v0 = fmaxf(v0, 0.f); v1 = fmaxf(v1, 0.f); v2 = fmaxf(v2, 0.f); v3 = fmaxf(v3, 0.f);
+                    uint2 o;
+                    o.x = ec_pack2(v0, v1);
+                    o.y = ec_pack2(v2, v3);
+                    *reinterpret_cast<uint2*>(stg + px * QP + lc * 2) = o;
+                    if constexpr (g & 1) { idv.z = o.x; idv.w = o.y; }
+                    else { idv.x = o.x; idv.y = o.y; }
+                });
+#pragma unroll
+            for (int i = 0; i < 4; ++i) {
+                const int idx = i * 64 + lane;
+                const uint4 v = *reinterpret_cast<const uint4*>(stg + (idx >> 3) * QP + (idx & 7) * 16);
+                __builtin_nontemporal_store(__builtin_bit_cast(u32x4, v),
+                                            reinterpret_cast<u32x4*>(p.y + (m0 + (idx >> 3)) * NY + qt * 64 + (idx & 7) * 8));
+            }
+        };
+        quarter_epilogue(std::integral_constant<int, 0>{});
+        quarter_epilogue(std::integral_constant<int, 1>{});
+        quarter_epilogue(std::integral_constant<int, 2>{});
+        quarter_epilogue(std::integral_constant<int, 3>{});
+
+        f32x16_t acc2[2];
+#pragma unroll
+        for (int n = 0; n < 2; ++n)
+#pragma unroll
+            for (int r = 0; r < 16; ++r) acc2[n][r] = 0.f;
+        lds_stream_mfma<32, 8>(
+            [&](auto ic) {
+                constexpr int i = decltype(ic)::value, st = i / 2, n = i % 2;
+                return std::pair<unsigned, std::integral_constant<int, (st >> 2) * (N2R * 128) + n * 4096>>{
+                    w_lds + (unsigned)(3 * WIMG) + wk_off[st & 3], {}};
+            },
+            [&](auto ic, const u32x4& wf) {
+                constexpr int i = decltype(ic)::value, st = i / 2, n = i % 2;
+                acc2[n] = __builtin_amdgcn_mfma_f32_32x32x16_bf16(__builtin_bit_cast(bf16x8_t, wf),
+                                                                  __builtin_bit_cast(bf16x8_t, P[st >> 1][st & 1]), acc2[n], 0, 0, 0);
+            });
+        lds_stream_mfma<8, 4>(
+            [&](auto ic) { return std::pair<unsigned, std::integral_constant<int, 2 * NY * 4 + 32 * decltype(ic)::value>>{b_lds, {}}; },
+            [&](auto ic, const u32x4& bq) {
+                constexpr int i = decltype(ic)::value, n = i / 4, g = i % 4;
+                const int lc = 32 * n + 8 * g + 4 * h;
+                const f32x4_t bv = __builtin_bit_cast(f32x4_t, bq);
+                uint2 o;
+                o.x = ec_pack2(fmaxf(acc2[n][4 * g + 0] + bv[0], 0.f), fmaxf(acc2[n][4 * g + 1] + bv[1], 0.f));
+                o.y = ec_pack2(fmaxf(acc2[n][4 * g + 2] + bv[2], 0.f), fmaxf(acc2[n][4 * g + 3] + bv[3], 0.f));
+                *reinterpret_cast<uint2*>(stg + px * QP + lc * 2) = o;
+            });
+#pragma unroll
+        for (int i = 0; i < 4; ++i) {
+            const int idx = i * 64 + lane;
+            const uint4 v = *reinterpret_cast<const uint4*>(stg + (idx >> 3) * QP + (idx & 7) * 16);
+            __builtin_nontemporal_store(__builtin_bit_cast(u32x4, v), reinterpret_cast<u32x4*>(p.z + (m0 + (idx >> 3)) * N2R + (idx & 7) * 8));
+        }
+        if (!more) break;
+        t = tn;
+    }
+}
+
+}
+
+extern "C" int ec_conv1x1_pair_rebuild_bf16(const void* a, const void* w3, const float* b3, const void* i0, const void* wi0,
+                                            const float* bi0, const void* i1, const void* wi1, const float* bi1, void* y,
+                                            const void* w2, const float* b2, void* z, long M, int K0, int N, int N2,
+                                            ec_stream_t stream) {
+    if (!a || !w3 || !b3 || !i0 || !wi0 || !bi0 || !i1 || !wi1 || !bi1 || !y || !w2 || !b2 || !z) return EC_ERR_ARG;
+    if (M <= 0 || (M % PX) != 0 || M / PX > 0x7fffffffL) return EC_ERR_SHAPE;
+    if (K0 != KA || N != NY || N2 != N2R) return EC_ERR_SHAPE;
+    RebuildArgs p{(const uint16_t*)a,  (const uint16_t*)i0, (const uint16_t*)i1, (const uint16_t*)w3, (const uint16_t*)wi0,
+                  (const uint16_t*)wi1, (const uint16_t*)w2, b3, bi0, bi1, b2, (uint16_t*)y, (uint16_t*)z, (int)(M / PX)};
+    static std::atomic<uint64_t> attr_done{0};
+    if (auto attr_g_ = ec_attr_needed(attr_done)) {
+        (void)hipFuncSetAttribute(reinterpret_cast<const void*>(conv1x1_pair_rebuild_kernel), hipFuncAttributeMaxDynamicSharedMemorySize,
+                                  (int)LDS_REBUILD);
+    }
+    const int wgs = (p.ntiles + 3) / 4 < 256 ? (p.ntiles + 3) / 4 : 256;
+    hipLaunchKernelGGL(conv1x1_pair_rebuild_kernel, dim3((unsigned)wgs), dim3(256), LDS_REBUILD, (hipStream_t)stream, p);
+    EC_CHECK_LAUNCH();
+    return EC_OK;
+}
diff --git a/embodied_clip_amd/csrc/rn50.hip b/embodied_clip_amd/csrc/rn50.hip
--- a/embodied_clip_amd/csrc/rn50.hip
+++ b/embodied_clip_amd/csrc/rn50.hip
@@ -33,6 +33,9 @@
     struct { int dst, ld, col; } pd;
     Conv c1, c2, c3, ds, next_c1;
     bool fold_ds;
+    bool no_y;
+    bool rebuild;
+    Conv id_c3, id_ds;
     int pooled_dst;
     bool fold_c1;
     size_t wpack_off;
@@ -51,6 +54,8 @@
     const float* bias;
     size_t n_w, n_b;
     int conv8_min_tiles = 0;
+    int layers4[4] = {0, 0, 0, 0};
+    int l1_rebuild = 0;
     uint16_t* wbneck = nullptr;
     float* bias_cat = nullptr;
     ~ec_rn50() {
@@ -73,10 +78,14 @@
     bool ds, last_of_layer;
     Slot c1, c2, c3, dsc;
 };
-struct Arch { TowerKind kind; int width, R1; Slot stem[3], total; std::vector<Blk> B; };
-
-Arch walk_arch(TowerKind kind, int width, int sc, const int* layers4, int R) {
-    Arch a{kind, width, R};
+struct Arch {
+    TowerKind kind; int width, R1;
+    bool l1_rebuild;
+    Slot stem[3], total; std::vector<Blk> B;
+};
+
+Arch walk_arch(TowerKind kind, int width, int sc, const int* layers4, int R, bool l1_rebuild = false) {
+    Arch a{kind, width, R, l1_rebuild};
     Slot& at = a.total;
     auto take = [&](size_t Cout, size_t K) { const Slot s = at; at.w += Cout * K; at.b += Cout; return s; };
     a.stem[0] = take(kind == CLIP ? sc : width, 0);
@@ -99,6 +108,7 @@
             x = k.y; inplanes = k.planes * expansion; R = k.Ro;
         }
     if (!a.B.empty()) a.B.back().out = BUF_OUT;
+    if (l1_rebuild && !a.B.empty()) a.B[0].x = a.B[0].y;
     return a;
 }
 
@@ -178,11 +188,20 @@
         return Given{};
     }
     if (f == F_PAIR1 || f == F_PAIR1_POOL) {
+        const bool rb0 = a.l1_rebuild && i == 0, rb1 = a.l1_rebuild && i == 1;
+        if (rb1) c2.dst = 3;
         p.conv(c2);
         o.kind = OP_PAIR;
-        o.c3 = mk_conv(2, k.out, k.ds ? BUF_NONE : x, R, R, planes, planes * 4, 1, 0, EC_ACT_RELU, k.c3);
+        o.c3 = mk_conv(c2.dst, k.out, k.ds || rb1 ? BUF_NONE : x, R, R, planes, planes * 4, 1, 0, EC_ACT_RELU, k.c3);
         o.fold_ds = k.ds;
         if (k.ds) o.ds = mk_conv(x, BUF_NONE, BUF_NONE, R, R, inplanes, planes * 4, 1, 0, EC_ACT_NONE, k.dsc);
+        o.no_y = rb0;
+        if (rb1) {
+            const Blk& b0 = a.B[0];
+            o.rebuild = true;
+            o.id_c3 = mk_conv(2, BUF_NONE, BUF_NONE, R, R, b0.planes, b0.planes * 4, 1, 0, EC_ACT_RELU, b0.c3);
+            o.id_ds = mk_conv(b0.x, BUF_NONE, BUF_NONE, R, R, b0.inplanes, b0.planes * 4, 1, 0, EC_ACT_NONE, b0.dsc);
+        }
         o.next_c1 = mk_conv(k.out, 1, BUF_NONE, R, R, planes * 4, nx->planes, 1, 0, EC_ACT_RELU, nx->c1);
         o.pooled_dst = f == F_PAIR1_POOL ? 3 : BUF_NONE;
         if (f == F_PAIR1_POOL) p.track(R / 2, R / 2, planes * 4);
@@ -248,18 +267,24 @@
     p.push(o, Ro, Ro, planes);
 }
 
-int pack_plan_weights(ec_rn50* h) {
-    size_t tot = 0, btot = 0;
-    auto cat_n = [](const Op& o) { return (size_t)(o.kind == OP_CAT ? o.c.Cout : o.c2.Cout); };
-    for (Op& o : h->ops)
+size_t cat_n(const Op& o) { return (size_t)(o.kind == OP_CAT ? o.c.Cout : o.c2.Cout); }
+
+void plan_offsets(std::vector<Op>& ops, size_t& tot, size_t& btot) {
+    tot = btot = 0;
+    for (Op& o : ops)
         if (o.kind == OP_CAT || o.kind == OP_BTAIL) {
             o.cat.w_off = tot; tot += cat_n(o) * (size_t)(o.cat.Ka + o.cat.Kb);
             o.cat.b_off = btot; btot += cat_n(o);
         }
-    for (Op& o : h->ops) {
+    for (Op& o : ops) {
         if (o.kind == OP_BNECK) { o.wpack_off = o.c2.wimg_off = tot; tot += ec_bneck3_packed_elems(o.c2.Cin); }
         if (o.kind == OP_CONV && o.c.img_max) { o.c.wimg_off = tot; tot += (size_t)o.c.Cout * 9 * o.c.Cin; }
     }
+}
+
+int pack_plan_weights(ec_rn50* h) {
+    size_t tot = 0, btot = 0;
+    plan_offsets(h->ops, tot, btot);
     if (btot && hipMalloc(&h->bias_cat, btot * sizeof(float)) != hipSuccess) { h->bias_cat = nullptr; return EC_ERR_LAUNCH; }
     if (!tot) return EC_OK;
     if (hipMalloc(&h->wbneck, tot * sizeof(uint16_t)) != hipSuccess) { h->wbneck = nullptr; return EC_ERR_LAUNCH; }
@@ -287,22 +312,14 @@
     return EC_OK;
 }
 
-int rn50_build(ec_rn50_t** out, TowerKind kind, int width, const int* layers4, int input_resolution, const void* stem_w,
-               const void* w_bf16, size_t n_w, const float* bias, size_t n_bias) {
-    if (!out || !layers4 || !stem_w || !w_bf16 || !bias) return EC_ERR_ARG;
-    if (width % 32 != 0 || width < 32 || input_resolution % 32 != 0) return EC_ERR_SHAPE;
-    if (kind == TV_BASIC && (input_resolution < 32 || layers4[0] < 1 || layers4[1] < 1 || layers4[2] < 1 || layers4[3] < 1)) return EC_ERR_SHAPE;
-    const int sc = (width / 2 + 31) / 32 * 32, res = input_resolution;
-    const Arch a = walk_arch(kind, width, sc, layers4, res / 4);
-    if (n_w != a.total.w || n_bias != a.total.b) return EC_ERR_SHAPE;
-    ec_rn50* h = new (std::nothrow) ec_rn50();
-    if (!h) return EC_ERR_ALLOC;
-    h->width = width; h->res = res; h->tv = kind;
-    h->stem_w = (const float*)stem_w; h->w = (const uint16_t*)w_bf16; h->bias = bias;
-    h->n_w = a.total.w; h->n_b = a.total.b;
-    Plan p{h->ops};
-    const int x0 = a.B.empty() ? BUF_OUT : 0;
-    if (kind == CLIP) {
+int stem_channels(int width) { return (width / 2 + 31) / 32 * 32; }
+
+size_t plan_tower(std::vector<Op>& ops, const Arch& a, int res) {
+    ops.clear();
+    Plan p{ops};
+    const int width = a.width, sc = stem_channels(width);
+    const int x0 = a.B.empty() ? BUF_OUT : a.B[0].x;
+    if (a.kind == CLIP) {
         const int R = res / 2;
         p.push(Op{OP_STEM1, mk_conv(BUF_IN, 1, BUF_NONE, res, res, 3, sc, 3, 0, EC_ACT_RELU, a.stem[0])}, R, R, sc);
         p.conv(mk_conv(1, 2, BUF_NONE, R, R, sc, sc, 3, 0, EC_ACT_RELU, a.stem[1]));
@@ -312,11 +329,32 @@
     }
     Given g;
     for (size_t i = 0; i < a.B.size(); ++i)
-        if (kind == TV_BASIC) plan_basic(p, a.B[i]);
+        if (a.kind == TV_BASIC) plan_basic(p, a.B[i]);
         else g = plan_bottleneck(p, a, i, g);
+    return p.mx;
+}
+
+bool l1_rebuild_ok(const Arch& a) {
+    return a.kind == CLIP && a.B.size() >= 3 && a.B[0].ds && block_form(a, 0) == F_PAIR1 && block_form(a, 1) == F_PAIR1;
+}
+
+int rn50_build(ec_rn50_t** out, TowerKind kind, int width, const int* layers4, int input_resolution, const void* stem_w,
+               const void* w_bf16, size_t n_w, const float* bias, size_t n_bias) {
+    if (!out || !layers4 || !stem_w || !w_bf16 || !bias) return EC_ERR_ARG;
+    if (width % 32 != 0 || width < 32 || input_resolution % 32 != 0) return EC_ERR_SHAPE;
+    if (kind == TV_BASIC && (input_resolution < 32 || layers4[0] < 1 || layers4[1] < 1 || layers4[2] < 1 || layers4[3] < 1)) return EC_ERR_SHAPE;
+    const int res = input_resolution;
+    const Arch a = walk_arch(kind, width, stem_channels(width), layers4, res / 4);
+    if (n_w != a.total.w || n_bias != a.total.b) return EC_ERR_SHAPE;
+    ec_rn50* h = new (std::nothrow) ec_rn50();
+    if (!h) return EC_ERR_ALLOC;
+    h->width = width; h->res = res; h->tv = kind;
+    std::copy(layers4, layers4 + 4, h->layers4);
+    h->stem_w = (const float*)stem_w; h->w = (const uint16_t*)w_bf16; h->bias = bias;
+    h->n_w = a.total.w; h->n_b = a.total.b;
+    h->max_elems_per_frame = plan_tower(h->ops, a, res);
     h->out_c = a.B.empty() ? width : a.B.back().planes * (kind == TV_BASIC ? 1 : 4);
     h->out_sp = a.B.empty() ? a.R1 : a.B.back().Ro;
-    h->max_elems_per_frame = p.mx;
     const int rc = pack_plan_weights(h);
     if (rc != EC_OK) { delete h; return rc; }
     *out = h;
@@ -352,6 +390,7 @@
     };
     mix(ec_version()); mix((long)ec_config_hash());
     mix(h->width); mix(h->res); mix(h->conv8_min_tiles); mix(h->tv);
+    if (h->l1_rebuild) mix(h->l1_rebuild);
     for (const Op& o : h->ops) {
         const Conv& c = o.kind == OP_PAIR || o.kind == OP_BNECK ? o.c3 : o.kind == OP_BTAIL ? o.c2 : o.c;
         long f[24] = {o.kind, c.src, c.dst, c.res, c.H, c.W, c.Cin, c.Cout, c.ks, c.pool, c.act, c.stride, -1, -1, 0, -1, 0, c.ldo, c.ocol, 0, -1, 0, 0, 0};
@@ -373,6 +412,21 @@
 extern "C" int ec_rn50_set_conv8_min_tiles(ec_rn50_t* h, int n) {
     if (!h) return EC_ERR_ARG;
     h->conv8_min_tiles = n > 0 ? n : 0;
+    return EC_OK;
+}
+
+extern "C" int ec_rn50_set_l1_rebuild(ec_rn50_t* h, int on) {
+    if (!h) return EC_ERR_ARG;
+    const Arch a = walk_arch((TowerKind)h->tv, h->width, stem_channels(h->width), h->layers4, h->res / 4, on != 0);
+    if (!l1_rebuild_ok(a)) return EC_ERR_UNSUPPORTED;
+    if ((on != 0) == (h->l1_rebuild != 0)) return EC_OK;
+    std::vector<Op> ops;
+    const size_t mx = plan_tower(ops, a, h->res);
+    size_t tot = 0, btot = 0;
+    plan_offsets(ops, tot, btot);
+    if (mx != h->max_elems_per_frame) return EC_ERR_UNSUPPORTED;
+    h->ops.swap(ops);
+    h->l1_rebuild = on != 0;
     return EC_OK;
 }
 
@@ -465,9 +519,14 @@
     if (o.pooled_dst != BUF_NONE)
         return ec_conv1x1_pair_pool_bf16(r.buf(c3.src), h->w + c3.at.w, h->bias + c3.at.b, r.buf(c3.res), nullptr, r.buf(o.pooled_dst),
                                          h->w + c1.at.w, h->bias + c1.at.b, r.buf(c1.dst), r.nb, c3.H, c3.W, c3.Cin, c3.Cout, c1.Cout, r.stream);
+    if (o.rebuild)
+        return ec_conv1x1_pair_rebuild_bf16(r.buf(c3.src), h->w + c3.at.w, h->bias + c3.at.b, r.buf(o.id_c3.src), h->w + o.id_c3.at.w,
+                                            h->bias + o.id_c3.at.b, r.buf(o.id_ds.src), h->w + o.id_ds.at.w, h->bias + o.id_ds.at.b,
+                                            r.buf(c3.dst), h->w + c1.at.w, h->bias + c1.at.b, r.buf(c1.dst), (long)r.nb * c3.H * c3.W,
+                                            c3.Cin, c3.Cout, c1.Cout, r.stream);
     int rc = ec_conv1x1_pair_bf16(r.buf(c3.src), h->w + c3.at.w, h->bias + c3.at.b, o.fold_ds ? r.buf(o.ds.src) : nullptr,
                                   o.fold_ds ? h->w + o.ds.at.w : nullptr, o.fold_ds ? h->bias + o.ds.at.b : nullptr, r.opt(c3.res),
-                                  r.buf(c3.dst), h->w + c1.at.w, h->bias + c1.at.b, r.buf(c1.dst), (long)r.nb * c3.H * c3.W, c3.Cin, c3.Cout,
+                                  o.no_y ? nullptr : r.buf(c3.dst), h->w + c1.at.w, h->bias + c1.at.b, r.buf(c1.dst), (long)r.nb * c3.H * c3.W, c3.Cin, c3.Cout,
                                   c1.Cout, r.stream);
     if (rc == EC_ERR_SHAPE && !o.fold_ds) {
         rc = run_conv(r, c3);
diff --git a/embodied_clip_amd/encoder.py b/embodied_clip_amd/encoder.py
--- a/embodied_clip_amd/encoder.py
+++ b/embodied_clip_amd/encoder.py
@@ -165,6 +165,13 @@
 
     def set_conv8_min_tiles(self, n: int) -> None:
         _lib.check(self.lib.ec_rn50_set_conv8_min_tiles(self.h, int(n)), "ec_rn50_set_conv8_min_tiles")
+
+    def set_l1_rebuild(self, on: bool = True) -> bool:
+        rc = self.lib.ec_rn50_set_l1_rebuild(self.h, int(bool(on)))
+        if rc == -6:
+            return False
+        _lib.check(rc, "ec_rn50_set_l1_rebuild")
+        return True
 
     def _workspace(self, n: int) -> torch.Tensor:
         need = self.lib.ec_rn50_workspace_bytes(self.h, n)
@@ -647,15 +654,28 @@
 
 
 @_guard_first
-def conv1x1_pair_bf16(a0, w0, b0, w2, b2, a1=None, w1=None, b1=None, res=None):
+def conv1x1_pair_bf16(a0, w0, b0, w2, b2, a1=None, w1=None, b1=None, res=None, store_y=True):
     lib = _lib.load()
     M, K0 = a0.shape
     N, N2 = w0.shape[0], w2.shape[0]
-    y = torch.empty((M, N), dtype=torch.bfloat16, device=a0.device)
+    y = torch.empty((M, N), dtype=torch.bfloat16, device=a0.device) if store_y else None
     z = torch.empty((M, N2), dtype=torch.bfloat16, device=a0.device)
     _lib.check(lib.ec_conv1x1_pair_bf16(a0.data_ptr(), w0.data_ptr(), b0.data_ptr(), _lib.ptr(a1), _lib.ptr(w1),
-                                        _lib.ptr(b1), _lib.ptr(res), y.data_ptr(), w2.data_ptr(), b2.data_ptr(),
+                                        _lib.ptr(b1), _lib.ptr(res), _lib.ptr(y), w2.data_ptr(), b2.data_ptr(),
                                         z.data_ptr(), M, K0, N, N2, _lib.stream_ptr()), "ec_conv1x1_pair_bf16")
+    return y, z
+
+
+@_guard_first
+def conv1x1_pair_rebuild_bf16(a, w3, b3, i0, wi0, bi0, i1, wi1, bi1, w2, b2):
+    lib = _lib.load()
+    M, K0 = a.shape
+    N, N2 = w3.shape[0], w2.shape[0]
+    y = torch.empty((M, N), dtype=torch.bfloat16, device=a.device)
+    z = torch.empty((M, N2), dtype=torch.bfloat16, device=a.device)
+    _lib.check(lib.ec_conv1x1_pair_rebuild_bf16(a.data_ptr(), w3.data_ptr(), b3.data_ptr(), i0.data_ptr(), wi0.data_ptr(), bi0.data_ptr(),
+                                                i1.data_ptr(), wi1.data_ptr(), bi1.data_ptr(), y.data_ptr(), w2.data_ptr(), b2.data_ptr(),
+                                                z.data_ptr(), M, K0, N, N2, _lib.stream_ptr()), "ec_conv1x1_pair_rebuild_bf16")
     return y, z
 
 
diff --git a/embodied_clip_amd/engine.py b/embodied_clip_amd/engine.py
--- a/embodied_clip_amd/engine.py
+++ b/embodied_clip_amd/engine.py
@@ -335,6 +335,9 @@
         self._conv8_min_tiles = (50 if n >= 128 else (75 if n >= 64 else 0)) if ns == 2 else 0
         for e in encs:
             e.set_conv8_min_tiles(self._conv8_min_tiles)
+        if encoder == "rn50":
+            for e in encs:
+                e.set_l1_rebuild(True)
         fused = os.environ.get("EC_ACT_FUSED_SAMPLE", "1") != "0"
         self._act_fused = fused and self.A + 1 <= 8
         self._act_wide = fused and 8 < self.A + 1 <= 257 and self.H <= 3576
diff --git a/include/ec_amd.h b/include/ec_amd.h
--- a/include/ec_amd.h
+++ b/include/ec_amd.h
@@ -74,6 +74,11 @@
 int ec_conv1x1_pair_bf16(const void* a0, const void* w0, const float* b0, const void* a1, const void* w1,
                          const float* b1, const void* res, void* y, const void* w2, const float* b2, void* z,
                          long M, int K0, int N, int N2, ec_stream_t stream);
+
+int ec_conv1x1_pair_rebuild_bf16(const void* a, const void* w3, const float* b3, const void* i0, const void* wi0,
+                                 const float* bi0, const void* i1, const void* wi1, const float* bi1, void* y,
+                                 const void* w2, const float* b2, void* z, long M, int K0, int N, int N2,
+                                 ec_stream_t stream);
 
 int ec_conv1x1_pair_pool_bf16(const void* a0, const void* w0, const float* b0, const void* res, void* y,
                               void* y_pooled, const void* w2, const float* b2, void* z, int B, int H, int W, int K0,
@@ -140,6 +145,7 @@
 int ec_rn50_num_ops(const ec_rn50_t* h);
 uint64_t ec_rn50_plan_hash(const ec_rn50_t* h);
 int ec_rn50_set_conv8_min_tiles(ec_rn50_t* h, int n);
+int ec_rn50_set_l1_rebuild(ec_rn50_t* h, int on);
 
 
 enum {
```

After: 65550, median of 6. 1.7% higher.
